# weiaicunzai/pytorch-camvid

Hardware: AMD Instinct MI355X
Metric: images/sec fwd+bwd UNet 3x360x480 bs=8 (higher is better)
Workload: dtype f32; 1 GPU; UNET(3,12) train fwd+bwd+CE, per-GPU batch 8 x 3x360x480 fp32 (BASELINE.json configs[1]); global_batch=8, parallelism=dp1

## Files before the change

include/cvk.h:

```cpp
#ifndef CVK_H
#define CVK_H

#include <stddef.h>
#include <stdint.h>

#ifdef __cplusplus
extern "C" {
#endif

#define CVK_VERSION 100
#define CVK_OK 0
#define CVK_EINVAL (-1)
#define CVK_EWORKSPACE (-2)
#define CVK_STAT_ROWS 64

typedef struct cvk_view {
    float*  ptr;
    int64_t sN, sY, sX;
} cvk_view;

typedef struct cvk_viewh {
    void*   ptr;
    int64_t sN, sY, sX;
} cvk_viewh;

int         cvk_version(void);
uint64_t    cvk_abi_hash(void);
const char* cvk_last_error_string(void);

int cvk_import_nchw(const float* src, int64_t sN, int64_t sC, int64_t sH, int64_t sW,
                    float* dst, int ld, int N, int C, int H, int W, void* stream);
int cvk_export_nchw(const float* src, int ld, float* dst, int64_t dN, int64_t dC, int64_t dH, int64_t dW,
                    int N, int C, int H, int W, void* stream);
int cvk_zero_frame(cvk_view buf, int N, int H, int W, int C, int y0, int x0, int h, int w, void* stream);

int cvk_conv3x3_fwd(const float* x, const float* w, const float* bias, float* y, float* stats,
                    int N, int H, int W, int Cin, int Cout, int ldy, void* stream);
int cvk_pack_weight_fwd(const float* w_src, float* dst, int Cout, int Cin, int Cin_pad, void* stream);
int cvk_pack_weight_dgrad(const float* w_src, float* dst, int Cout, int Cin, int Cin_pad, int Cout_pad, void* stream);
size_t cvk_conv3x3_wgrad_workspace_bytes(int N, int H, int W, int Cin_pad, int Cout);
int cvk_conv3x3_wgrad(const float* x, const float* dy, float* dw, int N, int H, int W, int Cin, int Cin_pad,
                      int Cout, int ld_dy, void* workspace, size_t workspace_bytes, void* stream);

int cvk_wino_weight_transform(const float* w, float* U, int Cout, int Cin, void* stream);
size_t cvk_conv3x3_wino_workspace_bytes(int N, int H, int W, int Cout_ld);
int cvk_conv3x3_wino_gemm(const float* x, const float* U, float* Mo, int N, int H, int W, int Cin, int Cout, int ldm,
                          void* stream);
int cvk_wino_output(const float* Mo, const float* bias, float* y, float* stats, int N, int H, int W, int Cout, int ldy,
                    void* stream);

int cvk_wino4_weight_transform(const float* w, float* U, int Cout, int Cin, void* stream);
int cvk_wino4_weight_transform_dgrad(const float* w, float* U, int Cout, int Cin, void* stream);
int cvk_conv3x3_wino4_ksplit(int N, int H, int W, int Cin, int Cout_ld);
size_t cvk_conv3x3_wino4_workspace_bytes(int N, int H, int W, int Cin, int Cout_ld);
int cvk_conv3x3_wino4_gemm(const float* x, const float* U, float* Mo, int N, int H, int W, int Cin, int Cout, int ldm,
                           void* stream);
int cvk_wino4_output(const float* Mo, const float* bias, float* y, float* stats, int N, int H, int W, int Cout, int ldy,
                     int ksplit, void* stream);

int cvk_w2d_tiles(int N, int H, int W);
int cvk_w2d_tpad(int T);
int cvk_w2d_stat_partials(int N, int H, int W);
size_t cvk_conv3x3_w2d_workspace_bytes(int N, int H, int W, int Cin, int Cout);
int cvk_w2d_weight_transform(const float* w, float* U, int Cout, int Cin, void* stream);
int cvk_w2d_weight_transform_dgrad(const float* w, float* U, int Cout, int Cin, void* stream);
int cvk_conv3x3_w2d(const float* x, const float* U, const float* bias, float* y, float* stats, float* counts, int N, int H,
                    int W, int Cin, int Cout, int ldy, void* workspace, size_t workspace_bytes, void* stream);
int cvk_w2d_ksplit(int T, int Cin, int Cout);
int cvk_w2d_input_transform(const float* x, float* V, int N, int H, int W, int Cin, void* stream);
int cvk_w2d_gemm(const float* V, const float* U, float* Mo, int T, int Cin, int Cout, void* stream);
int cvk_w2d_output(const float* Mo, const float* bias, float* y, float* stats, float* counts, int N, int H, int W, int Cin,
                   int Cout, int ldy, void* stream);
size_t cvk_conv3x3_wgrad_w2d_workspace_bytes(int N, int H, int W, int Cin_pad, int Cout);
int cvk_conv3x3_wgrad_w2d(const float* x, const float* dy, float* dw, int N, int H, int W, int Cin, int Cin_pad, int Cout,
                          int ld_dy, void* workspace, size_t workspace_bytes, void* stream);
int cvk_w2d_wgrad_ksplit(int T, int Cin_pad, int Cout);
int cvk_w2d_dy_transform(const float* dy, int ld_dy, float* E, int N, int H, int W, int Cout, void* stream);
int cvk_w2d_dy_transform_both(const float* dy, int ld_dy, float* Vp, float* E, int N, int H, int W, int Cout, void* stream);
int cvk_w2d_gemm_tn(const float* E, const float* V, float* P, int T, int Cin_pad, int Cout, void* stream);
int cvk_w2d_wgrad_output(const float* P, float* dw, int T, int Cin, int Cin_pad, int Cout, void* stream);

int cvk_w6_tiles(int N, int H, int W);
int cvk_w6_stat_partials(int N, int H, int W);
size_t cvk_conv3x3_w6_workspace_bytes(int N, int H, int W, int Cin, int Cout);
int cvk_w6_weight_transform(const float* w, float* U, int Cout, int Cin, void* stream);
int cvk_w6_weight_transform_dgrad(const float* w, float* U, int Cout, int Cin, void* stream);
int cvk_w6_ksplit(int T, int Cin, int Cout);
int cvk_w6_input_transform(const float* x, float* V, int N, int H, int W, int Cin, void* stream);
int cvk_w6_gemm(const float* V, const float* U, float* Mo, int T, int Cin, int Cout, void* stream);
int cvk_w6_output(const float* Mo, const float* bias, float* y, float* stats, float* counts, int N, int H, int W, int Cin,
                  int Cout, int ldy, void* stream);
int cvk_w6_wgrad_ksplit(int T, int Cin_pad, int Cout);
int cvk_w6_dy_transform(const float* dy, int ld_dy, float* E, int N, int H, int W, int Cout, void* stream);
int cvk_w6_dy_transform_both(const float* dy, int ld_dy, float* Vp, float* E, int N, int H, int W, int Cout, void* stream);
int cvk_w6_gemm_tn(const float* E, const float* V, float* P, int T, int Cin_pad, int Cout, void* stream);
int cvk_split3_rows_pad(int R, int mult);
int cvk_split3_planes(const float* P, void* S, int NX, int R, int Rpad, int C, void* stream);
int cvk_w2d_gemm_split3(const void* V3, const void* U3, float* Mo, int NX, int T, int Tpad, int Cin, int Cout, int Cpad, void* stream);
int cvk_amax_block_words(void);
unsigned cvk_amax_block_value(const unsigned* host_words, int n);
int cvk_absmax_f32(const float* x, long rows, int C, int ld, void* amax_block, void* stream);
int cvk_split_scale_exponent(int tile, int kind, int xi, unsigned amax_block);
int cvk_split_planes(int fmt, int tile, int kind, const float* P, void* S, const void* amax, int NX, int R, int Rpad, int C, void* stream);
int cvk_w2d_gemm_split(int fmt, int tile, const void* V, const void* U, float* Mo, const void* amax_v, const void* amax_u, int NX, int T, int Tpad,
                       int Cin, int Cout, int Cpad, void* stream);
int cvk_w2d_input_transform_split3(int tile, const float* x, void* V3, int N, int H, int W, int Cin, void* stream);
int cvk_w2d_dy_transform_both_split3(int tile, const float* dy, int ld_dy, void* Vp3, void* E, int e_split, int N, int H, int W, int C,
                                     void* stream);
int cvk_w2d_weight_transform_split3(int tile, const float* w, void* U3, float* tmp, int Cout, int Cin, int dgrad, void* stream);
int cvk_w2d_input_transform_split(int fmt, int tile, const float* x, void* V, const void* amax_x, int N, int H, int W, int Cin, void* stream);
int cvk_w2d_dy_transform_both_split(int fmt, int tile, const float* dy, int ld_dy, void* Vp, void* E, int e_split, const void* amax_dy, int N, int H,
                                    int W, int C, void* stream);
int cvk_w2d_weight_transform_split(int fmt, int tile, const float* w, void* U, const void* amax_w, int Cout, int Cin, int dgrad, void* stream);
int cvk_w2d_output_plain(int tile, const float* Mo, const float* bias, float* y, float* stats, float* counts, int N, int H, int W,
                         int Cout, int ldy, void* stream);
int cvk_w2d_gemm_tn_split3_ksplit(int NX, int Tpad, int Cin, int Cout);
int cvk_w2d_gemm_tn_split3(const void* E3, const void* V3, float* P, int NX, int Tpad, int Cin, int Cout, void* stream);
int cvk_w2d_gemm_tn_split(int fmt, int tile, const void* E, const void* V, float* P, const void* amax_e, const void* amax_v, int NX, int Tpad, int Cin,
                          int Cout, void* stream);
int cvk_w2d_wgrad_output_f(int tile, const float* P, float* dw, int Cin, int Cin_pad, int Cout, int f, void* stream);
int cvk_w6_wgrad_output(const float* P, float* dw, int T, int Cin, int Cin_pad, int Cout, void* stream);
int cvk_wino4h_weight_transform(const float* w, void* Uh, const void* amax_w, int Cn, int Ck, int dgrad, void* stream);
int cvk_conv3x3_wino4h(const float* x, const void* Uh, const float* bias, float* y, float* stats, float* counts, const void* amax_x,
                       const void* amax_w, int N, int H, int W, int Cin, int Cout, int ldy, int max_workgroups, void* stream);
int cvk_conv3x3_wino4h_bnred(const float* x, const void* Uh, float* y, const void* amax_x, const void* amax_w, int N, int H, int W, int Cin,
                             int Cout, int ldy, const float* yP, const float* scale, const float* shift, const float* mean,
                             const float* rstd, float* part, int max_workgroups, void* stream);
size_t cvk_wino4f_weight_floats(int Cn, int Ck);
int cvk_wino4f_weight_transform(const float* w, float* Uf, int Cn, int Ck, int dgrad, void* stream);
#define CVK_WT_BATCH_MAX 48
typedef struct cvk_wt_job { const float* w; float* out; int rows, cols, tile, dgrad; } cvk_wt_job;
int cvk_wino4f_weight_transform_batch(const cvk_wt_job* jobs, int n, void* stream);
int cvk_w2d_weight_transform_batch(const cvk_wt_job* jobs, int n, void* stream);
int cvk_wino4f_stat_partials(int N, int H, int W);
int cvk_conv3x3_wino4f_vplanes(const float* x, const float* Uf, const float* bias, float* y, float* stats, float* counts, float* Vsm,
                               int N, int H, int W, int Cin, int Cout, int ldy, int max_workgroups, void* stream);
int cvk_conv3x3_wino4f(const float* x, const float* Uf, const float* bias, float* y, float* stats, float* counts, int N, int H,
                       int W, int Cin, int Cout, int ldy, int max_workgroups, void* stream);
int cvk_conv3x3_wino4f_bnred(const float* x, const float* Uf, float* y, int N, int H, int W, int Cin, int Cout, int ldy,
                             const float* yP, const float* scale, const float* shift, const float* mean, const float* rstd,
                             float* part, int max_workgroups, void* stream);

int cvk_thin_fwd_supported(int Cin_ld, int Cout, int ldy);
int cvk_thin_stat_partials(int N, int H, int W, int Cin_ld);
int cvk_conv3x3_thin_fwd(const float* x, const float* w, const float* bias, float* y, float* stats, float* counts, int N, int H,
                         int W, int Cin_ld, int Cout, int ldy, void* stream);
int cvk_thin_wgrad_supported(int Cin, int Cin_ld, int Cout, int ld_dy);
size_t cvk_conv3x3_thin_wgrad_workspace_bytes(int N, int H, int W, int Cin_ld, int Cout);
int cvk_conv3x3_thin_wgrad(const float* x, const float* dy, float* dw, int N, int H, int W, int Cin, int Cin_ld, int Cout,
                           int ld_dy, void* workspace, size_t workspace_bytes, void* stream);

size_t cvk_conv3x3_wgradp_workspace_bytes(int N, int H, int W, int Cin_pad, int Cout);
int cvk_conv3x3_wgradp(const float* x, const float* dy, const float* E6_pre, float* dw, int N, int H, int W, int Cin, int Cin_pad,
                       int Cout, int ld_dy, void* workspace, size_t workspace_bytes, void* stream);
long cvk_wgradp_plane_rows(int N, int H, int W);
int cvk_wgradp_planes(const float* t, int ld, float* planes, int N, int H, int W, int C, int is_dy, void* stream);
size_t cvk_wgradp_gemm_workspace_bytes(int N, int H, int W, int Cin_pad, int Cout);
int cvk_wgradp_gemm(const float* E6, const float* V6, float* dw, int N, int H, int W, int Cin, int Cin_pad, int Cout, void* workspace,
                    size_t workspace_bytes, void* stream);
int cvk_wgradp_zero_pads(float* planes, int N, int H, int W, int C, void* stream);
int cvk_wgradp_zero_pads_sm(float* planes, int N, int H, int W, int C, void* stream);
int cvk_wgradp_planes_sm(const float* x, int ld, float* planes, int N, int H, int W, int C, void* stream);
int cvk_wgradp_gemm_sm(const float* E6, const float* V6sm, float* dw, int N, int H, int W, int Cin, int Cin_pad, int Cout, void* workspace,
                       size_t workspace_bytes, void* stream);
int cvk_wgradp_zero_pads4(float* planes, int N, int H, int W, int C, void* stream);
int cvk_bn_bwd_dx_e4p(cvk_view dout, const float* y, int ldy, const float* scale, const float* shift, const float* mean,
                      const float* rstd, const float* dgamma, const float* dbeta, float* dy, int ld_dy, float* E4p, float* part,
                      int N, int H, int W, int C, int use_batch_stats, void* stream);
int cvk_wgradp_dy_slack(int W);
int cvk_wgradp_gemm_sm_dy(const float* E4p, const float* dy, const float* V6sm, float* dw, int N, int H, int W, int Cin, int Cin_pad, int Cout,
                          void* workspace, size_t workspace_bytes, void* stream);
int cvk_bn_bwd_dx_e6(cvk_view dout, const float* y, int ldy, const float* scale, const float* shift, const float* mean,
                     const float* rstd, const float* dgamma, const float* dbeta, float* dy, int ld_dy, float* E6, float* part,
                     int N, int H, int W, int C, int use_batch_stats, void* stream);

size_t cvk_conv3x3_wgrad_wino4_workspace_bytes(int N, int H, int W, int Cin_pad, int Cout, int ld_dy);
int cvk_conv3x3_wgrad_wino4(const float* x, const float* dy, const float* E_pre, float* dw, int N, int H, int W, int Cin,
                            int Cin_pad, int Cout, int ld_dy, void* workspace, size_t workspace_bytes, void* stream);
int cvk_bn_bwd_e_blocks(int N, int H, int W);
int cvk_bn_bwd_dx_e(cvk_view dout, const float* y, int ldy, const float* scale, const float* shift, const float* mean,
                    const float* rstd, const float* dgamma, const float* dbeta, float* dy, int ld_dy, float* E, float* part,
                    int N, int H, int W, int C, int use_batch_stats, void* stream);

size_t cvk_conv3x3_wgrad_wino_workspace_bytes(int N, int H, int W, int Cin_pad, int Cout);
int cvk_conv3x3_wgrad_wino(const float* x, const float* dy, float* dw, int N, int H, int W, int Cin, int Cin_pad,
                           int Cout, int ld_dy, void* workspace, size_t workspace_bytes, void* stream);

size_t cvk_bn_finalize_workspace_bytes(int P, int C);
int cvk_bn_finalize(const float* stats, int P, int M, int C, const float* gamma, const float* beta,
                    float* mean, float* rstd, float* scale, float* shift,
                    float* running_mean, float* running_var, int64_t* num_batches_tracked,
                    float momentum, float eps, void* workspace, size_t workspace_bytes, void* stream);
int cvk_bn_eval_params(const float* gamma, const float* beta, const float* running_mean, const float* running_var,
                       float* mean, float* rstd, float* scale, float* shift, int C, float eps, void* stream);
int cvk_bn_relu_apply(const float* y, int ldy, const float* scale, const float* shift, cvk_view out,
                      int N, int H, int W, int C, void* stream);
int cvk_bn_relu_apply_pool(const float* y, int ldy, const float* scale, const float* shift, cvk_view out, float* pool,
                           unsigned char* code, int N, int H, int W, int C, void* stream);
int cvk_bn_bwd_blocks(int M);
int cvk_bn_bwd_reduce(cvk_view dout, const float* y, int ldy, const float* scale, const float* shift,
                      const float* mean, const float* rstd, float* part, int N, int H, int W, int C, void* stream);
int cvk_colsum_finalize(const float* part, int PB, int C, float* out0, float* out1, void* stream);
#define CVK_COLSUM_BATCH_MAX 64
typedef struct cvk_colsum_job { const float* part; float* out; int PB, C; } cvk_colsum_job;
int cvk_colsum_finalize_batch(const cvk_colsum_job* jobs, int n, void* stream);
int cvk_bn_relu_apply_amax(const float* y, int ldy, const float* scale, const float* shift, cvk_view out, int N, int H, int W, int C,
                           void* amax_block, void* stream);
int cvk_bn_relu_apply_pool_amax(const float* y, int ldy, const float* scale, const float* shift, cvk_view out, float* pool,
                                unsigned char* code, int N, int H, int W, int C, void* amax_out, void* amax_pool, void* stream);
int cvk_bn_bwd_dx_e_amax(int six, cvk_view dout, const float* y, int ldy, const float* scale, const float* shift, const float* mean,
                         const float* rstd, const float* dgamma, const float* dbeta, float* dy, int ld_dy, float* E, float* part, int N, int H,
                         int W, int C, int use_batch_stats, void* amax_block, void* stream);
int cvk_bn_bwd_dx_amax(cvk_view dout, const float* y, int ldy, const float* scale, const float* shift, const float* mean,
                       const float* rstd, const float* dgamma, const float* dbeta, float* dy, int ld_dy, float* dbias_part, int N,
                       int H, int W, int C, int use_batch_stats, void* amax_block, void* stream);
int cvk_bn_bwd_dx(cvk_view dout, const float* y, int ldy, const float* scale, const float* shift,
                  const float* mean, const float* rstd, const float* dgamma, const float* dbeta,
                  float* dy, int ld_dy, float* dbias_part, int N, int H, int W, int C, int use_batch_stats, void* stream);

int cvk_maxpool2x2_fwd(cvk_view x, float* out, uint8_t* code, int N, int H, int W, int C, void* stream);
int cvk_maxpool2x2_bwd(const float* dout, cvk_view x, const uint8_t* code, cvk_view dx, int accumulate,
                       int N, int H, int W, int C, void* stream);
int cvk_maxpool2x2_bwd_bnred_blocks(int N, int H, int W, int C);
int cvk_maxpool2x2_bwd_bnred(const float* dout, cvk_view x, const uint8_t* code, cvk_view dx, int accumulate, int N, int H, int W, int C,
                             const float* yP, int ldp, const float* scale, const float* shift, const float* mean, const float* rstd,
                             float* part, void* stream);
int cvk_maxunpool2x2_fwd(const float* v, const uint8_t* code, float* out, int N, int H, int W, int C, void* stream);
int cvk_maxunpool2x2_bwd(const float* dout, const uint8_t* code, float* dv, int N, int H, int W, int C, void* stream);
int cvk_pool_code_to_index(const uint8_t* code, int64_t* idx, int N, int H, int W, int C, void* stream);

int cvk_bilinear_up2_fwd(const float* x, float* out, int N, int H, int W, int C, void* stream);
int cvk_bilinear_up2_bwd(const float* dout, float* dx, int N, int H, int W, int C, void* stream);

int cvk_ce_blocks(int M);
int cvk_softmax_ce_fwd(const float* logits, int ld, const int64_t* target, float* part, float* loss,
                       int M, int C, int ignore_index, void* stream);
int cvk_softmax_ce_bwd(const float* logits, int ld, const int64_t* target, const float* loss3, const float* grad_out,
                       float scale, float* dlogits, int ld_d, int M, int C, int ignore_index, void* stream);

#define CVK_REDUCTION_NONE 0
#define CVK_REDUCTION_MEAN 1
#define CVK_REDUCTION_SUM 2
int cvk_ce_ex_part_floats(int M);
int cvk_softmax_ce_fwd_ex(const float* logits, int ld, const int64_t* target, const float* weight, float label_smoothing,
                          int reduction, float* part, float* loss, float* loss_px, int M, int C, int ignore_index, void* stream);
int cvk_softmax_ce_bwd_ex(const float* logits, int ld, const int64_t* target, const float* weight, float label_smoothing,
                          int reduction, const float* loss4, const float* grad_out, float scale, float* dlogits, int ld_d,
                          int M, int C, int ignore_index, void* stream);

#define CVK_DICE_PRESENT 0
#define CVK_DICE_ALL 1
int cvk_seg_loss_part_floats(int M, int C);
int cvk_seg_loss_record_floats(int C);
int cvk_seg_loss_fwd(const float* logits, int ld, const int64_t* target, const float* weight, float ce, float dice, float focal_gamma,
                     float dice_smooth, int dice_average, float* part, float* record, int M, int C, int ignore_index, void* stream);
int cvk_seg_loss_bwd(const float* logits, int ld, const int64_t* target, const float* weight, float ce, float dice, float focal_gamma,
                     const float* record, const float* grad_out, float scale, float* dlogits, int ld_d, int M, int C, int ignore_index,
                     void* stream);

int cvk_ohem_scratch_bytes(int M);
int cvk_ohem_record_floats(void);
int cvk_ohem_ce_fwd(const float* logits, int ld, const int64_t* target, const float* weight, float loss_thresh, int min_kept,
                    void* scratch, float* record, float* loss_px, int M, int C, int ignore_index, void* stream);
int cvk_ohem_ce_bwd(const float* logits, int ld, const int64_t* target, const float* weight, const float* record,
                    const float* loss_px, const float* grad_out, float scale, float* dlogits, int ld_d, int M, int C, int ignore_index,
                    void* stream);

int cvk_class_histogram(const void* masks, int mask_bytes, int N, int64_t HW, int num_classes, int ignore_index, int64_t* hist,
                        void* stream);

int cvk_argmax_channels(const float* logits, int ld, int64_t* out, int M, int C, void* stream);
int cvk_confusion_accumulate(const int64_t* pred, const int64_t* label, int64_t* hist, int M, int num_classes,
                             int ignore_index, void* stream);

int cvk_tta_accumulate(const float* logits, int ld, int h, int w, float* acc, int64_t* pred, int N, int H, int W, int C, int flip,
                       int first, int last, float inv_k, void* stream);
int cvk_tta_resize_input(const float* src, int64_t sN, int64_t sC, int64_t sH, int64_t sW, float* dst, int N, int H, int W, int h, int w,
                         int flip, void* stream);

int cvk_window_merge(const float* logits, int ld, float* out, int64_t* pred, int N, int H, int W, int C, int hc, int wc, int sy, int sx,
                     int iy, int ix, void* stream);

int cvk_preprocess_u8(const uint8_t* src, float* dst, int N, int H, int W, const float* mean3, const float* std3, void* stream);

typedef struct cvk_augment_record {
    int32_t flip;
    int32_t ksize;
    int32_t use_lut;
    int32_t reserved;
    float   taps[12];
    uint8_t lut[256];
} cvk_augment_record;
int cvk_augment_record_bytes(void);
int cvk_augment_u8(const uint8_t* frames, const void* masks, int mask_bytes, int N, int Hs, int Ws, int H, int W,
// ... 105 lines not shown
```

pytorch-camvid_amd/_lib.py:

```python
import ctypes
import os
import subprocess
import threading

_HERE = os.path.dirname(os.path.abspath(__file__))
LIB_PATH = os.environ.get("CVK_LIB_PATH") or os.path.join(_HERE, "lib", "libcvk.so")
CSRC = os.path.join(_HERE, "csrc")
HEADER = os.path.join(os.path.dirname(_HERE), "include", "cvk.h")

CVK_STAT_ROWS = 64

c_f32p = ctypes.c_void_p
c_i64 = ctypes.c_int64
c_int = ctypes.c_int
c_size = ctypes.c_size_t
c_float = ctypes.c_float
c_vp = ctypes.c_void_p


class View(ctypes.Structure):
    _fields_ = [("ptr", ctypes.c_void_p), ("sN", ctypes.c_int64), ("sY", ctypes.c_int64), ("sX", ctypes.c_int64)]


class ViewH(ctypes.Structure):
    _fields_ = [("ptr", ctypes.c_void_p), ("sN", ctypes.c_int64), ("sY", ctypes.c_int64), ("sX", ctypes.c_int64)]


SIGNATURES = {
    "cvk_version": (c_int, []),
    "cvk_abi_hash": (ctypes.c_uint64, []),
    "cvk_last_error_string": (ctypes.c_char_p, []),
    "cvk_import_nchw": (c_int, [c_vp, c_i64, c_i64, c_i64, c_i64, c_vp, c_int, c_int, c_int, c_int, c_int, c_vp]),
    "cvk_export_nchw": (c_int, [c_vp, c_int, c_vp, c_i64, c_i64, c_i64, c_i64, c_int, c_int, c_int, c_int, c_vp]),
    "cvk_zero_frame": (c_int, [View, c_int, c_int, c_int, c_int, c_int, c_int, c_int, c_int, c_vp]),
    "cvk_conv3x3_fwd": (c_int, [c_vp, c_vp, c_vp, c_vp, c_vp, c_int, c_int, c_int, c_int, c_int, c_int, c_vp]),
    "cvk_pack_weight_fwd": (c_int, [c_vp, c_vp, c_int, c_int, c_int, c_vp]),
    "cvk_pack_weight_dgrad": (c_int, [c_vp, c_vp, c_int, c_int, c_int, c_int, c_vp]),
    "cvk_conv3x3_wgrad_workspace_bytes": (c_size, [c_int, c_int, c_int, c_int, c_int]),
    "cvk_conv3x3_wgrad": (c_int, [c_vp, c_vp, c_vp, c_int, c_int, c_int, c_int, c_int, c_int, c_int, c_vp, c_size, c_vp]),
    "cvk_wino_weight_transform": (c_int, [c_vp, c_vp, c_int, c_int, c_vp]),
    "cvk_conv3x3_wino_workspace_bytes": (c_size, [c_int, c_int, c_int, c_int]),
    "cvk_conv3x3_wino_gemm": (c_int, [c_vp, c_vp, c_vp, c_int, c_int, c_int, c_int, c_int, c_int, c_vp]),
    "cvk_wino_output": (c_int, [c_vp, c_vp, c_vp, c_vp, c_int, c_int, c_int, c_int, c_int, c_vp]),
    "cvk_wino4_weight_transform": (c_int, [c_vp, c_vp, c_int, c_int, c_vp]),
    "cvk_wino4_weight_transform_dgrad": (c_int, [c_vp, c_vp, c_int, c_int, c_vp]),
    "cvk_conv3x3_wino4_ksplit": (c_int, [c_int, c_int, c_int, c_int, c_int]),
    "cvk_conv3x3_wino4_workspace_bytes": (c_size, [c_int, c_int, c_int, c_int, c_int]),
    "cvk_conv3x3_wino4_gemm": (c_int, [c_vp, c_vp, c_vp, c_int, c_int, c_int, c_int, c_int, c_int, c_vp]),
    "cvk_wino4_output": (c_int, [c_vp, c_vp, c_vp, c_vp, c_int, c_int, c_int, c_int, c_int, c_int, c_vp]),
    "cvk_wino4f_weight_floats": (c_size, [c_int, c_int]),
    "cvk_wino4f_weight_transform": (c_int, [c_vp, c_vp, c_int, c_int, c_int, c_vp]),
    "cvk_wino4f_weight_transform_batch": (c_int, [c_vp, c_int, c_vp]),
    "cvk_w2d_weight_transform_batch": (c_int, [c_vp, c_int, c_vp]),
    "cvk_wino4f_stat_partials": (c_int, [c_int, c_int, c_int]),
    "cvk_conv3x3_wino4f": (c_int, [c_vp, c_vp, c_vp, c_vp, c_vp, c_vp, c_int, c_int, c_int, c_int, c_int, c_int, c_int, c_vp]),
    "cvk_conv3x3_wino4f_bnred": (c_int, [c_vp, c_vp, c_vp, c_int, c_int, c_int, c_int, c_int, c_int, c_vp, c_vp, c_vp, c_vp, c_vp, c_vp, c_int, c_vp]),
    "cvk_wino4h_weight_transform": (c_int, [c_vp, c_vp, c_vp, c_int, c_int, c_int, c_vp]),
    "cvk_conv3x3_wino4h": (c_int, [c_vp, c_vp, c_vp, c_vp, c_vp, c_vp, c_vp, c_vp, c_int, c_int, c_int, c_int, c_int, c_int, c_int, c_vp]),
    "cvk_conv3x3_wino4h_bnred": (c_int, [c_vp, c_vp, c_vp, c_vp, c_vp, c_int, c_int, c_int, c_int, c_int, c_int, c_vp, c_vp, c_vp, c_vp, c_vp, c_vp,
                                         c_int, c_vp]),
    "cvk_thin_fwd_supported": (c_int, [c_int, c_int, c_int]),
    "cvk_thin_stat_partials": (c_int, [c_int, c_int, c_int, c_int]),
    "cvk_conv3x3_thin_fwd": (c_int, [c_vp, c_vp, c_vp, c_vp, c_vp, c_vp, c_int, c_int, c_int, c_int, c_int, c_int, c_vp]),
    "cvk_thin_wgrad_supported": (c_int, [c_int, c_int, c_int, c_int]),
    "cvk_conv3x3_thin_wgrad_workspace_bytes": (c_size, [c_int, c_int, c_int, c_int, c_int]),
    "cvk_conv3x3_thin_wgrad": (c_int, [c_vp, c_vp, c_vp, c_int, c_int, c_int, c_int, c_int, c_int, c_int, c_vp, c_size, c_vp]),
    "cvk_conv3x3_wgradp_workspace_bytes": (c_size, [c_int, c_int, c_int, c_int, c_int]),
    "cvk_conv3x3_wgradp": (c_int, [c_vp, c_vp, c_vp, c_vp, c_int, c_int, c_int, c_int, c_int, c_int, c_int, c_vp, c_size, c_vp]),
    "cvk_wgradp_plane_rows": (ctypes.c_long, [c_int, c_int, c_int]),
    "cvk_wgradp_planes": (c_int, [c_vp, c_int, c_vp, c_int, c_int, c_int, c_int, c_int, c_vp]),
    "cvk_wgradp_gemm_workspace_bytes": (c_size, [c_int, c_int, c_int, c_int, c_int]),
    "cvk_wgradp_gemm": (c_int, [c_vp, c_vp, c_vp, c_int, c_int, c_int, c_int, c_int, c_int, c_vp, c_size, c_vp]),
    "cvk_wgradp_zero_pads": (c_int, [c_vp, c_int, c_int, c_int, c_int, c_vp]),
    "cvk_wgradp_zero_pads_sm": (c_int, [c_vp, c_int, c_int, c_int, c_int, c_vp]),
    "cvk_wgradp_planes_sm": (c_int, [c_vp, c_int, c_vp, c_int, c_int, c_int, c_int, c_vp]),
    "cvk_wgradp_gemm_sm": (c_int, [c_vp, c_vp, c_vp, c_int, c_int, c_int, c_int, c_int, c_int, c_vp, c_size, c_vp]),
    "cvk_wgradp_zero_pads4": (c_int, [c_vp, c_int, c_int, c_int, c_int, c_vp]),
    "cvk_bn_bwd_dx_e4p": (c_int, [View, c_vp, c_int, c_vp, c_vp, c_vp, c_vp, c_vp, c_vp, c_vp, c_int, c_vp, c_vp,
                                  c_int, c_int, c_int, c_int, c_int, c_vp]),
    "cvk_wgradp_dy_slack": (c_int, [c_int]),
    "cvk_wgradp_gemm_sm_dy": (c_int, [c_vp, c_vp, c_vp, c_vp, c_int, c_int, c_int, c_int, c_int, c_int, c_vp, c_size, c_vp]),
    "cvk_conv3x3_wino4f_vplanes": (c_int, [c_vp, c_vp, c_vp, c_vp, c_vp, c_vp, c_vp, c_int, c_int, c_int, c_int, c_int, c_int, c_int, c_vp]),
    "cvk_bn_bwd_dx_e6": (c_int, [View, c_vp, c_int, c_vp, c_vp, c_vp, c_vp, c_vp, c_vp, c_vp, c_int, c_vp, c_vp,
                                 c_int, c_int, c_int, c_int, c_int, c_vp]),
    "cvk_w2d_tiles": (c_int, [c_int, c_int, c_int]),
    "cvk_w6_tiles": (c_int, [c_int, c_int, c_int]),
    "cvk_w6_stat_partials": (c_int, [c_int, c_int, c_int]),
    "cvk_conv3x3_w6_workspace_bytes": (c_size, [c_int, c_int, c_int, c_int, c_int]),
    "cvk_w6_weight_transform": (c_int, [c_vp, c_vp, c_int, c_int, c_vp]),
    "cvk_w6_weight_transform_dgrad": (c_int, [c_vp, c_vp, c_int, c_int, c_vp]),
    "cvk_w6_input_transform": (c_int, [c_vp, c_vp, c_int, c_int, c_int, c_int, c_vp]),
    "cvk_w6_gemm": (c_int, [c_vp, c_vp, c_vp, c_int, c_int, c_int, c_vp]),
    "cvk_w6_wgrad_ksplit": (c_int, [c_int, c_int, c_int]),
    "cvk_w6_dy_transform": (c_int, [c_vp, c_int, c_vp, c_int, c_int, c_int, c_int, c_vp]),
    "cvk_w6_gemm_tn": (c_int, [c_vp, c_vp, c_vp, c_int, c_int, c_int, c_vp]),
    "cvk_w6_wgrad_output": (c_int, [c_vp, c_vp, c_int, c_int, c_int, c_int, c_vp]),
    "cvk_w6_ksplit": (c_int, [c_int, c_int, c_int]),
    "cvk_w6_output": (c_int, [c_vp, c_vp, c_vp, c_vp, c_vp, c_int, c_int, c_int, c_int, c_int, c_int, c_vp]),
    "cvk_w2d_stat_partials": (c_int, [c_int, c_int, c_int]),
    "cvk_conv3x3_w2d_workspace_bytes": (c_size, [c_int, c_int, c_int, c_int, c_int]),
    "cvk_w2d_weight_transform": (c_int, [c_vp, c_vp, c_int, c_int, c_vp]),
    "cvk_w2d_weight_transform_dgrad": (c_int, [c_vp, c_vp, c_int, c_int, c_vp]),
    "cvk_w2d_input_transform": (c_int, [c_vp, c_vp, c_int, c_int, c_int, c_int, c_vp]),
    "cvk_w2d_gemm": (c_int, [c_vp, c_vp, c_vp, c_int, c_int, c_int, c_vp]),
    "cvk_conv3x3_wgrad_w2d_workspace_bytes": (c_size, [c_int, c_int, c_int, c_int, c_int]),
    "cvk_conv3x3_wgrad_w2d": (c_int, [c_vp, c_vp, c_vp, c_int, c_int, c_int, c_int, c_int, c_int, c_int, c_vp, c_size, c_vp]),
    "cvk_w2d_tpad": (c_int, [c_int]),
    "cvk_split3_rows_pad": (c_int, [c_int, c_int]),
    "cvk_split3_planes": (c_int, [c_vp, c_vp, c_int, c_int, c_int, c_int, c_vp]),
    "cvk_w2d_gemm_split3": (c_int, [c_vp, c_vp, c_vp, c_int, c_int, c_int, c_int, c_int, c_int, c_vp]),
    "cvk_w2d_input_transform_split3": (c_int, [c_int, c_vp, c_vp, c_int, c_int, c_int, c_int, c_vp]),
    "cvk_w2d_dy_transform_both_split3": (c_int, [c_int, c_vp, c_int, c_vp, c_vp, c_int, c_int, c_int, c_int, c_int, c_vp]),
    "cvk_w2d_weight_transform_split3": (c_int, [c_int, c_vp, c_vp, c_vp, c_int, c_int, c_int, c_vp]),
    "cvk_w2d_output_plain": (c_int, [c_int, c_vp, c_vp, c_vp, c_vp, c_vp, c_int, c_int, c_int, c_int, c_int, c_vp]),
    "cvk_w2d_gemm_tn_split3_ksplit": (c_int, [c_int, c_int, c_int, c_int]),
    "cvk_w2d_gemm_tn_split3": (c_int, [c_vp, c_vp, c_vp, c_int, c_int, c_int, c_int, c_vp]),
    "cvk_amax_block_words": (c_int, []),
    "cvk_amax_block_value": (ctypes.c_uint, [c_vp, c_int]),
    "cvk_absmax_f32": (c_int, [c_vp, ctypes.c_long, c_int, c_int, c_vp, c_vp]),
    "cvk_split_scale_exponent": (c_int, [c_int, c_int, c_int, ctypes.c_uint]),
    "cvk_split_planes": (c_int, [c_int, c_int, c_int, c_vp, c_vp, c_vp, c_int, c_int, c_int, c_int, c_vp]),
    "cvk_w2d_gemm_split": (c_int, [c_int, c_int, c_vp, c_vp, c_vp, c_vp, c_vp, c_int, c_int, c_int, c_int, c_int, c_int, c_vp]),
    "cvk_w2d_input_transform_split": (c_int, [c_int, c_int, c_vp, c_vp, c_vp, c_int, c_int, c_int, c_int, c_vp]),
    "cvk_w2d_dy_transform_both_split": (c_int, [c_int, c_int, c_vp, c_int, c_vp, c_vp, c_int, c_vp, c_int, c_int, c_int, c_int, c_vp]),
    "cvk_w2d_weight_transform_split": (c_int, [c_int, c_int, c_vp, c_vp, c_vp, c_int, c_int, c_int, c_vp]),
    "cvk_w2d_gemm_tn_split": (c_int, [c_int, c_int, c_vp, c_vp, c_vp, c_vp, c_vp, c_int, c_int, c_int, c_int, c_vp]),
    "cvk_w2d_wgrad_output_f": (c_int, [c_int, c_vp, c_vp, c_int, c_int, c_int, c_int, c_vp]),
    "cvk_w2d_wgrad_ksplit": (c_int, [c_int, c_int, c_int]),
    "cvk_w2d_dy_transform": (c_int, [c_vp, c_int, c_vp, c_int, c_int, c_int, c_int, c_vp]),
    "cvk_w2d_dy_transform_both": (c_int, [c_vp, c_int, c_vp, c_vp, c_int, c_int, c_int, c_int, c_vp]),
    "cvk_w6_dy_transform_both": (c_int, [c_vp, c_int, c_vp, c_vp, c_int, c_int, c_int, c_int, c_vp]),
    "cvk_w2d_gemm_tn": (c_int, [c_vp, c_vp, c_vp, c_int, c_int, c_int, c_vp]),
    "cvk_w2d_wgrad_output": (c_int, [c_vp, c_vp, c_int, c_int, c_int, c_int, c_vp]),
    "cvk_w2d_ksplit": (c_int, [c_int, c_int, c_int]),
    "cvk_w2d_output": (c_int, [c_vp, c_vp, c_vp, c_vp, c_vp, c_int, c_int, c_int, c_int, c_int, c_int, c_vp]),
    "cvk_conv3x3_w2d": (c_int, [c_vp, c_vp, c_vp, c_vp, c_vp, c_vp, c_int, c_int, c_int, c_int, c_int, c_int, c_vp, c_size, c_vp]),
    "cvk_conv3x3_wgrad_wino4_workspace_bytes": (c_size, [c_int, c_int, c_int, c_int, c_int, c_int]),
    "cvk_conv3x3_wgrad_wino4": (c_int, [c_vp, c_vp, c_vp, c_vp, c_int, c_int, c_int, c_int, c_int, c_int, c_int, c_vp, c_size, c_vp]),
    "cvk_bn_bwd_e_blocks": (c_int, [c_int, c_int, c_int]),
    "cvk_bn_bwd_dx_e": (c_int, [View, c_vp, c_int, c_vp, c_vp, c_vp, c_vp, c_vp, c_vp, c_vp, c_int, c_vp, c_vp,
                                c_int, c_int, c_int, c_int, c_int, c_vp]),
    "cvk_conv3x3_wgrad_wino_workspace_bytes": (c_size, [c_int, c_int, c_int, c_int, c_int]),
    "cvk_conv3x3_wgrad_wino": (c_int, [c_vp, c_vp, c_vp, c_int, c_int, c_int, c_int, c_int, c_int, c_int, c_vp, c_size, c_vp]),
    "cvk_bn_finalize_workspace_bytes": (c_size, [c_int, c_int]),
    "cvk_bn_finalize": (c_int, [c_vp, c_int, c_int, c_int, c_vp, c_vp, c_vp, c_vp, c_vp, c_vp, c_vp, c_vp, c_vp,
                                c_float, c_float, c_vp, c_size, c_vp]),
    "cvk_bn_eval_params": (c_int, [c_vp, c_vp, c_vp, c_vp, c_vp, c_vp, c_vp, c_vp, c_int, c_float, c_vp]),
    "cvk_bn_relu_apply": (c_int, [c_vp, c_int, c_vp, c_vp, View, c_int, c_int, c_int, c_int, c_vp]),
    "cvk_bn_relu_apply_pool": (c_int, [c_vp, c_int, c_vp, c_vp, View, c_vp, c_vp, c_int, c_int, c_int, c_int, c_vp]),
    "cvk_bn_bwd_blocks": (c_int, [c_int]),
    "cvk_bn_bwd_reduce": (c_int, [View, c_vp, c_int, c_vp, c_vp, c_vp, c_vp, c_vp, c_int, c_int, c_int, c_int, c_vp]),
    "cvk_colsum_finalize": (c_int, [c_vp, c_int, c_int, c_vp, c_vp, c_vp]),
    "cvk_colsum_finalize_batch": (c_int, [c_vp, c_int, c_vp]),
    "cvk_bn_bwd_dx": (c_int, [View, c_vp, c_int, c_vp, c_vp, c_vp, c_vp, c_vp, c_vp, c_vp, c_int, c_vp,
                              c_int, c_int, c_int, c_int, c_int, c_vp]),
    "cvk_bn_relu_apply_amax": (c_int, [c_vp, c_int, c_vp, c_vp, View, c_int, c_int, c_int, c_int, c_vp, c_vp]),
    "cvk_bn_relu_apply_pool_amax": (c_int, [c_vp, c_int, c_vp, c_vp, View, c_vp, c_vp, c_int, c_int, c_int, c_int, c_vp, c_vp, c_vp]),
    "cvk_bn_bwd_dx_e_amax": (c_int, [c_int, View, c_vp, c_int, c_vp, c_vp, c_vp, c_vp, c_vp, c_vp, c_vp, c_int, c_vp, c_vp,
                                     c_int, c_int, c_int, c_int, c_int, c_vp, c_vp]),
    "cvk_bn_bwd_dx_amax": (c_int, [View, c_vp, c_int, c_vp, c_vp, c_vp, c_vp, c_vp, c_vp, c_vp, c_int, c_vp,
                                   c_int, c_int, c_int, c_int, c_int, c_vp, c_vp]),
    "cvk_maxpool2x2_fwd": (c_int, [View, c_vp, c_vp, c_int, c_int, c_int, c_int, c_vp]),
    "cvk_maxpool2x2_bwd": (c_int, [c_vp, View, c_vp, View, c_int, c_int, c_int, c_int, c_int, c_vp]),
    "cvk_maxpool2x2_bwd_bnred_blocks": (c_int, [c_int, c_int, c_int, c_int]),
    "cvk_maxpool2x2_bwd_bnred": (c_int, [c_vp, View, c_vp, View, c_int, c_int, c_int, c_int, c_int, c_vp, c_int, c_vp, c_vp, c_vp, c_vp, c_vp, c_vp]),
    "cvk_maxunpool2x2_fwd": (c_int, [c_vp, c_vp, c_vp, c_int, c_int, c_int, c_int, c_vp]),
    "cvk_maxunpool2x2_bwd": (c_int, [c_vp, c_vp, c_vp, c_int, c_int, c_int, c_int, c_vp]),
    "cvk_pool_code_to_index": (c_int, [c_vp, c_vp, c_int, c_int, c_int, c_int, c_vp]),
    "cvk_bilinear_up2_fwd": (c_int, [c_vp, c_vp, c_int, c_int, c_int, c_int, c_vp]),
    "cvk_bilinear_up2_bwd": (c_int, [c_vp, c_vp, c_int, c_int, c_int, c_int, c_vp]),
    "cvk_ce_blocks": (c_int, [c_int]),
    "cvk_softmax_ce_fwd": (c_int, [c_vp, c_int, c_vp, c_vp, c_vp, c_int, c_int, c_int, c_vp]),
    "cvk_softmax_ce_bwd": (c_int, [c_vp, c_int, c_vp, c_vp, c_vp, c_float, c_vp, c_int, c_int, c_int, c_int, c_vp]),
    "cvk_ce_ex_part_floats": (c_int, [c_int]),
    "cvk_softmax_ce_fwd_ex": (c_int, [c_vp, c_int, c_vp, c_vp, c_float, c_int, c_vp, c_vp, c_vp, c_int, c_int, c_int, c_vp]),
    "cvk_softmax_ce_bwd_ex": (c_int, [c_vp, c_int, c_vp, c_vp, c_float, c_int, c_vp, c_vp, c_float, c_vp, c_int, c_int, c_int, c_int,
                                      c_vp]),
    "cvk_seg_loss_part_floats": (c_int, [c_int, c_int]),
    "cvk_seg_loss_record_floats": (c_int, [c_int]),
    "cvk_seg_loss_fwd": (c_int, [c_vp, c_int, c_vp, c_vp, c_float, c_float, c_float, c_float, c_int, c_vp, c_vp, c_int, c_int, c_int, c_vp]),
    "cvk_seg_loss_bwd": (c_int, [c_vp, c_int, c_vp, c_vp, c_float, c_float, c_float, c_vp, c_vp, c_float, c_vp, c_int, c_int, c_int, c_int,
                                 c_vp]),
    "cvk_ohem_scratch_bytes": (c_int, [c_int]),
    "cvk_ohem_record_floats": (c_int, []),
    "cvk_ohem_ce_fwd": (c_int, [c_vp, c_int, c_vp, c_vp, c_float, c_int, c_vp, c_vp, c_vp, c_int, c_int, c_int, c_vp]),
    "cvk_ohem_ce_bwd": (c_int, [c_vp, c_int, c_vp, c_vp, c_vp, c_vp, c_vp, c_float, c_vp, c_int, c_int, c_int, c_int, c_vp]),
    "cvk_class_histogram": (c_int, [c_vp, c_int, c_int, c_i64, c_int, c_int, c_vp, c_vp]),
    "cvk_argmax_channels": (c_int, [c_vp, c_int, c_vp, c_int, c_int, c_vp]),
    "cvk_confusion_accumulate": (c_int, [c_vp, c_vp, c_vp, c_int, c_int, c_int, c_vp]),
    "cvk_tta_accumulate": (c_int, [c_vp, c_int, c_int, c_int, c_vp, c_vp, c_int, c_int, c_int, c_int, c_int, c_int, c_int, c_float, c_vp]),
    "cvk_tta_resize_input": (c_int, [c_vp, c_i64, c_i64, c_i64, c_i64, c_vp, c_int, c_int, c_int, c_int, c_int, c_int, c_vp]),
    "cvk_window_merge": (c_int, [c_vp, c_int, c_vp, c_vp, c_int, c_int, c_int, c_int, c_int, c_int, c_int, c_int, c_int, c_int, c_vp]),
    "cvk_preprocess_u8": (c_int, [c_vp, c_vp, c_int, c_int, c_int, ctypes.POINTER(ctypes.c_float), ctypes.POINTER(ctypes.c_float), c_vp]),
    "cvk_augment_record_bytes": (c_int, []),
    "cvk_augment_u8": (c_int, [c_vp, c_vp, c_int, c_int, c_int, c_int, c_int, c_int, c_vp, ctypes.POINTER(ctypes.c_float),
                               ctypes.POINTER(ctypes.c_float), c_vp, c_vp, c_vp, c_vp]),
    "cvk_bf16s_rows_pad": (c_int, [c_int]),
    "cvk_bf16s_stat_partials": (c_int, [c_int, c_int, c_int]),
    "cvk_bf16s_stat_partials_c": (c_int, [c_int, c_int, c_int, c_int, c_int]),
    "cvk_pack_weight_fwd_bf16": (c_int, [c_vp, c_vp, c_int, c_int, c_int, c_vp]),
    "cvk_pack_weight_dgrad_bf16": (c_int, [c_vp, c_vp, c_int, c_int, c_int, c_vp]),
    "cvk_pack_weights_bf16_batch": (c_int, [c_vp, c_int, c_vp]),
    "cvk_conv3x3_bf16s": (c_int, [c_vp, c_vp, c_vp, c_vp, c_vp, c_vp, c_int, c_int, c_int, c_int, c_int, c_int, c_vp]),
    "cvk_conv3x3_bf16s_wg": (c_int, [c_vp, c_vp, c_vp, c_vp, c_vp, c_vp, c_int, c_int, c_int, c_int, c_int, c_int, c_int, c_vp]),
    "cvk_conv3x3_bf16s_kernel": (c_int, [c_int, c_int, c_int, c_int, c_int, c_int]),
    "cvk_thin_bf16_mode": (c_int, [c_int, c_int, c_int, c_int, c_int]),
    "cvk_thin_bf16_stat_partials": (c_int, [c_int, c_int, c_int]),
    "cvk_thin_bf16_pack_elems": (c_size, [c_int]),
    "cvk_pack_weight_thin_bf16": (c_int, [c_vp, c_vp, c_int, c_int, c_int, c_vp]),
    "cvk_conv3x3_thin_bf16": (c_int, [c_vp, c_vp, c_vp, c_vp, c_vp, c_vp, c_int, c_int, c_int, c_int, c_int, c_int, c_int, c_vp]),
# ... 145 lines not shown
```

pytorch-camvid_amd/conv_fp32.py:

```python
import torch

from . import _lib
from ._lib import check
from .engine import _BF16, _F32, Op, Saved, _empty, _timed, amax_blocks, channels_last
from .route import pad4


def w2fn(lib, tile, name):
    return getattr(lib, ("cvk_w6_" if tile == 6 else "cvk_w2d_") + name)


_PLANE_DT = {0: _F32, 2: torch.float16, 3: _BF16}


def planes2d(lib, tile, N, H, W, fmt=0):
    T = w2fn(lib, tile, "tiles")(N, H, W)
    return 64 if tile == 6 else 36, T, lib.cvk_split3_rows_pad(T, 256) if fmt else lib.cvk_w2d_tpad(T)


def plane_elems(NX, Tp, C, fmt=0):
    return NX * (C // 32) * fmt * Tp * 32 if fmt else NX * Tp * C + 128


def absmax(R, t, rows, cols, ld, s, what):
    a = amax_blocks(R.lib, 1, t.device)[0]
    _timed(R, "k_absmax", 4.0 * rows * cols, lambda: check(R.lib.cvk_absmax_f32(t.data_ptr(), rows, cols, ld, a.data_ptr(), s), "cvk_absmax_f32(%s)" % what), "byte")
    return a


def amax_call(lib, name, args, blocks, s):
    if blocks.count(None) == len(blocks):
        return getattr(lib, name)(*args, s)
    return getattr(lib, name + "_amax")(*args, *(b.data_ptr() if b is not None else None for b in blocks), s)


class WinoConv:

    def __init__(self, R, s, x, w, bias, y, sp, N, H, W, k_ch, cout, ldy, flops, wsrc, ck, what="", dgrad_of=None):
        self.R, self.lib, self.s, self.x, self.w, self.bias, self.y, self.sp = R, R.lib, s, x, w, bias, y, sp
        self.N, self.H, self.W, self.M, self.k_ch, self.cout, self.ldy = N, H, W, N * H * W, k_ch, cout, ldy
        self.flops, self.wsrc, self.ck, self.what, self.dgrad_of = flops, wsrc, ck, what, dgrad_of
        self.wt = dgrad_of[0] if dgrad_of is not None else w
        self.v = self.v_amax = self.bnred_sums = None

    def run(self, fam, tile=0, fmt=0, keep=False, v_pre=None, x_amax=None, bnred=None):
        if fam == "w2d":
            return self.w2d(tile, keep, v_pre)
        if fam == "w2d_split":
            return self.w2d_split(tile, fmt, keep, v_pre, x_amax)
        if fam in ("w4f", "w4f_vplanes", "w4h"):
            return self.w4f(fam == "w4f_vplanes", bnred, fam == "w4h", x_amax)
        return self.w4() if fam == "w4" else self.w2()

    def _filter(self, kind, build, job=None):
        d = self.dgrad_of
        straight = self.wt.data_ptr() == self.wsrc.data_ptr() and (d is None or (d[1] == self.k_ch and d[2] == self.cout))
        return self.R.derived((self.ck, kind), self.wsrc, build, job if straight else None)

    def _amax_w(self):
        wt = self.wt
        return self.R.derived(((self.ck[0], "a"), "amaxw"), self.wsrc, lambda: absmax(self.R, wt, wt.numel() // 4, 4, 4, self.s, "w"))

    def _counts(self, P):
        return self.sp + 4 * 2 * P * self.cout if self.sp is not None else None

    def w2d(self, tile, keep, v_pre):
        R, lib, s, x, d = self.R, self.lib, self.s, self.x, self.dgrad_of
        N, H, W, M, k_ch, cout, ldy = self.N, self.H, self.W, self.M, self.k_ch, self.cout, self.ldy
        NX, T, Tp = planes2d(lib, tile, N, H, W)

        dg = d is not None and d[1] == k_ch and d[2] == cout
        rows, cols = (d[1], d[2]) if dg else (cout, k_ch)

        def build():
            u, wt = _empty(NX * cout * k_ch, x.device), d[0] if dg else (self.w() if callable(self.w) else self.w)
            kind = "weight_transform_dgrad" if dg else "weight_transform"
            _timed(R, "k_w2d_weight_dgrad" if dg else "k_w2d_weight", 4.0 * (9 + NX) * cout * k_ch, lambda: check(
                w2fn(lib, tile, kind)(wt.data_ptr(), u.data_ptr(), rows, cols, s), "cvk_w2d_" + kind), "byte")
            return u
        U = self._filter("w2d%d" % tile, build, ("w2d", NX * cout * k_ch, rows, cols, tile, int(d is not None)))
        vfl = plane_elems(NX, Tp, k_ch)
        if keep:
            self.v = _empty(vfl, x.device)
        Vt = v_pre if v_pre is not None else self.v
        wsb = (lib.cvk_conv3x3_w6_workspace_bytes if tile == 6 else lib.cvk_conv3x3_w2d_workspace_bytes)(N, H, W, k_ch, cout)
        ws = R.workspace(wsb - (4 * vfl if Vt is not None else 0), x.device)
        V, Mo = (Vt.data_ptr(), ws.data_ptr()) if Vt is not None else (ws.data_ptr(), ws.data_ptr() + 4 * vfl)
        P2 = w2fn(lib, tile, "stat_partials")(N, H, W)
        cnt = self._counts(P2)
        if v_pre is None:
            _timed(R, "k_w2d_input", 4.0 * (M + NX * T) * k_ch, lambda: check(
                w2fn(lib, tile, "input_transform")(x.data_ptr(), V, N, H, W, k_ch, s), "cvk_w2d_input_transform" + self.what), "byte")
        _timed(R, "k_w2d_gemm<128, 32, 2, 2>", self.flops, lambda: check(w2fn(lib, tile, "gemm")(V, U.data_ptr(), Mo, T, k_ch, cout, s), "cvk_w2d_gemm" + self.what),
            executed=2.0 * NX * T * k_ch * cout)
        _timed(R, "k_w2d_output", 4.0 * (NX * T + M) * cout, lambda: check(
            w2fn(lib, tile, "output")(Mo, self.bias, self.y.data_ptr(), self.sp, cnt, N, H, W, k_ch, cout, ldy, s), "cvk_w2d_output" + self.what), "byte")
        return (P2, cnt) if self.sp is not None else None

    def w2d_split(self, tile, fmt, keep, v_pre, x_amax):
        R, lib, s, x, d = self.R, self.lib, self.s, self.x, self.dgrad_of
        N, H, W, M, k_ch, cout, ldy = self.N, self.H, self.W, self.M, self.k_ch, self.cout, self.ldy
        (NX, T, Tp), pdt = planes2d(lib, tile, N, H, W, fmt), _PLANE_DT[fmt]
        tag = "split3" if fmt == 3 else "split2h"
        Cp = lib.cvk_split3_rows_pad(cout, 128)
        wt = self.wt
        am_w = self._amax_w() if fmt == 2 else None

        def build():
            u3 = torch.empty(NX * (k_ch // 32) * fmt * Cp * 32, device=x.device, dtype=pdt)
            amp = am_w.data_ptr() if am_w is not None else None
            rows, cols = (d[1], d[2]) if d is not None else (cout, k_ch)
            _timed(R, ("k_w2d_weight_dgrad+" if d is not None else "k_w2d_weight+") + tag, 4.0 * 9 * cout * k_ch + 2.0 * fmt * NX * cout * k_ch,
                   lambda: check(lib.cvk_w2d_weight_transform_split(fmt, tile, wt.data_ptr(), u3.data_ptr(), amp, rows, cols, int(d is not None), s),
                                 "cvk_w2d_weight_transform_split" + ("(dgrad)" if d is not None else "")), "byte")
            return u3
        U3 = self._filter("w2ds%d_%d" % (fmt, tile), build)
        am_x = x_amax
        if v_pre is not None:
            V3 = v_pre
        else:
            V3 = torch.empty(plane_elems(NX, Tp, k_ch, fmt), device=x.device, dtype=pdt)
            if fmt == 2 and am_x is None:
                am_x = absmax(R, x, M, k_ch, k_ch, s, "x")
            if keep:
                self.v, self.v_amax = V3, am_x
            _timed(R, "k_w2d_input<%s>" % tag, (4.0 * M + 2.0 * fmt * NX * T) * k_ch, lambda: check(
                lib.cvk_w2d_input_transform_split(fmt, tile, x.data_ptr(), V3.data_ptr(), am_x.data_ptr() if am_x is not None else None,
                                                  N, H, W, k_ch, s), "cvk_w2d_input_transform_split" + self.what), "byte")
        ws = R.workspace(4 * NX * T * cout + 1024, x.device)
        _timed(R, "k_gemm_" + tag, self.flops, lambda: check(
            lib.cvk_w2d_gemm_split(fmt, tile, V3.data_ptr(), U3.data_ptr(), ws.data_ptr(), am_x.data_ptr() if am_x is not None else None,
                                   am_w.data_ptr() if am_w is not None else None, NX, T, Tp, k_ch, cout, Cp, s), "cvk_w2d_gemm_split" + self.what),
            executed=2.0 * (6 if fmt == 3 else 3) * NX * Tp * k_ch * Cp)
        P2 = w2fn(lib, tile, "stat_partials")(N, H, W)
        cnt = self._counts(P2)
        _timed(R, "k_w2d_output", 4.0 * (NX * T + M) * cout, lambda: check(
            lib.cvk_w2d_output_plain(tile, ws.data_ptr(), self.bias, self.y.data_ptr(), self.sp, cnt, N, H, W, cout, ldy, s),
            "cvk_w2d_output_plain" + self.what), "byte")
        return (P2, cnt) if self.sp is not None else None

    def w4f(self, vplanes=False, bnred=None, h2=False, x_amax=None):
        R, lib, s, x, d, wt = self.R, self.lib, self.s, self.x, self.dgrad_of, self.wt
        N, H, W, M, k_ch, cout, ldy, flops = self.N, self.H, self.W, self.M, self.k_ch, self.cout, self.ldy, self.flops
        floats, dg, f = lib.cvk_wino4f_weight_floats(cout, k_ch), int(d is not None), "h" if h2 else "f"
        am_w = self._amax_w() if h2 else None

        def build():
            u, name = _empty(floats, x.device), "cvk_wino4%s_weight_transform" % f
            _timed(R, "k_wino4%s_weight" % f, 4.0 * (9 + 18) * cout * k_ch, lambda: check(getattr(lib, name)(
                wt.data_ptr(), u.data_ptr(), *((am_w.data_ptr(),) if h2 else ()), cout, k_ch, dg, s), name + ("(dgrad)" if dg and not h2 else "")), "byte")
            return u
        U = self._filter("w4" + f, build, None if h2 else ("w4f", floats, cout, k_ch, 0, dg))
        am = ()
        if h2:
            am_x = x_amax if x_amax is not None else absmax(R, x, M, k_ch, k_ch, s, "x")
            am = (am_x.data_ptr(), am_w.data_ptr())
        executed = (1.5 if h2 else 0.5) * flops
        Pf = lib.cvk_wino4f_stat_partials(N, H, W)
        cnt = self._counts(Pf)
        if bnred is not None:
            bpart = _empty(2 * Pf * cout, x.device)
            name = "cvk_conv3x3_wino4%s_bnred" % f
            _timed(R, "k_conv3x3_wino4%s<bnred>" % f, flops, lambda: check(getattr(lib, name)(
                x.data_ptr(), U.data_ptr(), self.y.data_ptr(), *am, N, H, W, k_ch, cout, ldy, *bnred, bpart.data_ptr(), R.launch_wgs(), s), name), executed=executed)
            self.bnred_sums = (bpart, Pf)
            return None
        if vplanes:
            self.v = _empty(6 * lib.cvk_wgradp_plane_rows(N, H, W) * k_ch, x.device)
            check(lib.cvk_wgradp_zero_pads_sm(self.v.data_ptr(), N, H, W, k_ch, s), "cvk_wgradp_zero_pads_sm")
            _timed(R, "k_conv3x3_wino4f<vplanes>", flops, lambda: check(
                lib.cvk_conv3x3_wino4f_vplanes(x.data_ptr(), U.data_ptr(), self.bias, self.y.data_ptr(), self.sp, cnt, self.v.data_ptr(), N, H, W,
                                               k_ch, cout, ldy, R.launch_wgs(), s), "cvk_conv3x3_wino4f_vplanes" + self.what), executed=executed)
        else:
            name = "cvk_conv3x3_wino4" + f
            _timed(R, "k_conv3x3_wino4" + f, flops, lambda: check(getattr(lib, name)(
                x.data_ptr(), U.data_ptr(), self.bias, self.y.data_ptr(), self.sp, cnt, *am, N, H, W, k_ch, cout, ldy, R.launch_wgs(), s),
                name + self.what), executed=executed)
        return (Pf, cnt) if self.sp is not None else None

    def w4(self):
        R, lib, s, x, d = self.R, self.lib, self.s, self.x, self.dgrad_of
        N, H, W, M, k_ch, cout, ldy = self.N, self.H, self.W, self.M, self.k_ch, self.cout, self.ldy

        dg = d is not None and d[1] == k_ch and d[2] == cout

        def build():
            u, wt = _empty(6 * cout * 3 * k_ch, x.device), d[0] if dg else (self.w() if callable(self.w) else self.w)
            kind = "weight_transform_dgrad" if dg else "weight_transform"
            _timed(R, "k_wino4_weight_dgrad" if dg else "k_wino4_weight", 4.0 * (9 + 18) * cout * k_ch, lambda: check(getattr(lib, "cvk_wino4_" + kind)(
                wt.data_ptr(), u.data_ptr(), *((d[1], d[2]) if dg else (cout, k_ch)), s), "cvk_wino4_" + kind), "byte")
            return u
        U = self._filter("w4", build)
        ws = R.workspace(lib.cvk_conv3x3_wino4_workspace_bytes(N, H, W, k_ch, ldy), x.device)
        ksplit = lib.cvk_conv3x3_wino4_ksplit(N, H, W, k_ch, ldy)
        _timed(R, conv_kernel_name("wino4", ldy), self.flops, lambda: check(
            lib.cvk_conv3x3_wino4_gemm(x.data_ptr(), U.data_ptr(), ws.data_ptr(), N, H, W, k_ch, cout, ldy, s), "cvk_conv3x3_wino4_gemm" + self.what))
        _timed(R, "k_wino4_output", (4.0 + 6.0 * ksplit) * M * ldy, lambda: check(
            lib.cvk_wino4_output(ws.data_ptr(), self.bias, self.y.data_ptr(), self.sp, N, H, W, cout, ldy, ksplit, s), "cvk_wino4_output"), "byte")

    def w2(self):
        R, lib, s, x = self.R, self.lib, self.s, self.x
        N, H, W, M, k_ch, cout, ldy = self.N, self.H, self.W, self.M, self.k_ch, self.cout, self.ldy

        def build():
            wt = self.w() if callable(self.w) else self.w
            u = _empty(4 * cout * 3 * k_ch, x.device)
            _timed(R, "k_wino_weight", 4.0 * (9 + 12) * cout * k_ch, lambda: check(
                lib.cvk_wino_weight_transform(wt.data_ptr(), u.data_ptr(), cout, k_ch, s), "cvk_wino_weight_transform"), "byte")
            return u
        U = self._filter("w", build)
        ws = R.workspace(lib.cvk_conv3x3_wino_workspace_bytes(N, H, W, ldy), x.device)
        _timed(R, conv_kernel_name("wino", ldy), self.flops, lambda: check(
            lib.cvk_conv3x3_wino_gemm(x.data_ptr(), U.data_ptr(), ws.data_ptr(), N, H, W, k_ch, cout, ldy, s), "cvk_conv3x3_wino_gemm" + self.what))
        _timed(R, "k_wino_output", 12.0 * M * ldy, lambda: check(
            lib.cvk_wino_output(ws.data_ptr(), self.bias, self.y.data_ptr(), self.sp, N, H, W, cout, ldy, s), "cvk_wino_output"), "byte")


class WeightGrad:

    def __init__(self, R, s, x, dy, gw, N, H, W, cin, k_ch, cout, ldy, flops):
        self.R, self.lib, self.s, self.x, self.dy, self.gw = R, R.lib, s, x, dy, gw
        self.N, self.H, self.W, self.M, self.cin, self.k_ch, self.cout, self.ldy, self.flops = N, H, W, N * H * W, cin, k_ch, cout, ldy, flops

    def run(self, fam, tile=0, fmt=0, V=None, am_v=None, E=None, dy_e=False, Eb=None, am_dy=None):
        if fam == "w2d":
            return self.w2d(tile, V, Eb)
        if fam == "w2d_split":
            return self.w2d_split(tile, fmt, V, am_v, Eb, am_dy)
        if fam in ("wgradp", "wgradp_sm"):
            return self.wgradp(fam == "wgradp", V, E, dy_e and E is not None)
        return self.w4(E) if fam == "w4" else self.direct(fam)

    def w2d(self, tile, V, Eb):
        R, lib, s, x, dy = self.R, self.lib, self.s, self.x, self.dy
        N, H, W, M, k_ch, C, ldy = self.N, self.H, self.W, self.M, self.k_ch, self.cout, self.ldy
        NX, T, Tp = planes2d(lib, tile, N, H, W)
        efl = plane_elems(NX, Tp, C)
        f = w2fn(lib, tile, "wgrad_ksplit")(T, k_ch, C)
        if V is None:
            V = _empty(plane_elems(NX, Tp, k_ch), x.device)
            _timed(R, "k_w2d_input", 4.0 * (M + NX * T) * k_ch, lambda: check(
                w2fn(lib, tile, "input_transform")(x.data_ptr(), V.data_ptr(), N, H, W, k_ch, s), "cvk_w2d_input_transform(wgrad)"), "byte")
        ws = R.workspace(4 * ((0 if Eb is not None else efl) + f * NX * C * k_ch), x.device)
        Ep, Pp = (Eb.data_ptr(), ws.data_ptr()) if Eb is not None else (ws.data_ptr(), ws.data_ptr() + 4 * efl)
        if Eb is None:
            _timed(R, "k_w2d_dy", 4.0 * (M + NX * T) * C, lambda: check(
                w2fn(lib, tile, "dy_transform")(dy.data_ptr(), ldy, Ep, N, H, W, C, s), "cvk_w2d_dy_transform"), "byte")
        _timed(R, "k_w2d_gemm_tn", self.flops, lambda: check(
            w2fn(lib, tile, "gemm_tn")(Ep, V.data_ptr(), Pp, T, k_ch, C, s), "cvk_w2d_gemm_tn"), executed=2.0 * NX * Tp * k_ch * C)
        _timed(R, "k_w2d_wgrad_out", 4.0 * (NX * f + 9) * C * self.cin, lambda: check(
            w2fn(lib, tile, "wgrad_output")(Pp, self.gw, T, self.cin, k_ch, C, s), "cvk_w2d_wgrad_output"), "byte")

    def w2d_split(self, tile, fmt, V, am_v, Eb, am_dy):
        R, lib, s, k_ch, C = self.R, self.lib, self.s, self.k_ch, self.cout
        NX, _, Tp = planes2d(lib, tile, self.N, self.H, self.W, fmt)
        f = lib.cvk_w2d_gemm_tn_split3_ksplit(NX, Tp, k_ch, C)
        ws = R.workspace(4 * f * NX * C * k_ch, self.x.device)
        _timed(R, "k_gemm_tn_" + ("split3" if fmt == 3 else "split2h"), self.flops, lambda: check(
            lib.cvk_w2d_gemm_tn_split(fmt, tile, Eb.data_ptr(), V.data_ptr(), ws.data_ptr(), am_dy.data_ptr() if am_dy is not None else None,
                                      am_v.data_ptr() if am_v is not None else None, NX, Tp, k_ch, C, s), "cvk_w2d_gemm_tn_split"),
            executed=2.0 * (6 if fmt == 3 else 3) * NX * Tp * k_ch * C)
        _timed(R, "k_w2d_wgrad_out", 4.0 * (NX * f + 9) * C * self.cin, lambda: check(
            lib.cvk_w2d_wgrad_output_f(tile, ws.data_ptr(), self.gw, self.cin, k_ch, C, f, s), "cvk_w2d_wgrad_output_f"), "byte")

    def wgradp(self, own_v, V, E, sm_dy):
        R, lib, s, x, dy = self.R, self.lib, self.s, self.x, self.dy
        N, H, W, M, k_ch, C, ldy = self.N, self.H, self.W, self.M, self.k_ch, self.cout, self.ldy
        rows6 = lib.cvk_wgradp_plane_rows(N, H, W)
        wsb = lib.cvk_wgradp_gemm_workspace_bytes(N, H, W, k_ch, C)
        nE = 0 if E is not None else 6 * rows6 * C
        nV = 6 * rows6 * k_ch if own_v else 0
        ws = R.workspace(4 * (nV + nE) + wsb, x.device)
        V6p = ws.data_ptr() if own_v else V.data_ptr()
        E6p = E.data_ptr() if E is not None else ws.data_ptr() + 4 * nV
        slabp = ws.data_ptr() + 4 * (nV + nE)
        if own_v:
            _timed(R, "k_wgradp_planes", 4.0 * (M + 6.0 * rows6) * k_ch, lambda: check(
                lib.cvk_wgradp_planes(x.data_ptr(), k_ch, V6p, N, H, W, k_ch, 0, s), "cvk_wgradp_planes(x)"), "byte")
        if E is None:
            _timed(R, "k_wgradp_planes", 4.0 * (M + 6.0 * rows6) * C, lambda: check(
                lib.cvk_wgradp_planes(dy.data_ptr(), ldy, E6p, N, H, W, C, 1, s), "cvk_wgradp_planes(dy)"), "byte")
        fn = "cvk_wgradp_gemm_sm_dy" if sm_dy else ("cvk_wgradp_gemm" if own_v else "cvk_wgradp_gemm_sm")
        ev = (E6p, dy.data_ptr(), V6p) if sm_dy else (E6p, V6p)
        _timed(R, "k_wgradp_gemm", self.flops, lambda: check(getattr(lib, fn)(*ev, self.gw, N, H, W, self.cin, k_ch, C, slabp, wsb, s), fn),
               executed=9.0 * M * C * self.cin)

    def w4(self, E):
        R, lib, N, H, W, k_ch, C, ldy = self.R, self.lib, self.N, self.H, self.W, self.k_ch, self.cout, self.ldy
        wsb = lib.cvk_conv3x3_wgrad_wino4_workspace_bytes(N, H, W, k_ch, C, ldy)
        ws = R.workspace(wsb, self.x.device)
        _timed(R, f"k_wgrad_wino4<{'128' if C > 64 else '64'}, 128, 2, 2>", self.flops, lambda: check(
            lib.cvk_conv3x3_wgrad_wino4(self.x.data_ptr(), self.dy.data_ptr(), E.data_ptr() if E is not None else None, self.gw, N, H, W,
                                        self.cin, k_ch, C, ldy, ws.data_ptr(), wsb, self.s), "cvk_conv3x3_wgrad_wino4"))

    def direct(self, fam):
        R, lib, N, H, W, M, k_ch, C, ldy = self.R, self.lib, self.N, self.H, self.W, self.M, self.k_ch, self.cout, self.ldy
        fn = {"thin": "cvk_conv3x3_thin_wgrad", "w2": "cvk_conv3x3_wgrad_wino", "direct": "cvk_conv3x3_wgrad"}[fam]
        wsb = getattr(lib, fn + "_workspace_bytes")(N, H, W, k_ch, C)
        ws = R.workspace(wsb, self.x.device)
        head = k_ch == 64
        name, kw = {"thin": ("k_thin_co_wgrad" if head else "k_thin_ci_wgrad",
                             dict(executed=18.0 * M * (16 * self.cin if head else C * 16 / 3.0), nbytes=4.0 * M * (k_ch + ldy))),
                    "w2": (f"k_wgrad_wino<{'128' if C > 64 else '64'}, 128, 2, 2>", {}), "direct": (conv_kernel_name("wgrad", C, k_ch), {})}[fam]
        _timed(R, name, self.flops, lambda: check(getattr(lib, fn)(
            self.x.data_ptr(), self.dy.data_ptr(), self.gw, N, H, W, self.cin, k_ch, C, ldy, ws.data_ptr(), wsb, self.s), fn), **kw)


def conv_kernel_name(kind, n_cols, k_ch=32):
    if kind in ("wino4", "wino"):
        return "k_conv3x3_%s<%s>" % (kind, "128, 128, 2, 2" if n_cols > 64 else ("128, 64, 2, 2" if n_cols > 32 else "128, 32, 4, 1"))
    if kind == "wgrad":
        if n_cols <= 16 and k_ch == 64:
            return "k_wgrad_smallco"
        t = "128, 128, 2, 2" if n_cols > 64 else ("64, 128, 2, 2" if n_cols > 32 else "32, 256, 1, 4")
        if 32 < n_cols <= 64 and k_ch * 9 <= 64:
            t = "64, 64, 2, 2"
        return f"k_conv3x3_wgrad<{t}>"
    t = "128, 128, 2, 2" if n_cols > 64 else ("128, 64, 2, 2" if n_cols > 32 else "256, 32, 4, 1")
    return f"k_conv3x3_igemm<{t}, {'true' if kind == 'fwd' else 'false'}, {'true' if k_ch % 32 == 0 else 'false'}>"


class ConvBnRelu(Op):
    _pitch, _ydt = staticmethod(pad4), _F32
    _BN = ("cvk_bn_bwd_blocks", "cvk_bn_bwd_reduce", "k_bn_bwd<reduce>")

    def __init__(self, src, dst, pslot, holder, cin, cout, src_needs_grad, bn_train=True, req=(True, True, True, True)):
        self.src, self.dst, self.pslot, self.holder = src, dst, pslot, holder
        self.cin, self.cout, self.src_needs_grad = cin, cout, src_needs_grad
        self.bn_train = bool(bn_train)
# ... 253 lines not shown
```

pytorch-camvid_amd/csrc/wino4f.hip:

```cpp
#include "conv_tile.h"
#include "lds_dma.h"
#include "split_fmt.h"
#include <utility>

namespace {

template <int... Ks, class F>
__device__ __forceinline__ void f_static_for(std::integer_sequence<int, Ks...>, F&& f) {
    (f(std::integral_constant<int, Ks>{}), ...);
}

constexpr int F_BM = 128, F_BN = 64, F_BK = 16;
constexpr int F_ABYTES = 6 * F_BM * 64;
constexpr int F_BBYTES = 6 * F_BN * 64;
constexpr int F_STAGE = F_ABYTES + F_BBYTES;
constexpr int F_CMAX = 512;
constexpr int F_CST = 5 * F_CMAX * 4;

template <bool H2 = false>
__device__ __forceinline__ void wino4f_weight_body(const float* __restrict__ w, float* __restrict__ Uf, int Cn, int Ck, int tilesN, int dgrad,
                                                   unsigned vblock, unsigned nblocks, const unsigned* __restrict__ amaxW = nullptr,
                                                   const CvkSplitTab& tabG = CvkSplitTab{}) {
    float sc[6] = {1.f, 1.f, 1.f, 1.f, 1.f, 1.f};
    if (H2) {
        const unsigned am = cvk_amax_read(amaxW);
#pragma unroll
        for (int x = 0; x < 6; ++x) sc[x] = cvk_pow2f(cvk_split_exp(am, cvk_split_tab_c(tabG, x), 0));
    }
    const int Nn = tilesN * F_BN;
    const size_t total = (size_t)Nn * 3 * Ck;
    for (size_t i = (size_t)vblock * blockDim.x + threadIdx.x; i < total; i += (size_t)nblocks * blockDim.x) {
        int n, r, k;
        if (dgrad) {
            n = (int)(i % Nn);
            const size_t q = i / Nn;
            k = (int)(q % Ck);
            r = (int)(q / Ck);
        } else {
            k = (int)(i % Ck);
            const size_t q = i / Ck;
            r = (int)(q % 3);
            n = (int)(q / 3);
        }
        double g0 = 0.0, g1 = 0.0, g2 = 0.0;
        if (n < Cn) {
            if (dgrad) {
                const float* g = w + ((size_t)(k * 3 + (2 - r)) * 3) * Cn + n;
                g0 = g[2 * (size_t)Cn]; g1 = g[Cn]; g2 = g[0];
            } else {
                const float* g = w + ((size_t)(n * 3 + r) * 3) * Ck + k;
                g0 = g[0]; g1 = g[Ck]; g2 = g[2 * (size_t)Ck];
            }
        }
        const int kk = r * Ck + k, slice = kk >> 4, kf = kk & 15;
        const int tn = n >> 6, nl = n & 63;
        if (H2) {
            const float u[6] = {(float)(0.25 * g0), (float)(-(g0 + g1 + g2) / 6.0), (float)(-(g0 - g1 + g2) / 6.0),
                                (float)(g0 / 24.0 + g1 / 12.0 + g2 / 6.0), (float)(g0 / 24.0 - g1 / 12.0 + g2 / 6.0), (float)g2};
            _Float16* const Uh = reinterpret_cast<_Float16*>(Uf);
            const int swz = (nl >> 2) & 3;
            const size_t row = (((size_t)(slice * tilesN + tn) * 6) * 64 + nl) * 32;
            const int p1 = (((kf >> 3) ^ swz) << 3) + (kf & 7), p2 = (((2 + (kf >> 3)) ^ swz) << 3) + (kf & 7);
#pragma unroll
            for (int x = 0; x < 6; ++x) {
                const float v = u[x] * sc[x];
                const _Float16 h1 = (_Float16)v;
                const _Float16 h2 = (_Float16)(v - (float)h1);
                Uh[row + (size_t)x * (64 * 32) + p1] = h1;
                Uh[row + (size_t)x * (64 * 32) + p2] = h2;
            }
            continue;
        }
        const size_t o = (((size_t)(slice * tilesN + tn) * 6) * 64 + nl) * 16 + (((kf >> 2) ^ ((nl >> 2) & 3)) << 2) + (kf & 3);
        const size_t ps = 64 * 16;
        Uf[o] = (float)(0.25 * g0);
        Uf[o + ps] = (float)(-(g0 + g1 + g2) / 6.0);
        Uf[o + 2 * ps] = (float)(-(g0 - g1 + g2) / 6.0);
        Uf[o + 3 * ps] = (float)(g0 / 24.0 + g1 / 12.0 + g2 / 6.0);
        Uf[o + 4 * ps] = (float)(g0 / 24.0 - g1 / 12.0 + g2 / 6.0);
        Uf[o + 5 * ps] = (float)g2;
    }
}

__global__ __launch_bounds__(256) void k_wino4f_weight(const float* __restrict__ w, float* __restrict__ Uf, int Cn, int Ck,
                                                      int tilesN, int dgrad) {
    wino4f_weight_body(w, Uf, Cn, Ck, tilesN, dgrad, blockIdx.x, gridDim.x);
}
__global__ __launch_bounds__(256) void k_wino4h_weight(const float* __restrict__ w, float* __restrict__ Uh, int Cn, int Ck, int tilesN, int dgrad,
                                                      const unsigned* __restrict__ amaxW, CvkSplitTab tabG) {
    wino4f_weight_body<true>(w, Uh, Cn, Ck, tilesN, dgrad, blockIdx.x, gridDim.x, amaxW, tabG);
}

struct F4WJobsDev { const float* w[CVK_WT_BATCH_MAX]; float* out[CVK_WT_BATCH_MAX]; int Cn[CVK_WT_BATCH_MAX], Ck[CVK_WT_BATCH_MAX], dgrad[CVK_WT_BATCH_MAX];
                    unsigned first[CVK_WT_BATCH_MAX + 1]; int n; };
__global__ __launch_bounds__(256) void k_wino4f_weight_batch(const F4WJobsDev jobs) {
    int j = 0;
    while (j + 1 < jobs.n && blockIdx.x >= jobs.first[j + 1]) ++j;
    wino4f_weight_body(jobs.w[j], jobs.out[j], jobs.Cn[j], jobs.Ck[j], (jobs.Cn[j] + F_BN - 1) / F_BN, jobs.dgrad[j],
                       blockIdx.x - jobs.first[j], jobs.first[j + 1] - jobs.first[j]);
}

__device__ __forceinline__ void f_dma16(const void* sbase, unsigned voff, unsigned lds_byte_addr) {
    asm volatile("s_mov_b32 m0, %2\n\ts_nop 0\n\tglobal_load_lds_dwordx4 %0, %1" : : "v"(voff), "s"(sbase), "s"(lds_byte_addr) : "memory");
}

struct FBnRed {
    const float* y;
    const float* scale;
    const float* shift;
    const float* mean;
    const float* rstd;
};

struct FSplit {
    const unsigned* amaxX;
    const unsigned* amaxW;
    CvkSplitTab tabB, tabG;
};
struct FVpl {
    float* p;
    long rows;
    int Wtp;
};
typedef unsigned u32x4f __attribute__((ext_vector_type(4)));
typedef _Float16 f16x8 __attribute__((ext_vector_type(8)));
typedef _Float16 f16x4 __attribute__((ext_vector_type(4)));
typedef float f32x2v __attribute__((ext_vector_type(2)));

template <bool STATS, int ABL = 0, bool BNR = false, bool H2 = false, bool VPL = false, bool CL = false>
__global__ __launch_bounds__(512, 2) void k_conv3x3_wino4f(
    const float* __restrict__ X, const float* __restrict__ Uf, const float* __restrict__ bias, float* __restrict__ Y,
    float* __restrict__ stats, float* __restrict__ counts, int Mt, int H, int W, int Wt, int Cin, int Cout, int ldy,
    int tilesN, int ntiles, int Mpix, int P, FBnRed bn, FSplit sp, FVpl vp) {
    static_assert(!(STATS && BNR), "forward statistics and the BatchNorm-backward sums are different launches");
    static_assert(!(VPL && (BNR || H2)), "the weight-grad's V planes are written by exact-fp32 forward launches only");
    static_assert(!(CL && H2) && !(VPL && !CL), "LDS constants: exact-fp32 variants; the plane-writing launch always has them");
    __shared__ __attribute__((aligned(1024))) char smem[2 * F_STAGE + 2048 + (CL ? F_CST : 0)];
    const unsigned smem_addr = cvk_lds_addr(smem);
    float* const red = reinterpret_cast<float*>(smem + 2 * F_STAGE);
    float* const cst = red + 512;
    if constexpr (CL) {
        const int c = threadIdx.x;
        const bool ok = c < Cout;
        cst[c] = (bias != nullptr && ok) ? bias[c] : 0.f;
        if (BNR) {
            cst[F_CMAX + c] = ok ? bn.scale[c] : 0.f;
            cst[2 * F_CMAX + c] = ok ? bn.shift[c] : 0.f;
            cst[3 * F_CMAX + c] = ok ? bn.mean[c] : 0.f;
            cst[4 * F_CMAX + c] = ok ? bn.rstd[c] : 0.f;
        }
    }

    const int tid = threadIdx.x, lane = tid & 63;
    const int wave = __builtin_amdgcn_readfirstlane(tid >> 6);
    const int li = lane & 31, lh = lane >> 5;
    const int wm = wave >> 1, wn = wave & 1;

    const int G = gridDim.x;
    const int nx = G < 8 ? G : 8;
    const int xcd = blockIdx.x % nx, wi = blockIdx.x / nx;
    const int ng = G / nx + (xcd < G % nx ? 1 : 0);
    const int xbeg = (int)((long)xcd * ntiles / nx), xend = (int)((long)(xcd + 1) * ntiles / nx);
    const int tbeg = xbeg + wi, tend = xend, tstride = ng;
    if (tbeg >= tend) return;
    const int ntw = (tend - tbeg + tstride - 1) / tstride;
    const int nS = 3 * Cin / F_BK;
    const int total = ntw * nS;
    float sA[6];
    CvkUnscale un[6];
#pragma unroll
    for (int x = 0; x < 6; ++x) { sA[x] = 1.f; un[x] = CvkUnscale{1.f, 1.f}; }
    if (H2) {
        const unsigned ax = cvk_amax_read(sp.amaxX), aw = cvk_amax_read(sp.amaxW);
#pragma unroll
        for (int x = 0; x < 6; ++x) {
            const int ea = cvk_split_exp(ax, cvk_split_tab_c(sp.tabB, x), 0), eu = cvk_split_exp(aw, cvk_split_tab_c(sp.tabG, x), 0);
            sA[x] = cvk_pow2f(ea);
            un[x] = cvk_unscale(-(ea + eu));
        }
    }

    const FastDiv divWt((unsigned)Wt), divH((unsigned)H);
    __amdgpu_buffer_rsrc_t xr;
    const __amdgpu_buffer_rsrc_t null_rsrc = __builtin_amdgcn_make_buffer_rsrc((void*)X, 0, 0, 0x00020000);

    const int srow = tid >> 2, schunk = tid & 3;
    unsigned ibase = 0, iflag = 0;
    unsigned aoff[6];
    constexpr unsigned VPO_NONE = 0xFFFFFFF0u;
    unsigned vpo = VPO_NONE;
    auto set_tile = [&](int tile) {
        const int m0 = (tile / tilesN) * F_BM;
        const int q0 = (int)divWt.div((unsigned)m0);
        const int first = q0 * W + 4 * (m0 - q0 * Wt);
        const long xfirst = ((long)first - (W + 1)) * Cin;
        const size_t xbytes = (size_t)((long)Mpix * Cin - xfirst) * 4;
        xr = __builtin_amdgcn_make_buffer_rsrc((void*)(X + xfirst), 0, (int)(xbytes < 0x7FFFFFFFu ? xbytes : 0x7FFFFFFFu), 0x00020000);
        const int t = m0 + srow;
        unsigned fl = 0, base = 0;
        if (t < Mt) {
            const int q = (int)divWt.div((unsigned)t), xt = t - q * Wt;
            const int nimg = (int)divH.div((unsigned)q);
            const int y = q - nimg * H;
            if (VPL) vpo = ((unsigned)(vp.Wtp + (q + 2 * nimg + 1) * vp.Wtp + xt) << 6) + (unsigned)schunk * 16u;
            fl = 2u | (y > 0 ? 1u : 0u) | (y + 1 < H ? 4u : 0u);
            fl |= (xt > 0 ? 8u : 0u) | 16u;
#pragma unroll
            for (int j = 2; j < 6; ++j) fl |= (4 * xt + j - 1 < W) ? (8u << j) : 0u;
            base = (unsigned)(q * W + 4 * xt - first) * (unsigned)Cin * 4u + (unsigned)schunk * 16u;
        }
        else if (VPL) vpo = VPO_NONE;
        ibase = base;
        iflag = fl;
    };
    auto regroup = [&](int r) {
        const unsigned cs = (unsigned)Cin * 4u;
#pragma unroll
        for (int j = 0; j < 6; ++j) {
            const unsigned need = (1u << r) | (8u << j);
            aoff[j] = oob_unless((iflag & need) == need, ibase + j * cs);
        }
    };

    int ltile = tbeg, lr = 0, lcib = 0, lleft = total;
    f32x4 d[2][6];
    auto load_A = [&](int set, int j) {
        const __amdgpu_buffer_rsrc_t xs = (lleft > 0 && !(ABL & 1)) ? xr : null_rsrc;
        const unsigned so = (unsigned)((lr * W * Cin + lcib) * 4);
        d[set][j] = __builtin_bit_cast(f32x4, __builtin_amdgcn_raw_buffer_load_b128(xs, aoff[j], so, 0));
    };
    auto advance_A = [&]() {
        --lleft;
        lcib += F_BK;
        const int w1 = lcib >= Cin;
        lcib = w1 ? 0 : lcib;
        lr += w1;
        const int w2 = lr == 3;
        lr = w2 ? 0 : lr;
        ltile += w2 ? tstride : 0;
    };
    auto issue_A = [&](int set) {
        if (lcib == 0) {
            if (lr == 0 && ltile < tend) set_tile(ltile);
            regroup(lr);
        }
#pragma unroll
        for (int j = 0; j < 6; ++j) load_A(set, j);
        advance_A();
    };
    f32x4 tv[6];
    auto xform2 = [&](int set, int p) {
        if (ABL & 2) return;
        auto pr = [&](int j) { return f32x2v{d[set][j][2 * p], d[set][j][2 * p + 1]}; };
        const f32x2v d0 = pr(0), d1 = pr(1), d2 = pr(2), d3 = pr(3), d4 = pr(4), d5 = pr(5);
        auto pkfma = [](unsigned long long cc, f32x2v u, f32x2v v) {
            f32x2v r;
            asm("v_pk_fma_f32 %0, %1, %2, %3" : "=v"(r) : "s"(cc), "v"(u), "v"(v));
            return r;
        };
        auto pkadd = [](f32x2v u, f32x2v v) {
            f32x2v r;
            asm("v_pk_add_f32 %0, %1, %2" : "=v"(r) : "v"(u), "v"(v));
            return r;
        };
        constexpr unsigned long long C_M4 = 0xC0800000C0800000ull, C_M1 = 0xBF800000BF800000ull, C_P4 = 0x4080000040800000ull,
                                     C_P2 = 0x4000000040000000ull, C_M2 = 0xC0000000C0000000ull, C_M5 = 0xC0A00000C0A00000ull;
        const f32x2v a = pkfma(C_M4, d2, d4), b = pkfma(C_M4, d1, d3), e = pkfma(C_M1, d2, d4), f = pkfma(C_M1, d1, d3);
        const f32x2v t0 = pkfma(C_P4, d0, pkfma(C_M5, d2, d4)), t1 = pkadd(a, b), t2 = pkfma(C_M1, b, a), t3 = pkfma(C_P2, f, e),
                     t4 = pkfma(C_M2, f, e), t5 = pkfma(C_P4, d1, pkfma(C_M5, d3, d5));
        tv[0][2 * p] = t0[0]; tv[0][2 * p + 1] = t0[1]; tv[1][2 * p] = t1[0]; tv[1][2 * p + 1] = t1[1];
        tv[2][2 * p] = t2[0]; tv[2][2 * p + 1] = t2[1]; tv[3][2 * p] = t3[0]; tv[3][2 * p + 1] = t3[1];
        tv[4][2 * p] = t4[0]; tv[4][2 * p + 1] = t4[1]; tv[5][2 * p] = t5[0]; tv[5][2 * p + 1] = t5[1];
    };
    const int wr_off = srow * 64 + ((schunk ^ ((srow >> 2) & 3)) << 4);
    auto write_A = [&](char* stage, int x) {
        if (ABL & 2) return;
        *reinterpret_cast<f32x4*>(stage + x * (F_BM * 64) + wr_off) = tv[x];
    };
    int st_r = 0, st_cib = F_BK, st_tn = tbeg % tilesN;
    const unsigned vsub = VPL ? (unsigned)(vp.rows * 64) : 0u;
    const unsigned vxs = vsub * (unsigned)(Cin >> 4);
    const unsigned long long vpa = (unsigned long long)vp.p;
    const u32x4f vr = {(unsigned)vpa, (unsigned)(vpa >> 32) & 0xFFFFu, 6u * vxs, 0x00020000u};
    unsigned vso = 0;
    auto advance_staged = [&]() {
        st_cib += F_BK;
        const int w1 = st_cib >= Cin;
        st_cib = w1 ? 0 : st_cib;
        st_r += w1;
        const int w2 = st_r == 3;
        st_r = w2 ? 0 : st_r;
        st_tn = w2 ? (st_tn + tstride) % tilesN : st_tn;
    };
    auto store_V = [&](int x) {
        if (!VPL) return;
asm volatile("buffer_store_dwordx4 %0, %1, %2, %3 offen nt" : : "v"(tv[x]), "v"(vpo), "s"(vr), "s"(vso + (unsigned)x * vxs) : "memory");
    };
    const int swr = (((srow >> 2) & 1) << 1) | ((srow >> 3) & 1);
    const int wr_h1 = srow * 64 + (((schunk >> 1) ^ swr) << 4) + (schunk & 1) * 8;
    const int wr_h2 = srow * 64 + (((2 + (schunk >> 1)) ^ swr) << 4) + (schunk & 1) * 8;
    auto split_A = [&](char* stage, int x) {
        if (ABL & 2) return;
        const unsigned sb = __builtin_bit_cast(unsigned, sA[x]);
        const unsigned long long sc2 = ((unsigned long long)sb << 32) | sb;
        f32x2v vlo = {tv[x][0], tv[x][1]}, vhi = {tv[x][2], tv[x][3]};
        asm("v_pk_mul_f32 %0, %1, %2" : "=v"(vlo) : "v"(vlo), "s"(sc2));
        asm("v_pk_mul_f32 %0, %1, %2" : "=v"(vhi) : "v"(vhi), "s"(sc2));
        const f32x4 v = {vlo[0], vlo[1], vhi[0], vhi[1]};
        if (ABL & 32) {
            typedef unsigned u32x2q __attribute__((ext_vector_type(2)));
            const u32x2q a = {(__builtin_bit_cast(unsigned, v[0]) >> 16) | (__builtin_bit_cast(unsigned, v[1]) & 0xFFFF0000u),
                              (__builtin_bit_cast(unsigned, v[2]) >> 16) | (__builtin_bit_cast(unsigned, v[3]) & 0xFFFF0000u)};
            *reinterpret_cast<u32x2q*>(stage + x * (F_BM * 64) + wr_h1) = a;
            *reinterpret_cast<u32x2q*>(stage + x * (F_BM * 64) + wr_h2) = a;
            return;
        }
        const f16x4 h1 = __builtin_convertvector(v, f16x4);
        typedef unsigned u32x2h __attribute__((ext_vector_type(2)));
        const u32x2h hp = __builtin_bit_cast(u32x2h, h1);
        f32x4 r;
        asm("v_fma_mix_f32 %0, %1, -1.0, %2 op_sel_hi:[1,0,0]" : "=v"(r[0]) : "v"(hp[0]), "v"(v[0]));
        asm("v_fma_mix_f32 %0, %1, -1.0, %2 op_sel:[1,0,0] op_sel_hi:[1,0,0]" : "=v"(r[1]) : "v"(hp[0]), "v"(v[1]));
        asm("v_fma_mix_f32 %0, %1, -1.0, %2 op_sel_hi:[1,0,0]" : "=v"(r[2]) : "v"(hp[1]), "v"(v[2]));
        asm("v_fma_mix_f32 %0, %1, -1.0, %2 op_sel:[1,0,0] op_sel_hi:[1,0,0]" : "=v"(r[3]) : "v"(hp[1]), "v"(v[3]));
        const f16x4 h2 = __builtin_convertvector(r, f16x4);
        if (ABL & 64) {
            asm volatile("" :: "v"(h1), "v"(h2));
            return;
        }
        *reinterpret_cast<f16x4*>(stage + x * (F_BM * 64) + wr_h1) = h1;
        *reinterpret_cast<f16x4*>(stage + x * (F_BM * 64) + wr_h2) = h2;
    };
    auto store_A = [&](char* stage, int set) {
        xform2(set, 0);
        xform2(set, 1);
#pragma unroll
        for (int x = 0; x < 6; ++x) { if (H2) split_A(stage, x); else write_A(stage, x); }
    };
    int btn = tbeg % tilesN, bslice = 0, bleft = total;
    const unsigned bvoff = (unsigned)(wave * 3 * 1024 + lane * 16);
    const char* bsrc = nullptr;
    auto dma_B_begin = [&]() {
        bsrc = reinterpret_cast<const char*>(Uf) + (size_t)(bslice * tilesN + btn) * F_BBYTES;
        if (--bleft > 0) {
            const int w = ++bslice == nS;
            bslice = w ? 0 : bslice;
            btn = w ? (btn + tstride) % tilesN : btn;
        }
    };
    auto dma_B_piece = [&](unsigned stage_addr, int q) {
        if (!(ABL & 4)) f_dma16(bsrc + q * 1024, bvoff, stage_addr + F_ABYTES + (wave * 3 + q) * 1024);
    };

    f32x16 acc[6];
#pragma unroll
    for (int x = 0; x < 6; ++x)
#pragma unroll
        for (int e = 0; e < 16; ++e) acc[x][e] = 0.f;

    const int sw = (li >> 2) & 3;
    const int a_off = (wm * 32 + li) * 64 + ((lh ^ sw) << 4);
    const int b_off = F_ABYTES + (wn * 32 + li) * 64 + ((lh ^ sw) << 4);
    f32x4 fa[2], fb[2];
    auto load_frag = [&](const char* st, int sidx, int slot) {
        const int x = sidx >> 1, kk = sidx & 1;
        fa[slot] = *reinterpret_cast<const f32x4*>(st + ((x * (F_BM * 64) + a_off) ^ (kk << 5)));
        fb[slot] = *reinterpret_cast<const f32x4*>(st + ((x * (F_BN * 64) + b_off) ^ (kk << 5)));
    };
    auto mfma1 = [&](int k) {
        if (ABL & 16) return;
        const int sidx = k >> 2, x = sidx >> 1, slot = sidx & 1, j = k & 3;
        acc[x] = __builtin_amdgcn_mfma_f32_32x32x2f32(fa[slot][j], fb[slot][j], acc[x], 0, 0, 0);
    };

    f16x8 ha1[2], hb1[2], ha2, hb2;
    const int swl = (li >> 2) & 3;
    const int swa = (((li >> 2) & 1) << 1) | ((li >> 3) & 1);
    const int ha_row = (wm * 32 + li) * 64, hb_row = F_ABYTES + (wn * 32 + li) * 64;
    auto load_h1 = [&](const char* st, int x, int slot) {
        ha1[slot] = *reinterpret_cast<const f16x8*>(st + x * (F_BM * 64) + ha_row + ((lh ^ swa) << 4));
        hb1[slot] = *reinterpret_cast<const f16x8*>(st + x * (F_BN * 64) + hb_row + ((lh ^ swl) << 4));
    };
    auto load_ha2 = [&](const char* st, int x) { ha2 = *reinterpret_cast<const f16x8*>(st + x * (F_BM * 64) + ha_row + (((2 + lh) ^ swa) << 4)); };
    auto load_hb2 = [&](const char* st, int x) { hb2 = *reinterpret_cast<const f16x8*>(st + x * (F_BN * 64) + hb_row + (((2 + lh) ^ swl) << 4)); };
    auto mfma_h = [&](int k) {
        if (ABL & 16) return;
        const int x = k / 3, p = k - 3 * x, slot = x & 1;
        if (p == 0) acc[x] = __builtin_amdgcn_mfma_f32_32x32x16_f16(ha1[slot], hb1[slot], acc[x], 0, 0, 0);
        else if (p == 1) acc[x] = __builtin_amdgcn_mfma_f32_32x32x16_f16(ha2, hb1[slot], acc[x], 0, 0, 0);
        else acc[x] = __builtin_amdgcn_mfma_f32_32x32x16_f16(ha1[slot], hb2, acc[x], 0, 0, 0);
    };

    auto epilogue = [&](int tile) {
        if (ABL & 8) {
            if (tile == -1) {
                float z = 0.f;
#pragma unroll
                for (int x = 0; x < 6; ++x)
#pragma unroll
                    for (int e = 0; e < 16; ++e) z += acc[x][e];
                Y[tid] = z;
            }
            return;
        }
        const int mt = tile / tilesN, tn = tile - mt * tilesN;
        const int m0 = mt * F_BM;
        const int col = tn * F_BN + wn * 32 + li;
        const bool cok = col < Cout;
        const float bs = CL ? cst[col & (F_CMAX - 1)] : ((bias != nullptr && cok) ? bias[col] : 0.f);
        const int qb = (int)divWt.div((unsigned)m0);
        const int pixb = qb * W + 4 * (m0 - qb * Wt);
        const size_t ybytes = ((size_t)Mpix - pixb) * ldy * 4;
        const __amdgpu_buffer_rsrc_t yr = __builtin_amdgcn_make_buffer_rsrc((void*)(Y + (size_t)pixb * ldy), 0,
                                                                            (int)(ybytes < 0x7FFFFFFFu ? ybytes : 0x7FFFFFFFu), 0x00020000);
        const unsigned ls = (unsigned)ldy * 4u;
        float s1 = 0.f, s2 = 0.f;
        __amdgpu_buffer_rsrc_t pr = null_rsrc;
        float bsc = 0.f, bsh = 0.f, bmu = 0.f;
        if (BNR) {
            pr = __builtin_amdgcn_make_buffer_rsrc((void*)(bn.y + (size_t)pixb * ldy), 0,
                                                   (int)(ybytes < 0x7FFFFFFFu ? ybytes : 0x7FFFFFFFu), 0x00020000);
            if (CL) { bsc = cst[F_CMAX + (col & (F_CMAX - 1))]; bsh = cst[2 * F_CMAX + (col & (F_CMAX - 1))]; bmu = cst[3 * F_CMAX + (col & (F_CMAX - 1))]; }
            else if (cok) { bsc = bn.scale[col]; bsh = bn.shift[col]; bmu = bn.mean[col]; }
        }
        auto bnacc = [&](float q, float v) {
            const float g = fmaf(q, bsc, bsh) > 0.f ? v : 0.f;
            s1 += g;
            s2 = fmaf(g, q - bmu, s2);
        };
        if ((W & 3) == 0 && m0 + F_BM <= Mt && (tn + 1) * F_BN <= Cout) {
            const unsigned ob = (unsigned)((4 * (wm * 32 + 4 * lh)) * ldy + col) * 4u;
#pragma unroll
            for (int e = 0; e < 16; ++e) {
                const float m0_ = H2 ? acc[0][e] * un[0].a * un[0].b : acc[0][e], m1 = H2 ? acc[1][e] * un[1].a * un[1].b : acc[1][e],
                            m2 = H2 ? acc[2][e] * un[2].a * un[2].b : acc[2][e], m3 = H2 ? acc[3][e] * un[3].a * un[3].b : acc[3][e],
                            m4 = H2 ? acc[4][e] * un[4].a * un[4].b : acc[4][e], m5 = H2 ? acc[5][e] * un[5].a * un[5].b : acc[5][e];
                const float s12 = m1 + m2, d12 = m1 - m2, s34 = m3 + m4, d34 = m3 - m4;
                const float y0 = m0_ + s12 + s34, y1 = fmaf(2.f, d34, d12), y2 = fmaf(4.f, s34, s12), y3 = fmaf(8.f, d34, d12) + m5;
#pragma unroll
                for (int x = 0; x < 6; ++x) acc[x][e] = 0.f;
                const unsigned so = (unsigned)(4 * ((e & 3) + 8 * (e >> 2))) * ls;
                __builtin_amdgcn_raw_buffer_store_b32(__builtin_bit_cast(unsigned, y0 + bs), yr, ob, so, 0);
                __builtin_amdgcn_raw_buffer_store_b32(__builtin_bit_cast(unsigned, y1 + bs), yr, ob, so + ls, 0);
                __builtin_amdgcn_raw_buffer_store_b32(__builtin_bit_cast(unsigned, y2 + bs), yr, ob, so + 2 * ls, 0);
                __builtin_amdgcn_raw_buffer_store_b32(__builtin_bit_cast(unsigned, y3 + bs), yr, ob, so + 3 * ls, 0);
                if (STATS) {
                    s1 += (y0 + y1) + (y2 + y3);
                    s2 += fmaf(y0, y0, y1 * y1) + fmaf(y2, y2, y3 * y3);
                }
                if (BNR) {
                    const float q0 = __builtin_bit_cast(float, __builtin_amdgcn_raw_buffer_load_b32(pr, ob, so, 0));
                    const float q1 = __builtin_bit_cast(float, __builtin_amdgcn_raw_buffer_load_b32(pr, ob, so + ls, 0));
                    const float q2 = __builtin_bit_cast(float, __builtin_amdgcn_raw_buffer_load_b32(pr, ob, so + 2 * ls, 0));
                    const float q3 = __builtin_bit_cast(float, __builtin_amdgcn_raw_buffer_load_b32(pr, ob, so + 3 * ls, 0));
                    bnacc(q0, y0 + bs); bnacc(q1, y1 + bs); bnacc(q2, y2 + bs); bnacc(q3, y3 + bs);
                }
            }
        } else {
#pragma unroll
            for (int e = 0; e < 16; ++e) {
                const int t = m0 + wm * 32 + (e & 3) + 8 * (e >> 2) + 4 * lh;
                const float m0_ = H2 ? acc[0][e] * un[0].a * un[0].b : acc[0][e], m1 = H2 ? acc[1][e] * un[1].a * un[1].b : acc[1][e],
                            m2 = H2 ? acc[2][e] * un[2].a * un[2].b : acc[2][e], m3 = H2 ? acc[3][e] * un[3].a * un[3].b : acc[3][e],
                            m4 = H2 ? acc[4][e] * un[4].a * un[4].b : acc[4][e], m5 = H2 ? acc[5][e] * un[5].a * un[5].b : acc[5][e];
                const float s12 = m1 + m2, d12 = m1 - m2, s34 = m3 + m4, d34 = m3 - m4;
                const float y0 = m0_ + s12 + s34, y1 = fmaf(2.f, d34, d12), y2 = fmaf(4.f, s34, s12), y3 = fmaf(8.f, d34, d12) + m5;
#pragma unroll
                for (int x = 0; x < 6; ++x) acc[x][e] = 0.f;
                const int q = (int)divWt.div((unsigned)t), xt = t - q * Wt;
                const int nv = (t < Mt && cok) ? W - 4 * xt : 0;
                const unsigned o = (unsigned)((q * W + 4 * xt - pixb) * ldy + col) * 4u;
                __builtin_amdgcn_raw_buffer_store_b32(__builtin_bit_cast(unsigned, y0 + bs), yr, oob_unless(nv > 0, o), 0, 0);
                __builtin_amdgcn_raw_buffer_store_b32(__builtin_bit_cast(unsigned, y1 + bs), yr, oob_unless(nv > 1, o), ls, 0);
                __builtin_amdgcn_raw_buffer_store_b32(__builtin_bit_cast(unsigned, y2 + bs), yr, oob_unless(nv > 2, o), 2 * ls, 0);
                __builtin_amdgcn_raw_buffer_store_b32(__builtin_bit_cast(unsigned, y3 + bs), yr, oob_unless(nv > 3, o), 3 * ls, 0);
                if (STATS) {
                    const float z0 = nv > 0 ? y0 : 0.f, z1 = nv > 1 ? y1 : 0.f, z2 = nv > 2 ? y2 : 0.f, z3 = nv > 3 ? y3 : 0.f;
                    s1 += (z0 + z1) + (z2 + z3);
                    s2 += fmaf(z0, z0, z1 * z1) + fmaf(z2, z2, z3 * z3);
                }
                if (BNR) {
                    const float q0 = __builtin_bit_cast(float, __builtin_amdgcn_raw_buffer_load_b32(pr, oob_unless(nv > 0, o), 0, 0));
                    const float q1 = __builtin_bit_cast(float, __builtin_amdgcn_raw_buffer_load_b32(pr, oob_unless(nv > 1, o), ls, 0));
                    const float q2 = __builtin_bit_cast(float, __builtin_amdgcn_raw_buffer_load_b32(pr, oob_unless(nv > 2, o), 2 * ls, 0));
                    const float q3 = __builtin_bit_cast(float, __builtin_amdgcn_raw_buffer_load_b32(pr, oob_unless(nv > 3, o), 3 * ls, 0));
                    bnacc(q0, nv > 0 ? y0 + bs : 0.f); bnacc(q1, nv > 1 ? y1 + bs : 0.f);
                    bnacc(q2, nv > 2 ? y2 + bs : 0.f); bnacc(q3, nv > 3 ? y3 + bs : 0.f);
                }
            }
        }
        if (BNR) {
            s1 += __shfl_xor(s1, 32, 64);
            s2 += __shfl_xor(s2, 32, 64);
            if (lh == 0) {
                red[wm * 64 + wn * 32 + li] = s1;
                red[256 + wm * 64 + wn * 32 + li] = s2;
            }
            __syncthreads();
            if (tid < 64) {
                const int c = tn * F_BN + tid;
                if (c < Cout) {
                    const float a = (red[tid] + red[64 + tid]) + (red[128 + tid] + red[192 + tid]);
                    const float b = (red[256 + tid] + red[320 + tid]) + (red[384 + tid] + red[448 + tid]);
                    stats[(size_t)mt * Cout + c] = a;
                    stats[(size_t)(P + mt) * Cout + c] = b * (CL ? cst[4 * F_CMAX + c] : bn.rstd[c]);
                }
            }
        }
        if (STATS) {
            s1 += __shfl_xor(s1, 32, 64);
            s2 += __shfl_xor(s2, 32, 64);
            if (lh == 0) {
                red[wm * 64 + wn * 32 + li] = s1;
                red[256 + wm * 64 + wn * 32 + li] = s2;
            }
            __syncthreads();
            if (tid < 64) {
                const int c = tn * F_BN + tid;
                if (c < Cout) {
                    const int mend = min(Mt, m0 + F_BM);
                    const int nlast = (int)divWt.div((unsigned)mend) - qb;
                    const float cnt = (float)(4 * (mend - m0) - nlast * (4 * Wt - W));
                    const float a = (red[tid] + red[64 + tid]) + (red[128 + tid] + red[192 + tid]);
                    const float b = (red[256 + tid] + red[320 + tid]) + (red[384 + tid] + red[448 + tid]);
                    const float m2 = b - a * a / cnt;
                    const float bc = CL ? cst[c] : (bias != nullptr ? bias[c] : 0.f);
                    stats[(size_t)mt * Cout + c] = a + cnt * bc;
                    stats[(size_t)(P + mt) * Cout + c] = m2 > 0.f ? m2 : 0.f;
                    if (tid == 0 && tn == 0) counts[mt] = cnt;
                }
            }
        }
    };

    char* const buf0 = smem;
    char* const buf1 = smem + F_STAGE;
    issue_A(0);
    issue_A(1);
    dma_B_begin();
#pragma unroll
    for (int q = 0; q < 3; ++q) dma_B_piece(smem_addr, q);
    store_A(buf0, 0);
    issue_A(0);
    cvk_wait_vm<6>();
    cvk_lds_retire_barrier();

#define F_SB() __builtin_amdgcn_sched_barrier(0)
    auto step = [&](auto par_, const char* cur, char* nxt, unsigned nxt_addr) {
        constexpr int SET = 1 - decltype(par_)::value;
        const bool VST = VPL && st_r == 1 && st_tn == 0;
        if (VPL) vso = (unsigned)(st_cib >> 4) * vsub;
        if (lcib == 0) {
            if (lr == 0 && ltile < tend) set_tile(ltile);
            regroup(lr);
        }
        dma_B_begin();
        load_frag(cur, 0, 0);
        F_SB();
        f_static_for(std::make_integer_sequence<int, 48>{}, [&](auto kc_) {
            constexpr int k_ = decltype(kc_)::value;
            constexpr int q_ = k_;
            mfma1(k_);
            if constexpr ((k_ & 3) == 0) {
                if constexpr (k_ < 44) load_frag(cur, (k_ >> 2) + 1, ((k_ >> 2) + 1) & 1);
            } else if constexpr (q_ == 1) {
                xform2(SET, 0);
            } else if constexpr (q_ == 2) {
                xform2(SET, 1);
                dma_B_piece(nxt_addr, 0);
            } else if constexpr (q_ == 3) {
                dma_B_piece(nxt_addr, 1);
            } else if constexpr (q_ == 5) {
                dma_B_piece(nxt_addr, 2);
            } else if constexpr (q_ == 6 || q_ == 7) {
                write_A(nxt, q_ - 6);
                if (VST) store_V(q_ - 6);
                load_A(SET, q_ - 6);
            } else if constexpr (q_ >= 9 && q_ <= 11) {
                write_A(nxt, q_ - 7);
                if (VST) store_V(q_ - 7);
                load_A(SET, q_ - 7);
            } else if constexpr (q_ == 13) {
                write_A(nxt, 5);
                if (VST) store_V(5);
                load_A(SET, 5);
                advance_A();
            }
            F_SB();
        });
        if (VST) cvk_wait_vm<12>(); else cvk_wait_vm<6>();
        cvk_lds_retire_barrier();
        if (VPL) advance_staged();
    };
    auto step_h = [&](auto par_, const char* cur, char* nxt, unsigned nxt_addr) {
        constexpr int SET = 1 - decltype(par_)::value;
        if (lcib == 0) {
            if (lr == 0 && ltile < tend) set_tile(ltile);
            regroup(lr);
        }
        dma_B_begin();
        load_h1(cur, 0, 0);
        load_ha2(cur, 0);
        load_hb2(cur, 0);
        F_SB();
        f_static_for(std::make_integer_sequence<int, 18>{}, [&](auto kc_) {
            constexpr int k_ = decltype(kc_)::value;
            mfma_h(k_);
            if constexpr (k_ < 15) {
                if constexpr (k_ % 3 == 0) load_h1(cur, k_ / 3 + 1, (k_ / 3 + 1) & 1);
                else if constexpr (k_ % 3 == 1) load_ha2(cur, k_ / 3 + 1);
                else load_hb2(cur, k_ / 3 + 1);
            }
            if constexpr (k_ % 3 == 0) {
            } else if constexpr (k_ == 1) {
                xform2(SET, 0);
            } else if constexpr (k_ == 2) {
                xform2(SET, 1);
                dma_B_piece(nxt_addr, 0);
            } else if constexpr (k_ == 4) {
                dma_B_piece(nxt_addr, 1);
            } else if constexpr (k_ == 5) {
                dma_B_piece(nxt_addr, 2);
            } else if constexpr (k_ == 7 || k_ == 10 || k_ == 13) {
                split_A(nxt, 2 * ((k_ - 7) / 3));
                split_A(nxt, 2 * ((k_ - 7) / 3) + 1);
            } else if constexpr (k_ == 8 || k_ == 11) {
                load_A(SET, 2 * ((k_ - 8) / 3));
                load_A(SET, 2 * ((k_ - 8) / 3) + 1);
            } else if constexpr (k_ == 14) {
                load_A(SET, 4);
                load_A(SET, 5);
                advance_A();
            }
            F_SB();
        });
        cvk_wait_vm<6>();
        cvk_lds_retire_barrier();
    };
    for (int tile = tbeg; tile < tend; tile += tstride) {
        for (int ks = 0; ks < nS; ks += 2) {
            if (H2) {
                step_h(std::integral_constant<int, 0>{}, buf0, buf1, smem_addr + F_STAGE);
                step_h(std::integral_constant<int, 1>{}, buf1, buf0, smem_addr);
            } else {
                step(std::integral_constant<int, 0>{}, buf0, buf1, smem_addr + F_STAGE);
                step(std::integral_constant<int, 1>{}, buf1, buf0, smem_addr);
            }
        }
        epilogue(tile);
    }
#undef F_SB
    cvk_wait_vm<0>();
}

}

static inline int f_tiles_n(int Cn) { return cvk_cdiv(Cn, F_BN); }

extern "C" size_t cvk_wino4f_weight_floats(int Cn, int Ck) {
    if (Cn <= 0 || Ck <= 0 || Ck % F_BK) return 0;
    return (size_t)(3 * Ck / F_BK) * f_tiles_n(Cn) * 6 * F_BN * F_BK;
}

extern "C" int cvk_wino4f_weight_transform(const float* w, float* Uf, int Cn, int Ck, int dgrad, void* stream) {
    CVK_CHECK_ARG(w && Uf && Cn > 0 && Ck > 0, "cvk_wino4f_weight_transform: bad arguments");
    CVK_CHECK_ARG(Ck % F_BK == 0, "cvk_wino4f_weight_transform: the contraction channel count %d must be a multiple of 16", Ck);
    CVK_CHECK_ARG(cvk_aligned16(Uf), "cvk_wino4f_weight_transform: Uf must be 16-byte aligned");
    const size_t total = (size_t)f_tiles_n(Cn) * F_BN * 3 * Ck;
    const int blocks = (int)((total + 255) / 256 < 8192 ? (total + 255) / 256 : 8192);
    hipLaunchKernelGGL(k_wino4f_weight, dim3(blocks), dim3(256), 0, (hipStream_t)stream, w, Uf, Cn, Ck, f_tiles_n(Cn), dgrad ? 1 : 0);
    CVK_LAUNCH_RETURN("cvk_wino4f_weight_transform");
}

extern "C" int cvk_wino4f_weight_transform_batch(const cvk_wt_job* jobs, int n, void* stream) {
    CVK_CHECK_ARG(jobs && n > 0 && n <= CVK_WT_BATCH_MAX, "cvk_wino4f_weight_transform_batch: 1..%d jobs", CVK_WT_BATCH_MAX);
    F4WJobsDev d;
    unsigned nb = 0;
    for (int i = 0; i < n; ++i) {
        const cvk_wt_job& q = jobs[i];
        CVK_CHECK_ARG(q.w && q.out && q.rows > 0 && q.cols > 0 && q.cols % F_BK == 0 && cvk_aligned16(q.out), "cvk_wino4f_weight_transform_batch: bad job %d", i);
        d.w[i] = q.w; d.out[i] = q.out; d.Cn[i] = q.rows; d.Ck[i] = q.cols; d.dgrad[i] = q.dgrad ? 1 : 0;
        const size_t total = (size_t)f_tiles_n(q.rows) * F_BN * 3 * q.cols;
        d.first[i] = nb;
        nb += (unsigned)((total + 255) / 256 < 2048 ? (total + 255) / 256 : 2048);
    }
    d.first[n] = nb; d.n = n;
    hipLaunchKernelGGL(k_wino4f_weight_batch, dim3(nb), dim3(256), 0, (hipStream_t)stream, d);
    CVK_LAUNCH_RETURN("cvk_wino4f_weight_transform_batch");
}

extern "C" int cvk_wino4f_stat_partials(int N, int H, int W) {
    if (N <= 0 || H <= 0 || W <= 0) return 0;
    return cvk_cdiv((long)N * H * ((W + 3) / 4), F_BM);
}

static int wino4f_launch(const char* who, const float* x, const float* Uf, const float* bias, float* y, float* stats, float* counts,
                         const FBnRed* bn, int N, int H, int W, int Cin, int Cout, int ldy, int max_workgroups, void* stream,
                         const void* amax_x = nullptr, const void* amax_w = nullptr, float* vplanes = nullptr) {
    CVK_CHECK_ARG(x && Uf && y, "%s: null pointer", who);
    CVK_CHECK_ARG(N > 0 && H > 0 && W > 0 && Cout > 0 && ldy >= Cout, "%s: bad shape", who);
    CVK_CHECK_ARG(Cin >= 32 && Cin % 32 == 0, "%s: Cin=%d must be a multiple of 32", who, Cin);
    CVK_CHECK_ARG((stats == nullptr) == (counts == nullptr) || bn, "%s: stats and counts go together", who);
    CVK_CHECK_ARG(cvk_aligned16(x) && cvk_aligned16(Uf), "%s: x and Uf must be 16-byte aligned", who);
    CVK_CHECK_ARG((long)N * H * W < (1L << 31) - 512, "%s: tensor too large for 32-bit pixel indices", who);
    const int Wt = (W + 3) / 4, Mt = N * H * Wt, Mpix = N * H * W;
    CVK_CHECK_ARG((long)Mt * Wt < (1L << 32) && (long)N * H * H < (1L << 32), "%s: frame too large for the multiply-high coordinate split", who);
    const int tilesN = f_tiles_n(Cout), tilesM = cvk_cdiv(Mt, F_BM), ntiles = tilesM * tilesN;
    static int cus = 0;
    if (cus == 0) {
        int dev = 0, v = 0;
        if (hipGetDevice(&dev) == hipSuccess && hipDeviceGetAttribute(&v, hipDeviceAttributeMultiprocessorCount, dev) == hipSuccess && v > 0) cus = v;
        else cus = 256;
    }
    const int wgs = (max_workgroups > 0 && max_workgroups < cus) ? max_workgroups : cus;
    const int grid = ntiles < wgs ? ntiles : wgs;
    CVK_CHECK_ARG((F_BM * 4 + 3L * W + 8) * Cin * 4 < (1L << 31), "%s: a tile's input window exceeds the 2 GiB buffer-addressing limit", who);
    hipStream_t s = (hipStream_t)stream;
    const FBnRed none = {nullptr, nullptr, nullptr, nullptr, nullptr};
    const bool h2 = amax_x != nullptr;
    CVK_CHECK_ARG((amax_x == nullptr) == (amax_w == nullptr), "%s: the two amax blocks go together", who);
    FSplit sp = {(const unsigned*)amax_x, (const unsigned*)amax_w, CvkSplitTab{}, CvkSplitTab{}};
    if (h2) { sp.tabB = cvk_split_tab(4, CVK_SPLIT_KIND_B); sp.tabG = cvk_split_tab(4, CVK_SPLIT_KIND_G); }
    FVpl vp = {nullptr, 0, 0};
    if (vplanes) {
        CVK_CHECK_ARG(!bn && !h2 && cvk_aligned16(vplanes), "%s: V planes go with plain fp32 forward launches", who);
        vp.Wtp = (Wt + 7) / 8 * 8;
        vp.rows = (long)N * (H + 2) * vp.Wtp + 2L * vp.Wtp;
        vp.p = vplanes;
        CVK_CHECK_ARG(6L * Cin * vp.rows * 4 < (1L << 32) - 4096, "%s: V planes of %ld rows x %d channels exceed the 4 GiB addressing limit", who, vp.rows, Cin);
    }
    const bool cl = Cout <= F_CMAX;
    CVK_CHECK_ARG(!vplanes || cl, "%s: the plane-writing launch needs Cout <= %d", who, F_CMAX);
#define CVK_W4F_GO(ST_, BN_, H2_, CL_, BNV_) hipLaunchKernelGGL((k_conv3x3_wino4f<ST_, 0, BN_, H2_, false, CL_>), dim3(grid), dim3(512), 0, s, x, Uf, bias, y, \
                                                                stats, counts, Mt, H, W, Wt, Cin, Cout, ldy, tilesN, ntiles, Mpix, tilesM, BNV_, sp, vp)
#define CVK_W4F_GO2(ST_, BN_, BNV_) do { if (cl) CVK_W4F_GO(ST_, BN_, false, true, BNV_); else CVK_W4F_GO(ST_, BN_, false, false, BNV_); } while (0)
#define CVK_W4F_GOV(ST_) hipLaunchKernelGGL((k_conv3x3_wino4f<ST_, 0, false, false, true, true>), dim3(grid), dim3(512), 0, s, x, Uf, bias, y, stats, counts, \
                                            Mt, H, W, Wt, Cin, Cout, ldy, tilesN, ntiles, Mpix, tilesM, none, sp, vp)
    if (vplanes)    { if (stats) CVK_W4F_GOV(true); else CVK_W4F_GOV(false); }
    else if (bn)    { if (h2) CVK_W4F_GO(false, true, true, false, *bn); else CVK_W4F_GO2(false, true, *bn); }
    else if (stats) { if (h2) CVK_W4F_GO(true, false, true, false, none); else CVK_W4F_GO2(true, false, none); }
    else            { if (h2) CVK_W4F_GO(false, false, true, false, none); else CVK_W4F_GO2(false, false, none); }
#undef CVK_W4F_GO
#undef CVK_W4F_GO2
#undef CVK_W4F_GOV
    CVK_LAUNCH_RETURN(who);
}

extern "C" int cvk_conv3x3_wino4f(const float* x, const float* Uf, const float* bias, float* y, float* stats, float* counts, int N,
                                  int H, int W, int Cin, int Cout, int ldy, int max_workgroups, void* stream) {
    return wino4f_launch("cvk_conv3x3_wino4f", x, Uf, bias, y, stats, counts, nullptr, N, H, W, Cin, Cout, ldy, max_workgroups, stream);
}

extern "C" int cvk_conv3x3_wino4f_vplanes(const float* x, const float* Uf, const float* bias, float* y, float* stats, float* counts, float* Vsm,
                                          int N, int H, int W, int Cin, int Cout, int ldy, int max_workgroups, void* stream) {
    CVK_CHECK_ARG(Vsm, "cvk_conv3x3_wino4f_vplanes: null plane pointer");
    return wino4f_launch("cvk_conv3x3_wino4f_vplanes", x, Uf, bias, y, stats, counts, nullptr, N, H, W, Cin, Cout, ldy, max_workgroups, stream,
                         nullptr, nullptr, Vsm);
}

extern "C" int cvk_conv3x3_wino4f_bnred(const float* x, const float* Uf, float* y, int N, int H, int W, int Cin, int Cout, int ldy,
                                        const float* yP, const float* scale, const float* shift, const float* mean,
                                        const float* rstd, float* part, int max_workgroups, void* stream) {
    CVK_CHECK_ARG(yP && scale && shift && mean && rstd && part, "cvk_conv3x3_wino4f_bnred: null pointer");
    const FBnRed bn = {yP, scale, shift, mean, rstd};
    return wino4f_launch("cvk_conv3x3_wino4f_bnred", x, Uf, nullptr, y, part, nullptr, &bn, N, H, W, Cin, Cout, ldy, max_workgroups, stream);
}

extern "C" int cvk_wino4h_weight_transform(const float* w, void* Uh, const void* amax_w, int Cn, int Ck, int dgrad, void* stream) {
    CVK_CHECK_ARG(w && Uh && amax_w && Cn > 0 && Ck > 0, "cvk_wino4h_weight_transform: bad arguments");
    CVK_CHECK_ARG(Ck % F_BK == 0, "cvk_wino4h_weight_transform: the contraction channel count %d must be a multiple of 16", Ck);
    CVK_CHECK_ARG(cvk_aligned16(Uh), "cvk_wino4h_weight_transform: Uh must be 16-byte aligned");
    const size_t total = (size_t)f_tiles_n(Cn) * F_BN * 3 * Ck;
    const int blocks = (int)((total + 255) / 256 < 8192 ? (total + 255) / 256 : 8192);
    hipLaunchKernelGGL(k_wino4h_weight, dim3(blocks), dim3(256), 0, (hipStream_t)stream, w, (float*)Uh, Cn, Ck, f_tiles_n(Cn), dgrad ? 1 : 0,
                       (const unsigned*)amax_w, cvk_split_tab(4, CVK_SPLIT_KIND_G));
    CVK_LAUNCH_RETURN("cvk_wino4h_weight_transform");
}
extern "C" int cvk_conv3x3_wino4h(const float* x, const void* Uh, const float* bias, float* y, float* stats, float* counts, const void* amax_x,
                                  const void* amax_w, int N, int H, int W, int Cin, int Cout, int ldy, int max_workgroups, void* stream) {
    CVK_CHECK_ARG(amax_x && amax_w, "cvk_conv3x3_wino4h: null amax block");
    return wino4f_launch("cvk_conv3x3_wino4h", x, (const float*)Uh, bias, y, stats, counts, nullptr, N, H, W, Cin, Cout, ldy, max_workgroups, stream,
                         amax_x, amax_w);
}
extern "C" int cvk_conv3x3_wino4h_bnred(const float* x, const void* Uh, float* y, const void* amax_x, const void* amax_w, int N, int H, int W, int Cin,
                                        int Cout, int ldy, const float* yP, const float* scale, const float* shift, const float* mean,
                                        const float* rstd, float* part, int max_workgroups, void* stream) {
    CVK_CHECK_ARG(yP && scale && shift && mean && rstd && part && amax_x && amax_w, "cvk_conv3x3_wino4h_bnred: null pointer");
    const FBnRed bn = {yP, scale, shift, mean, rstd};
    return wino4f_launch("cvk_conv3x3_wino4h_bnred", x, (const float*)Uh, nullptr, y, part, nullptr, &bn, N, H, W, Cin, Cout, ldy, max_workgroups, stream,
                         amax_x, amax_w);
}

#ifdef CVK_WINO4F_ABLATE
extern "C" int cvk_conv3x3_wino4f_ablate(const float* x, const float* Uf, const float* bias, float* y, int N, int H, int W, int Cin,
                                         int Cout, int ldy, int abl, void* stream) {
    const int Wt = (W + 3) / 4, Mt = N * H * Wt, Mpix = N * H * W;
    const int tilesN = f_tiles_n(Cout), tilesM = cvk_cdiv(Mt, F_BM), ntiles = tilesM * tilesN;
    const int grid = ntiles < 256 ? ntiles : 256;
    hipStream_t s = (hipStream_t)stream;
#define CVK_ABL(A) case A: hipLaunchKernelGGL((k_conv3x3_wino4f<false, A>), dim3(grid), dim3(512), 0, s, x, Uf, bias, y, nullptr, nullptr, Mt, H, W, Wt, Cin, Cout, ldy, tilesN, ntiles, Mpix, tilesM, FBnRed{nullptr, nullptr, nullptr, nullptr, nullptr}, FSplit{nullptr, nullptr, CvkSplitTab{}, CvkSplitTab{}}, FVpl{nullptr, 0, 0}); break;
    switch (abl) {
        CVK_ABL(0) CVK_ABL(1) CVK_ABL(2) CVK_ABL(3) CVK_ABL(4) CVK_ABL(7) CVK_ABL(8) CVK_ABL(9) CVK_ABL(11) CVK_ABL(15) CVK_ABL(16) CVK_ABL(24) CVK_ABL(31)
        default: return -1;
    }
#undef CVK_ABL
    CVK_LAUNCH_RETURN("cvk_conv3x3_wino4f_ablate");
}
extern "C" int cvk_conv3x3_wino4h_ablate(const float* x, const void* Uh, const float* bias, float* y, const void* amax_x, const void* amax_w, int N,
                                         int H, int W, int Cin, int Cout, int ldy, int abl, void* stream) {
    const int Wt = (W + 3) / 4, Mt = N * H * Wt, Mpix = N * H * W;
    const int tilesN = f_tiles_n(Cout), tilesM = cvk_cdiv(Mt, F_BM), ntiles = tilesM * tilesN;
    const int grid = ntiles < 256 ? ntiles : 256;
    hipStream_t s = (hipStream_t)stream;
    const FSplit sp = {(const unsigned*)amax_x, (const unsigned*)amax_w, cvk_split_tab(4, CVK_SPLIT_KIND_B), cvk_split_tab(4, CVK_SPLIT_KIND_G)};
#define CVK_ABLH(A) case A: hipLaunchKernelGGL((k_conv3x3_wino4f<false, A, false, true>), dim3(grid), dim3(512), 0, s, x, (const float*)Uh, bias, y, nullptr, nullptr, Mt, H, W, Wt, Cin, Cout, ldy, tilesN, ntiles, Mpix, tilesM, FBnRed{nullptr, nullptr, nullptr, nullptr, nullptr}, sp, FVpl{nullptr, 0, 0}); break;
    switch (abl) {
        CVK_ABLH(0) CVK_ABLH(1) CVK_ABLH(2) CVK_ABLH(4) CVK_ABLH(8) CVK_ABLH(9) CVK_ABLH(11) CVK_ABLH(15) CVK_ABLH(16) CVK_ABLH(31) CVK_ABLH(32) CVK_ABLH(33) CVK_ABLH(64) CVK_ABLH(65)
        default: return -1;
    }
#undef CVK_ABLH
    CVK_LAUNCH_RETURN("cvk_conv3x3_wino4h_ablate");
}
#endif
```

pytorch-camvid_amd/engine.py:

```python
import ctypes
import os
from collections import namedtuple

import torch

from . import _lib
from ._lib import View, ViewH, check
from .route import conv_route, pad4, split_fmt
from .route import layer_tile, wgrad2d_pays, wino2d_ok, wino2d_pays, wino4_pays

_F32, _BF16 = torch.float32, torch.bfloat16


class ActBuf:
    __slots__ = ("id", "N", "H", "W", "C", "ld", "name", "dtype")

    def __init__(self, id_, N, H, W, C, name="", dtype=_F32):
        self.id, self.N, self.H, self.W, self.C, self.name, self.dtype = id_, N, H, W, C, name, dtype
        self.ld = pad4(C) if dtype == _F32 else max(32, (C + 7) // 8 * 8)

    @property
    def esize(self):
        return 4 if self.dtype == _F32 else 2

    @property
    def M(self):
        return self.N * self.H * self.W

    def full_view(self):
        return BufView(self, 0, self.C, 0, 0, self.H, self.W)

    def __repr__(self):
        return f"ActBuf({self.name}#{self.id} {self.N}x{self.H}x{self.W}x{self.C}/{self.ld})"


class BufView:
    __slots__ = ("buf", "c0", "C", "y0", "x0", "H", "W")

    def __init__(self, buf, c0, C, y0, x0, H, W):
        assert 0 <= c0 and c0 + C <= buf.ld and 0 <= y0 and y0 + H <= buf.H and 0 <= x0 and x0 + W <= buf.W
        self.buf, self.c0, self.C, self.y0, self.x0, self.H, self.W = buf, c0, C, y0, x0, H, W

    def cview(self, tensor):
        b = self.buf
        ptr = tensor.data_ptr() + 4 * ((self.y0 * b.W + self.x0) * b.ld + self.c0)
        return View(ptr, b.H * b.W * b.ld, b.W * b.ld, b.ld)

    def hview(self, tensor):
        b = self.buf
        ptr = tensor.data_ptr() + b.esize * ((self.y0 * b.W + self.x0) * b.ld + self.c0)
        return ViewH(ptr, b.H * b.W * b.ld, b.W * b.ld, b.ld)

    @property
    def is_full(self):
        b = self.buf
        return self.c0 == 0 and self.C == b.C and self.y0 == 0 and self.x0 == 0 and self.H == b.H and self.W == b.W


class RunState:

    def __init__(self, params, training, need_grad):
        self.params = params
        self.training = training
        self.need_grad = need_grad
        self.act = {}
        self.saved = {}
        self.routes = None
        self.grad = {}
        self.gflat = None
        self.stream = None
        self.sync = None
        self.pooled_by_block = {}
        self.colsums = []
        self.wreduces = []
        self.pass_token = 0
        self.bnred = {}
        self.amax = {}
        self.amax_spare = []
        self.scratch = []
        self.fold = None


def _empty(n, dev, dtype=_F32):
    return torch.empty(n, device=dev, dtype=dtype)


def channels_last(w):
    return w if w.is_contiguous(memory_format=torch.channels_last) else w.contiguous(memory_format=torch.channels_last)


class Saved(namedtuple("Saved", "y bnp rt kept", defaults=(None, None))):
    def pointers(self, ld):
        pb = self.bnp.data_ptr()
        return self.y.data_ptr(), pb + 8 * ld, pb + 12 * ld, pb, pb + 4 * ld


WINO_DEFAULT = os.environ.get("CVK_WINO", "1") != "0"
WINO4_DEFAULT = {"0": False, "1": True, "always": "always"}[os.environ.get("CVK_WINO4", "1")]
WINO2D_DEFAULT = {"0": False, "1": True, "always": "always"}[os.environ.get("CVK_WINO2D", "1")]
W2TILE_DEFAULT = {"auto": None, "4": 4, "6": 6}[os.environ.get("CVK_W2D_TILE", "auto")]
WINO4F_DEFAULT = os.environ.get("CVK_WINO4F", "1") != "0"
WGRADP_DEFAULT = {"0": False, "1": True, "always": "always"}[os.environ.get("CVK_WGRADP", "1")]
VPLANES_DEFAULT = os.environ.get("CVK_VPLANES", "1") != "0"


def amax_blocks(lib, n, dev):
    nw = lib.cvk_amax_block_words()
    t = torch.zeros(n * nw, device=dev, dtype=torch.int32)
    return [t[i * nw:(i + 1) * nw] for i in range(n)]


WEIGHT_EPOCH = [0]
WCACHE_DEFAULT = os.environ.get("CVK_WEIGHT_CACHE", "1") != "0"


def _bump_epoch(*_a, **_k):
    WEIGHT_EPOCH[0] += 1


try:
    from torch.optim.optimizer import register_optimizer_step_post_hook as _reg_opt_hook
    _reg_opt_hook(_bump_epoch)
except ImportError:
    WCACHE_DEFAULT = False


def mark_weights_dirty(module):
    from .modules import runner_of
    runner_of(module).wepoch += 1


PROF = None
PROF_OPS = None
_CUR_OP = [None]


def _timed(R, name, work, fn, unit="flop", executed=None, nbytes=None):
    if PROF is None:
        return fn()
    e0, e1 = torch.cuda.Event(enable_timing=True), torch.cuda.Event(enable_timing=True)
    e0.record()
    r = fn()
    e1.record()
    PROF.append((name, work, e0, e1, unit, executed, nbytes))
    if PROF_OPS is not None:
        PROF_OPS.append(_CUR_OP[0])
    return r


class Op:
    idx = -1

    def fwd(self, R, st):
        raise NotImplementedError

    def bwd(self, R, st):
        pass


class MaxPool(Op):

    def __init__(self, src_view, dst_buf, keep_code):
        self.src, self.dst, self.keep_code = src_view, dst_buf, keep_code
        self.fused = False
        self.producer_idx = -1
        self.wants = True
        if src_view.H < 2 or src_view.W < 2:
            raise RuntimeError(f"max_pool2d: input {src_view.H}x{src_view.W} is too small for a 2x2 window")

    def fwd(self, R, st):
        v, d = self.src, self.dst
        X = st.act[v.buf.id]
        if st.plan.bf16:
            if not self.fused:
                raise NotImplementedError("bf16 mode: a max pool must directly follow a conv block (it is fused into its BN pass)")
            return
        if self.fused and st.pooled_by_block.get(self.producer_idx, False):
            return
        out = R.alloc_act(st, d, X.device)
        code = None
        if self.keep_code:
            code = torch.empty(d.M * d.ld, device=X.device, dtype=torch.uint8)
            st.saved[self.idx] = code
        _timed(R, "k_maxpool_fwd", 5.0 * v.buf.N * v.H * v.W * v.C, lambda: check(
            R.lib.cvk_maxpool2x2_fwd(v.cview(X), out.data_ptr(), code.data_ptr() if code is not None else None,
                                     v.buf.N, v.H, v.W, v.C, st.stream), "cvk_maxpool2x2_fwd"), "byte")

    def bwd(self, R, st):
        v, d = self.src, self.dst
        if not self.wants or d.id not in st.grad:
            st.grad.pop(d.id, None)
            return
        X = st.act[v.buf.id]
        acc = v.buf.id in st.grad
        if not acc:
            if not v.is_full:
                st.grad[v.buf.id] = torch.zeros_like(X)
            else:
                st.grad[v.buf.id] = torch.empty_like(X)
        prod = st.plan.ops[self.producer_idx] if (self.fused and self.producer_idx >= 0) else None
        fuse_sums = (prod is not None and st.training and R.pool_bnred and isinstance(prod, ConvBnRelu) and prod.bn_train and prod.idx in st.saved
                     and prod.idx not in st.bnred and prod.dst.buf is v.buf
                     and (prod.dst.c0, prod.dst.C, prod.dst.y0, prod.dst.x0, prod.dst.H, prod.dst.W) == (v.c0, v.C, v.y0, v.x0, v.H, v.W)
                     and prod.cout == v.C and st.plan.last_gradient_writer(v, prod.idx) == self.idx)
        if st.plan.bf16:
            PBp = R.lib.cvk_maxpool2x2_bwd_bnred_blocks_bf16(v.buf.N, v.H, v.W, v.C) if fuse_sums else 0
            if PBp > 0:
                py, *pbn = st.saved[prod.idx].pointers(v.C)
                part = _empty(2 * PBp * v.C, X.device)
                rc = _timed(R, "k_pool_bwd_bf16(+bnred)", (2.0 * 0.25 + 2.0 + (4.0 if acc else 2.0) + 2.0) * v.buf.N * v.H * v.W * v.C,
                            lambda: R.lib.cvk_maxpool2x2_bwd_bnred_bf16(
                                st.grad[d.id].data_ptr(), v.hview(X), v.hview(st.grad[v.buf.id]), 1 if acc else 0, v.buf.N, v.H, v.W, v.C,
                                py, v.C, *pbn, part.data_ptr(), st.stream), "byte")
                if rc == 0:
                    st.bnred[prod.idx] = (part, PBp)
                    st.grad.pop(d.id)
                    return
            _timed(R, "k_pool_bwd_bf16", (2.0 * 0.25 + 2.0 + (4.0 if acc else 2.0)) * v.buf.N * v.H * v.W * v.C, lambda: check(
                R.lib.cvk_maxpool2x2_bwd_bf16(st.grad[d.id].data_ptr(), v.hview(X), v.hview(st.grad[v.buf.id]), 1 if acc else 0,
                                              v.buf.N, v.H, v.W, v.C, st.stream), "cvk_maxpool2x2_bwd_bf16"), "byte")
            st.grad.pop(d.id)
            return
        code = st.saved.get(self.idx)
        if fuse_sums and pad4(prod.cout) == prod.cout:
            PBp = R.lib.cvk_maxpool2x2_bwd_bnred_blocks(v.buf.N, v.H, v.W, v.C)
            if PBp > 0:
                ldp = pad4(prod.cout)
                py, *pbn = st.saved[prod.idx].pointers(ldp)
                part = _empty(2 * PBp * v.C, X.device)
                rc = _timed(R, "k_pool_scatter(bwd+bnred)", (1.0 + (0.25 if code is not None else 4.0) + (8.0 if acc else 4.0) + 4.0) * v.buf.N * v.H * v.W * v.C,
                            lambda: R.lib.cvk_maxpool2x2_bwd_bnred(
                                st.grad[d.id].data_ptr(), v.cview(X), code.data_ptr() if code is not None else None, v.cview(st.grad[v.buf.id]),
                                1 if acc else 0, v.buf.N, v.H, v.W, v.C, py, ldp, *pbn, part.data_ptr(), st.stream), "byte")
                if rc == 0:
                    st.bnred[prod.idx] = (part, PBp)
                    st.grad.pop(d.id)
                    return
        _timed(R, "k_pool_scatter(bwd)", (1.0 + (0.25 if code is not None else 4.0) + (8.0 if acc else 4.0)) * v.buf.N * v.H * v.W * v.C, lambda: check(
            R.lib.cvk_maxpool2x2_bwd(st.grad[d.id].data_ptr(), v.cview(X), code.data_ptr() if code is not None else None,
                                     v.cview(st.grad[v.buf.id]), 1 if acc else 0, v.buf.N, v.H, v.W, v.C, st.stream),
            "cvk_maxpool2x2_bwd"), "byte")
        st.grad.pop(d.id)


class Unpool(Op):

    def __init__(self, src_buf, pool_op, dst_buf):
        self.src, self.pool, self.dst = src_buf, pool_op, dst_buf
        self.wants = True

    def fwd(self, R, st):
        V = st.act[self.src.id]
        d = self.dst
        out = R.alloc_act(st, d, V.device)
        if st.plan.bf16:
            pv = self.pool.src
# ... 96 lines not shown
        self.routes = {}
        self.input = self.new_buf(cin, H, W, "input")
        self.output = None
        self.input_needs_grad = False

    def new_buf(self, C, H, W, name="", f32=False):
        b = ActBuf(len(self.bufs), self.N, H, W, C, name, _BF16 if (self.bf16 and not f32) else _F32)
        self.bufs.append(b)
        return b

    def add(self, op):
        op.idx = len(self.ops)
        self.ops.append(op)
        return op

    def _reads(self, buf):
        self._readers[buf.id] = self._readers.get(buf.id, 0) + 1

    def _writes(self, buf, c0, C, op):
        self._writers.setdefault(buf.id, []).append((c0, C, op))

    def _needs_grad(self, buf, c0=0, C=None):
        if buf is self.input:
            return bool(self.input_needs_grad)
        C = buf.C if C is None else C
        for w0, wC, op in self._writers.get(buf.id, ()):
            if w0 < c0 + C and c0 < w0 + wC and (op.active if isinstance(op, ConvBnRelu) else op.wants):
                return True
        return False

    def last_gradient_writer(self, view, producer_idx):
        for op in self.ops[producer_idx + 1:]:
            s = getattr(op, "src", None)
            if s is None:
                continue
            if isinstance(s, BufView):
                if s.buf is view.buf and s.c0 < view.c0 + view.C and view.c0 < s.c0 + s.C:
                    return op.idx
            elif s is view.buf:
                return op.idx
        return -1

    def sole_producer(self, buf):
        op = self._producer.get((buf.id, 0))
        if op is None or not op.dst.is_full or op.dst.buf is not buf or self._readers.get(buf.id, 0) != 1 or self.output is None \
                or self.output.buf is buf:
            return None
        return op

    def conv_bn_relu(self, src_buf, holder, dst_view=None):
        cin, cout = holder.in_channels, holder.out_channels
        if src_buf.C != cin:
            raise RuntimeError(f"Given groups=1, weight of size [{cout}, {cin}, 3, 3], expected input[{src_buf.N}, {src_buf.C}, "
                               f"{src_buf.H}, {src_buf.W}] to have {cin} channels, but got {src_buf.C} channels instead")
        if dst_view is None:
            dst_view = self.new_buf(cout, src_buf.H, src_buf.W, holder.tag).full_view()
        pslot = len(self.holders)
        self.holders.append(holder)
        conv, bn = holder.conv_bn()
        req = (conv.weight.requires_grad, conv.bias is not None and conv.bias.requires_grad, bn.weight is not None and bn.weight.requires_grad,
               bn.bias is not None and bn.bias.requires_grad)
        needs = self._needs_grad(src_buf)
        self._reads(src_buf)
        op = self.add((ConvBnReluBf16 if self.bf16 else ConvBnRelu)(src_buf, dst_view, pslot, holder, cin, cout, needs, bn.training, req))
        self.convs.append(op)
        self._producer[(dst_view.buf.id, dst_view.c0)] = op
        self._writes(dst_view.buf, dst_view.c0, dst_view.C, op)
        return dst_view

    def maxpool(self, src_view, keep_code=False):
        dst = self.new_buf(src_view.C, src_view.H // 2, src_view.W // 2, "pool")
        self._reads(src_view.buf)
        op = self.add(MaxPool(src_view, dst, keep_code))
        op.wants = self._needs_grad(src_view.buf, src_view.c0, src_view.C)
        self._writes(dst, 0, dst.C, op)
        prod = self._producer.get((src_view.buf.id, src_view.c0))
        if prod is not None and prod.dst.C == src_view.C and prod.pool_dst is None \
                and prod.dst.H == src_view.H and prod.dst.W == src_view.W and prod.dst.y0 == src_view.y0 and prod.dst.x0 == src_view.x0:
            prod.pool_dst = dst
            prod.pool_op = op
            op.fused = True
            op.producer_idx = prod.idx
        return op

    def unpool(self, src_buf, pool_op):
        v = pool_op.src
        dst = self.new_buf(v.C, v.H, v.W, "unpool")
        self._reads(src_buf)
        op = self.add(Unpool(src_buf, pool_op, dst))
        op.wants = self._needs_grad(src_buf)
        self._writes(dst, 0, dst.C, op)
        return dst

    def upsample(self, src_buf):
        dst = self.new_buf(src_buf.C, 2 * src_buf.H, 2 * src_buf.W, "up")
        self._reads(src_buf)
        op = self.add(Upsample(src_buf, dst))
        op.wants = self._needs_grad(src_buf)
        self._writes(dst, 0, dst.C, op)
        return dst

    def zero_frame(self, view):
        self.add(ZeroFrame(view))

    def seal(self, thin=True):
        if self.bf16:
            b = self.output.buf
            if not self.output.is_full:
                raise NotImplementedError("bf16 mode: the network output must be a whole buffer")
            b.dtype = _F32
            b.ld = pad4(b.C)
            readers = [op for op in self.ops if getattr(op, "src", None) is self.input]
            if (thin and not self.input_needs_grad and self.input.C <= 4 and readers and self.input is not self.output.buf
                    and all(isinstance(op, ConvBnRelu) and op.cout == 64 for op in readers)
                    and self.input.H * self.input.W * 64 * 2 < 2 ** 31):
                self.input.ld = 8


_SPLIT_ENV_LOGGED = False


def _split_mode_from_env():
    global _SPLIT_ENV_LOGGED
    raw = os.environ.get("CVK_W2D_SPLIT")
    if raw is None:
        return 0
    modes = {"0": 0, "1": 3, "3": 3, "2": 2}
    if raw.strip() not in modes:
        raise ValueError(f"CVK_W2D_SPLIT={raw!r}: allowed values are 0 (off, the default), 2 (two fp16 terms) and 3 or 1 (three bf16 terms); "
                         "or leave it unset and call pytorch_camvid_amd.set_split_operands(net, mode)")
    mode = modes[raw.strip()]
    if mode and not _SPLIT_ENV_LOGGED:
        _SPLIT_ENV_LOGGED = True
        import sys
        print(f"pytorch_camvid_amd: CVK_W2D_SPLIT={raw} — fp32 convolution products run as split {'fp16 x 2' if mode == 2 else 'bf16 x 3'} operands "
              "(opt-in, not the exact-fp32 default)", file=sys.stderr)
    return mode


class Runner:

    def __init__(self):
        self.lib = _lib.load()
        self._ws = None
        self._dp_wgs = None
        self._collectives_in_flight = False
        self.grad_sync = None
        self.accumulator = None
        self.wino = WINO_DEFAULT
        self.wino4 = WINO4_DEFAULT
        self.wino4f = WINO4F_DEFAULT
        self.wgradp = WGRADP_DEFAULT
        self.vplanes = VPLANES_DEFAULT
        self.thin = os.environ.get("CVK_THIN", "1") != "0"
        self.pool_bnred = os.environ.get("CVK_POOL_BNRED", "1") != "0"
        self.wino2d = WINO2D_DEFAULT
        self.w2d_split = _split_mode_from_env()
        self.w2tile_cfg = W2TILE_DEFAULT
        self.w2tile = 6
        self.w2tile_dgrad = 6
        self.bf16 = False
        self.wcache = WCACHE_DEFAULT
        self.wepoch = 0
        self._wc = {}
        self._wjobs, self._wjobs_cfg = {}, None
        self._pass_token = 0
        self._passes = 0
        self.wcache_builds = 0

    def persistent_wgs(self):
        gs = self.grad_sync
        if gs is None or (getattr(gs, "world", 1) <= 1 and not getattr(gs, "always_issue", False)):
            return 0
        if self._dp_wgs is None:
            cus = torch.cuda.get_device_properties(torch.cuda.current_device()).multi_processor_count
            self._dp_wgs = max(8, cus - int(os.environ.get("CVK_DP_RESERVE_CUS", "8")))
        return self._dp_wgs

    def launch_wgs(self):
        return self.persistent_wgs() if self._collectives_in_flight else 0

    def derived(self, key, src, build, job=None):
        if not self.wcache or key is None or torch.cuda.is_current_stream_capturing():
            self.wcache_builds += 1
            return build()
        if job is not None:
            self._wjobs[key] = (src, job)
        return self._cache(key, src, build)

    def _cache(self, key, src, build=None):
        sig = (WEIGHT_EPOCH[0], self.wepoch, src.data_ptr(), src._version, self._pass_token)
        ent = self._wc.get(key)
        if (ent is None or ent[0] != sig) and build is not None:
            ent = self._wc[key] = (sig, build())
            self.wcache_builds += 1
        return ent[1] if ent is not None and ent[0] == sig else None

    def prebuild_fp32(self, plan, st, need_grad):
        if not self.wcache or torch.cuda.is_current_stream_capturing():
            return
        cfg = (id(plan),) + self.kernel_config()
        if cfg != self._wjobs_cfg:
            self._wjobs, self._wjobs_cfg = {}, cfg
            return
        live = {p.data_ptr() for p in st.params}
        lib, fam_jobs = self.lib, {"w4f": [], "w2d": []}
        for key, (src, (fam, floats, rows, cols, tile, dgrad)) in self._wjobs.items():
            if src.data_ptr() not in live or (dgrad and not need_grad):
                continue
            if self._cache(key, src) is not None:
                continue
            t = self._cache(key, src, lambda: _empty(floats, src.device))
            fam_jobs[fam].append((_lib.WtJob(src.data_ptr(), t.data_ptr(), rows, cols, tile, dgrad), 4.0 * (src.numel() + floats)))
        for fam, fn in (("w4f", lib.cvk_wino4f_weight_transform_batch), ("w2d", lib.cvk_w2d_weight_transform_batch)):
            jobs = fam_jobs[fam]
            for i in range(0, len(jobs), _lib.WT_BATCH_MAX):
                chunk = jobs[i:i + _lib.WT_BATCH_MAX]
                arr = (_lib.WtJob * len(chunk))(*[j for j, _ in chunk])
                _timed(self, "k_weight_transform_batch", sum(b for _, b in chunk),
                       lambda: check(fn(ctypes.addressof(arr), len(chunk), st.stream), "cvk_%s_weight_transform_batch" % fam), "byte")

    def prepack_bf16(self, plan, st, need_grad):
        if not self.wcache or torch.cuda.is_current_stream_capturing():
            return
        lib, jobs, keep = self.lib, [], []
        for op in plan.ops:
            if not isinstance(op, ConvBnRelu):
                continue
            w = st.params[4 * op.pslot]
            for key, dgrad, rows, kpad in op.packs_wanted(self, need_grad):
                if self._cache(key, w) is not None:
                    continue
                wc = channels_last(w)
                t = self._cache(key, w, lambda: torch.empty(lib.cvk_bf16s_rows_pad(rows) * 9 * kpad, device=w.device, dtype=_BF16))
                jobs.append(_lib.PackJob(wc.data_ptr(), t.data_ptr(), op.cout, op.cin, kpad, dgrad))
                keep.append(wc)
        for i in range(0, len(jobs), _lib.PACK_BATCH_MAX):
            chunk = jobs[i:i + _lib.PACK_BATCH_MAX]
            arr = (_lib.PackJob * len(chunk))(*chunk)
            check(lib.cvk_pack_weights_bf16_batch(ctypes.addressof(arr), len(chunk), st.stream), "cvk_pack_weights_bf16_batch")

    def workspace(self, nbytes, dev):
        if self._ws is None or self._ws.numel() < nbytes or self._ws.device != dev:
            self._ws = torch.empty(max(nbytes, 1 << 20), device=dev, dtype=torch.uint8)
        return self._ws

    def alloc_act(self, st, buf, dev):
        t = st.act.get(buf.id)
        if t is None:
            shape = (buf.N, buf.H, buf.W, buf.ld)
            t = torch.zeros(shape, device=dev, dtype=buf.dtype) if buf.ld != buf.C else torch.empty(shape, device=dev, dtype=buf.dtype)
            st.act[buf.id] = t
        return t

    def grad_ptrs(self, st, slot):
        base = st.gflat.data_ptr()
        return tuple(base + 4 * st.goffs[4 * slot + j] for j in range(4))

    def defer_colsum(self, st, part, PB, C, out_ptr):
        st.colsums.append((part, PB, C, out_ptr))
        if len(st.colsums) >= _lib.COLSUM_BATCH_MAX:
            self.flush_colsums(st)

    def defer_wreduce(self, st, slab, splits, n, dw_ptr):
        st.wreduces.append((slab, splits, n, dw_ptr))
        if len(st.wreduces) >= _lib.WREDUCE_BATCH_MAX:
            self.flush_wreduces(st)

    def flush_wreduces(self, st):
        if not st.wreduces:
            return
        arr = (_lib.WReduceJob * len(st.wreduces))(*[_lib.WReduceJob(sl.data_ptr(), dw, n, sp, 0) for sl, sp, n, dw in st.wreduces])
        check(self.lib.cvk_wgrad_reduce_bf16s_batch(ctypes.addressof(arr), len(st.wreduces), st.stream), "cvk_wgrad_reduce_bf16s_batch")
        st.wreduces.clear()

    def flush_colsums(self, st):
        if not st.colsums:
            return
        arr = (_lib.ColsumJob * len(st.colsums))(*[_lib.ColsumJob(p.data_ptr(), o, pb, c) for p, pb, c, o in st.colsums])
        check(self.lib.cvk_colsum_finalize_batch(ctypes.addressof(arr), len(st.colsums), st.stream), "cvk_colsum_finalize_batch")
        st.colsums.clear()

    def grads_ready(self, st, slot):
        if st.sync is not None and st.plan.convs[slot].trainable:
            if st.sync.closes_bucket():
                self.flush_colsums(st)
                self.flush_wreduces(st)
            st.sync.layer_done(st, slot)
            self._collectives_in_flight = st.sync.in_flight()

    def begin_sync(self, st, plan, fold=None):
        gs = self.grad_sync
        if gs is None:
            return None
        if not gs.enabled or (fold is not None and not fold.closing):
            gs.launched = []
            return None
        return gs.begin(st, plan)

    def import_nchw(self, st, x, buf, dtype, zero_pad=False):
        xp = x.permute(0, 2, 3, 1)
        if dtype == _F32 and buf.ld == buf.C and xp.is_contiguous():
            return xp
        t = (torch.zeros if zero_pad and buf.ld != buf.C else torch.empty)((buf.N, buf.H, buf.W, buf.ld), device=x.device, dtype=dtype)
        fn = "cvk_import_nchw_bf16" if dtype == _BF16 else "cvk_import_nchw"
        check(getattr(self.lib, fn)(x.data_ptr(), *x.stride(), t.data_ptr(), buf.ld, buf.N, buf.C, buf.H, buf.W, st.stream), fn)
        return t

    def plan_amax(self, plan, st):
        if split_fmt(self) != 2 or plan.bf16 or not (st.training and st.need_grad):
            return
        routes = self.routes(plan, True, True)
        layers = [op for op in plan.ops if isinstance(op, ConvBnRelu) and (routes[op.idx].split or (op.src.ld % 32 == 0 and op.cout % 4 == 0))]
        if not layers:
            return

        def writers(buf):
            out = []
            for op in plan.ops:
                if isinstance(op, ConvBnRelu) and (op.dst.buf is buf or (op.pool_dst is buf and op.cout % 4 == 0)):
                    out.append(op)
                elif isinstance(op, (MaxPool, Unpool, Upsample)) and op.dst is buf and not (isinstance(op, MaxPool) and op.fused):
                    out.append(op)
                elif isinstance(op, ZeroFrame) and op.view.buf is buf:
                    out.append(op)
            return out

        want, ok = [], {}

        def fusable(buf):
            if buf.id in ok:
                return ok[buf.id]
            ok[buf.id] = False
            ws = writers(buf)
            good = bool(ws) and buf is not plan.input
            for op in ws:
                if isinstance(op, Upsample):
                    good = good and fusable(op.src)
                elif not isinstance(op, (ConvBnRelu, ZeroFrame)):
                    good = False
            ok[buf.id] = good
            if good:
                want.append(buf)
            return good
        for op in layers:
            fusable(op.src)
        blocks = amax_blocks(self.lib, len(want) + len(layers), st.device)
        for i, buf in enumerate(want):
            st.amax[buf.id] = blocks[i]
        st.amax_spare = blocks[len(want):]

    def kernel_config(self):
        return (self.wino, self.wino4, self.wino4f, self.wino2d, self.wgradp, self.vplanes, self.thin, self.pool_bnred, self.w2d_split,
                self.w2tile_cfg)

    def routes(self, plan, training, need_grad):
        key = (self.kernel_config(), training, need_grad)
        r = plan.routes.get(key)
        if r is None:
            if split_fmt(self):
                check_bn_modes(plan, training, "set_split_operands")
            self.w2tile, self.w2tile_dgrad = self.tile_for(plan)
            r = plan.routes[key] = {op.idx: conv_route(self, op, training, need_grad) for op in plan.ops if isinstance(op, ConvBnRelu)}
        return r

    def tile_for(self, plan):
        if self.w2tile_cfg in (4, 6):
            return self.w2tile_cfg, self.w2tile_cfg
        return (4, 6) if any(isinstance(op, Unpool) for op in plan.ops) else (6, 6)

    def forward(self, plan, x, params, training, need_grad):
        dev = x.device
        self._collectives_in_flight = False
        st = RunState(params, training, need_grad)
        st.device = dev
        st.plan = plan
        if training and need_grad:
            self._passes += 1
            st.pass_token = self._passes
        self._pass_token = st.pass_token
        st.stream = torch.cuda.current_stream(dev).cuda_stream
        st.act[plan.input.id] = self.import_nchw(st, x, plan.input, _BF16 if plan.bf16 else _F32)
        if plan.bf16:
            check_bn_modes(plan, training, "bf16 mode", need_grad, forward_only_ok=True)
            self.prepack_bf16(plan, st, need_grad)
        else:
            st.routes = self.routes(plan, training, need_grad)
            self.prebuild_fp32(plan, st, need_grad)
            self.plan_amax(plan, st)
        for op in plan.ops:
            _CUR_OP[0] = (op.idx, "fwd")
            op.fwd(self, st)
        _CUR_OP[0] = None
        ov = plan.output
        out = st.act[ov.buf.id][..., :ov.buf.C].permute(0, 3, 1, 2)
        if not need_grad:
            st.act.clear()
            st.saved.clear()
        return out, st

    def backward(self, plan, st, gout):
        dev = gout.device
        st.stream = torch.cuda.current_stream(dev).cuda_stream
        self._pass_token = st.pass_token
        params = st.params
        st.goffs, total = layout_grads(params)
        st.gflat = torch.empty(total, device=dev, dtype=_F32)
        fold = st.fold = self.accumulator.open_pass(st, plan, total) if self.accumulator is not None else None
        st.sync = self.begin_sync(st, plan, fold)
        self._collectives_in_flight = False
        st.grad[plan.output.buf.id] = self.import_nchw(st, gout, plan.output.buf, _F32, zero_pad=True)
        for op in reversed(plan.ops):
            _CUR_OP[0] = (op.idx, "bwd")
            op.bwd(self, st)
        _CUR_OP[0] = None
        self.flush_colsums(st)
        self.flush_wreduces(st)
        if fold is not None and st.sync is None:
            fold.whole(st)
        dx = None
        if plan.input_needs_grad:
            gi = st.grad[plan.input.id]
            dx = gi[..., :plan.input.C].permute(0, 3, 1, 2)
            if plan.bf16:
                dx = dx.float()
        grads = []
        hand_out = fold is None or fold.closing
        for i, p in enumerate(params):
            op = plan.convs[i // 4]
            if not hand_out or not (op.w_req, op.b_req, op.g_req, op.be_req)[i % 4]:
                grads.append(None)
                continue
            n = p.numel()
            seg = st.gflat[st.goffs[i]:st.goffs[i] + n]
            if p.dim() == 4:
                co, ci, kh, kw = p.shape
                seg = seg.view(co, kh, kw, ci).permute(0, 3, 1, 2)
            else:
                seg = seg.view(p.shape)
            grads.append(seg)
        if st.sync is not None:
            st.sync.finish(st)
        self._collectives_in_flight = False
        st.act.clear(); st.saved.clear(); st.grad.clear(); st.scratch.clear()
        if fold is not None:
            fold.done()
            st.fold = None
            if not hand_out:
                st.gflat = None
        return dx, grads


def check_bn_modes(plan, training, what, need_grad=True, forward_only_ok=False):
    for op in plan.convs:
        if forward_only_ok and not (need_grad and op.active):
            continue
        if op.bn_train != bool(training):
            raise NotImplementedError(f"{what}: BatchNorm of {op.label} is in {'training' if op.bn_train else 'eval'} mode inside a "
                                      f"{'training' if training else 'eval'} pass; per-block BatchNorm modes run in the fp32 mode only")


def layout_grads(params):
    offs = [0] * len(params)
    o = 0
    for slot in range(len(params) // 4 - 1, -1, -1):
        for j in range(4):
            i = 4 * slot + j
            offs[i] = o
            o += (params[i].numel() + 3) // 4 * 4
    return offs, o


class _PlanFunction(torch.autograd.Function):

    @staticmethod
    def forward(ctx, runner, plan, training, x, *params):
        out, st = runner.forward(plan, x, params, training, True)
        ctx.runner, ctx.plan, ctx.st = runner, plan, st
        return out

    @staticmethod
    def backward(ctx, gout):
        st = ctx.st
        if st is None:
            raise RuntimeError("Trying to backward through the plan a second time (activations were already freed)")
        ctx.st = None
        dx, grads = ctx.runner.backward(ctx.plan, st, gout)
        return (None, None, None, dx, *grads)


def run_plan(runner, plan, training, x, params):
    need = torch.is_grad_enabled() and (x.requires_grad or any(p.requires_grad for p in params))
    if not need:
        out, _ = runner.forward(plan, x, params, training, False)
        return out
    return _PlanFunction.apply(runner, plan, training, x, *params)


from .conv_fp32 import ConvBnRelu, conv_kernel_name
from .conv_bf16 import ConvBnReluBf16
```

Baseline: 247.7 images/s.

## Split leftover wino4f tiles across workgroups along K with slab reduction

Adds a tail-split mode to the persistent fused Winograd F(4,3) conv kernel. When the tile count per XCD does not divide evenly among its workgroups, the remainder tiles are split along the reduction dimension into 2-4 parts. Each part writes partial pre-transform products to workspace slabs, and a counter lets the last part finish the epilogue. This targets the idle-workgroup imbalance in the final wave, at the cost of a zeroing launch, a workspace, and extra slab traffic and synchronisation.

```diff
diff --git a/include/cvk.h b/include/cvk.h
--- a/include/cvk.h
+++ b/include/cvk.h
@@ -140,6 +140,16 @@
 int cvk_conv3x3_wino4f_bnred(const float* x, const float* Uf, float* y, int N, int H, int W, int Cin, int Cout, int ldy,
                              const float* yP, const float* scale, const float* shift, const float* mean, const float* rstd,
                              float* part, int max_workgroups, void* stream);
+size_t cvk_wino4f_tail_workspace_bytes(int N, int H, int W, int Cin, int Cout, int max_workgroups);
+int cvk_wino4f_tail_plan(int ntiles, int grid, int Cin, int* xcds, int* items, int max_items);
+int cvk_conv3x3_wino4f_ts(const float* x, const float* Uf, const float* bias, float* y, float* stats, float* counts, int N, int H, int W,
+                          int Cin, int Cout, int ldy, int max_workgroups, void* workspace, size_t workspace_bytes, int tail_split, void* stream);
+int cvk_conv3x3_wino4f_vplanes_ts(const float* x, const float* Uf, const float* bias, float* y, float* stats, float* counts, float* Vsm,
+                                  int N, int H, int W, int Cin, int Cout, int ldy, int max_workgroups, void* workspace,
+                                  size_t workspace_bytes, int tail_split, void* stream);
+int cvk_conv3x3_wino4f_bnred_ts(const float* x, const float* Uf, float* y, int N, int H, int W, int Cin, int Cout, int ldy,
+                                const float* yP, const float* scale, const float* shift, const float* mean, const float* rstd,
+                                float* part, int max_workgroups, void* workspace, size_t workspace_bytes, int tail_split, void* stream);
 
 int cvk_thin_fwd_supported(int Cin_ld, int Cout, int ldy);
 int cvk_thin_stat_partials(int N, int H, int W, int Cin_ld);
diff --git a/pytorch-camvid_amd/_lib.py b/pytorch-camvid_amd/_lib.py
--- a/pytorch-camvid_amd/_lib.py
+++ b/pytorch-camvid_amd/_lib.py
@@ -56,6 +56,13 @@
     "cvk_conv3x3_wino4f": (c_int, [c_vp, c_vp, c_vp, c_vp, c_vp, c_vp, c_int, c_int, c_int, c_int, c_int, c_int, c_int, c_vp]),
     "cvk_conv3x3_wino4f_bnred": (c_int, [c_vp, c_vp, c_vp, c_int, c_int, c_int, c_int, c_int, c_int, c_vp, c_vp, c_vp, c_vp, c_vp, c_vp, c_int, c_vp]),
     "cvk_wino4h_weight_transform": (c_int, [c_vp, c_vp, c_vp, c_int, c_int, c_int, c_vp]),
+    "cvk_wino4f_tail_workspace_bytes": (c_size, [c_int, c_int, c_int, c_int, c_int, c_int]),
+    "cvk_wino4f_tail_plan": (c_int, [c_int, c_int, c_int, c_vp, c_vp, c_int]),
+    "cvk_conv3x3_wino4f_ts": (c_int, [c_vp, c_vp, c_vp, c_vp, c_vp, c_vp, c_int, c_int, c_int, c_int, c_int, c_int, c_int, c_vp, c_size, c_int, c_vp]),
+    "cvk_conv3x3_wino4f_vplanes_ts": (c_int, [c_vp, c_vp, c_vp, c_vp, c_vp, c_vp, c_vp, c_int, c_int, c_int, c_int, c_int, c_int, c_int, c_vp, c_size,
+                                              c_int, c_vp]),
+    "cvk_conv3x3_wino4f_bnred_ts": (c_int, [c_vp, c_vp, c_vp, c_int, c_int, c_int, c_int, c_int, c_int, c_vp, c_vp, c_vp, c_vp, c_vp, c_vp, c_int, c_vp,
+                                            c_size, c_int, c_vp]),
     "cvk_conv3x3_wino4h": (c_int, [c_vp, c_vp, c_vp, c_vp, c_vp, c_vp, c_vp, c_vp, c_int, c_int, c_int, c_int, c_int, c_int, c_int, c_vp]),
     "cvk_conv3x3_wino4h_bnred": (c_int, [c_vp, c_vp, c_vp, c_vp, c_vp, c_int, c_int, c_int, c_int, c_int, c_int, c_vp, c_vp, c_vp, c_vp, c_vp, c_vp,
                                          c_int, c_vp]),
diff --git a/pytorch-camvid_amd/conv_fp32.py b/pytorch-camvid_amd/conv_fp32.py
--- a/pytorch-camvid_amd/conv_fp32.py
+++ b/pytorch-camvid_amd/conv_fp32.py
@@ -158,23 +158,28 @@
         executed = (1.5 if h2 else 0.5) * flops
         Pf = lib.cvk_wino4f_stat_partials(N, H, W)
         cnt = self._counts(Pf)
+        wgs, tail, sfx = R.launch_wgs(), (), ""
+        if not h2:
+            ts = 1 if R.w4f_tail and wgs == 0 else 0
+            wsb = lib.cvk_wino4f_tail_workspace_bytes(N, H, W, k_ch, cout, wgs) if ts else 0
+            tail, sfx = ((R.workspace(wsb, x.device).data_ptr() if wsb else None), wsb, ts), "_ts"
         if bnred is not None:
             bpart = _empty(2 * Pf * cout, x.device)
-            name = "cvk_conv3x3_wino4%s_bnred" % f
+            name = "cvk_conv3x3_wino4%s_bnred%s" % (f, sfx)
             _timed(R, "k_conv3x3_wino4%s<bnred>" % f, flops, lambda: check(getattr(lib, name)(
-                x.data_ptr(), U.data_ptr(), self.y.data_ptr(), *am, N, H, W, k_ch, cout, ldy, *bnred, bpart.data_ptr(), R.launch_wgs(), s), name), executed=executed)
+                x.data_ptr(), U.data_ptr(), self.y.data_ptr(), *am, N, H, W, k_ch, cout, ldy, *bnred, bpart.data_ptr(), wgs, *tail, s), name), executed=executed)
             self.bnred_sums = (bpart, Pf)
             return None
         if vplanes:
             self.v = _empty(6 * lib.cvk_wgradp_plane_rows(N, H, W) * k_ch, x.device)
             check(lib.cvk_wgradp_zero_pads_sm(self.v.data_ptr(), N, H, W, k_ch, s), "cvk_wgradp_zero_pads_sm")
             _timed(R, "k_conv3x3_wino4f<vplanes>", flops, lambda: check(
-                lib.cvk_conv3x3_wino4f_vplanes(x.data_ptr(), U.data_ptr(), self.bias, self.y.data_ptr(), self.sp, cnt, self.v.data_ptr(), N, H, W,
-                                               k_ch, cout, ldy, R.launch_wgs(), s), "cvk_conv3x3_wino4f_vplanes" + self.what), executed=executed)
+                lib.cvk_conv3x3_wino4f_vplanes_ts(x.data_ptr(), U.data_ptr(), self.bias, self.y.data_ptr(), self.sp, cnt, self.v.data_ptr(), N, H, W,
+                                                  k_ch, cout, ldy, wgs, *tail, s), "cvk_conv3x3_wino4f_vplanes_ts" + self.what), executed=executed)
         else:
-            name = "cvk_conv3x3_wino4" + f
+            name = "cvk_conv3x3_wino4" + f + sfx
             _timed(R, "k_conv3x3_wino4" + f, flops, lambda: check(getattr(lib, name)(
-                x.data_ptr(), U.data_ptr(), self.bias, self.y.data_ptr(), self.sp, cnt, *am, N, H, W, k_ch, cout, ldy, R.launch_wgs(), s),
+                x.data_ptr(), U.data_ptr(), self.bias, self.y.data_ptr(), self.sp, cnt, *am, N, H, W, k_ch, cout, ldy, wgs, *tail, s),
                 name + self.what), executed=executed)
         return (Pf, cnt) if self.sp is not None else None
 
diff --git a/pytorch-camvid_amd/csrc/wino4f.hip b/pytorch-camvid_amd/csrc/wino4f.hip
--- a/pytorch-camvid_amd/csrc/wino4f.hip
+++ b/pytorch-camvid_amd/csrc/wino4f.hip
@@ -100,6 +100,10 @@
                        blockIdx.x - jobs.first[j], jobs.first[j + 1] - jobs.first[j]);
 }
 
+__global__ __launch_bounds__(256) void k_wino4f_zero(unsigned* __restrict__ p, int n) {
+    for (int i = threadIdx.x; i < n; i += 256) p[i] = 0u;
+}
+
 __device__ __forceinline__ void f_dma16(const void* sbase, unsigned voff, unsigned lds_byte_addr) {
     asm volatile("s_mov_b32 m0, %2\n\ts_nop 0\n\tglobal_load_lds_dwordx4 %0, %1" : : "v"(voff), "s"(sbase), "s"(lds_byte_addr) : "memory");
 }
@@ -122,17 +126,38 @@
     long rows;
     int Wtp;
 };
+struct FTailX { int xbeg, nT, ng, full, r, S; };
+__host__ __device__ inline FTailX f_tail_xcd(int ntiles, int G, int xcd) {
+    const int nx = G < 8 ? G : 8;
+    FTailX t;
+    t.ng = G / nx + (xcd < G % nx ? 1 : 0);
+    t.xbeg = (int)((long)xcd * ntiles / nx);
+    t.nT = (int)((long)(xcd + 1) * ntiles / nx) - t.xbeg;
+    t.full = t.nT / t.ng;
+    t.r = t.nT % t.ng;
+    const int S = t.r > 0 ? t.ng / t.r : 0;
+    t.S = S >= 2 ? (S < 4 ? S : 4) : 0;
+    return t;
+}
+__host__ __device__ inline int f_tail_k(int part, int S, int nS) { return (int)((long)part * nS / S); }
+constexpr int F_TAIL_AUTO_CIN = 128;
+constexpr size_t F_SLAB_FLOATS = (size_t)F_BM * 4 * F_BN;
+struct FTail {
+    unsigned* ctr;
+    float* slabs;
+};
 typedef unsigned u32x4f __attribute__((ext_vector_type(4)));
 typedef _Float16 f16x8 __attribute__((ext_vector_type(8)));
 typedef _Float16 f16x4 __attribute__((ext_vector_type(4)));
 typedef float f32x2v __attribute__((ext_vector_type(2)));
 
-template <bool STATS, int ABL = 0, bool BNR = false, bool H2 = false, bool VPL = false, bool CL = false>
+template <bool STATS, int ABL = 0, bool BNR = false, bool H2 = false, bool VPL = false, bool CL = false, bool TS = false>
 __global__ __launch_bounds__(512, 2) void k_conv3x3_wino4f(
     const float* __restrict__ X, const float* __restrict__ Uf, const float* __restrict__ bias, float* __restrict__ Y,
     float* __restrict__ stats, float* __restrict__ counts, int Mt, int H, int W, int Wt, int Cin, int Cout, int ldy,
-    int tilesN, int ntiles, int Mpix, int P, FBnRed bn, FSplit sp, FVpl vp) {
+    int tilesN, int ntiles, int Mpix, int P, FBnRed bn, FSplit sp, FVpl vp, FTail tl) {
     static_assert(!(STATS && BNR), "forward statistics and the BatchNorm-backward sums are different launches");
+    static_assert(!(TS && (H2 || ABL)), "the tail split exists for the exact-fp32 product kernels only");
     static_assert(!(VPL && (BNR || H2)), "the weight-grad's V planes are written by exact-fp32 forward launches only");
     static_assert(!(CL && H2) && !(VPL && !CL), "LDS constants: exact-fp32 variants; the plane-writing launch always has them");
     __shared__ __attribute__((aligned(1024))) char smem[2 * F_STAGE + 2048 + (CL ? F_CST : 0)];
@@ -162,10 +187,35 @@
     const int ng = G / nx + (xcd < G % nx ? 1 : 0);
     const int xbeg = (int)((long)xcd * ntiles / nx), xend = (int)((long)(xcd + 1) * ntiles / nx);
     const int tbeg = xbeg + wi, tend = xend, tstride = ng;
-    if (tbeg >= tend) return;
-    const int ntw = (tend - tbeg + tstride - 1) / tstride;
     const int nS = 3 * Cin / F_BK;
-    const int total = ntw * nS;
+    int ntw, hs = 0, stile = 0, part = 0, nparts = 0, k0 = 0, k1 = 0, sr0 = 0, sc0 = 0, slab = 0, tctr = 0;
+    if constexpr (TS) {
+        const FTailX tx = f_tail_xcd(ntiles, G, xcd);
+        ntw = tx.full + ((tx.S == 0 && wi < tx.r) ? 1 : 0);
+        hs = tx.S >= 2 && wi < tx.r * tx.S;
+        if (ntw == 0 && !hs) return;
+        if (hs) {
+            nparts = tx.S;
+            part = wi % nparts;
+            stile = xbeg + tx.full * ng + wi / nparts;
+            k0 = f_tail_k(part, nparts, nS);
+            k1 = f_tail_k(part + 1, nparts, nS);
+            sr0 = k0 * F_BK / Cin;
+            sc0 = k0 * F_BK - sr0 * Cin;
+            slab = wi;
+            tctr = wi / nparts;
+            for (int j = 0; j < xcd; ++j) {
+                const FTailX o = f_tail_xcd(ntiles, G, j);
+                slab += o.S ? o.r * o.S : 0;
+                tctr += o.S ? o.r : 0;
+            }
+        }
+    } else {
+        if (tbeg >= tend) return;
+        ntw = (tend - tbeg + tstride - 1) / tstride;
+    }
+    const int total = ntw * nS + (TS ? k1 - k0 : 0);
+    const int stn0 = TS ? stile % tilesN : 0;
     float sA[6];
     CvkUnscale un[6];
 #pragma unroll
@@ -222,7 +272,9 @@
         }
     };
 
-    int ltile = tbeg, lr = 0, lcib = 0, lleft = total;
+    const bool sfirst = TS && ntw == 0;
+    int ltile = sfirst ? stile : tbeg, lr = sfirst ? sr0 : 0, lcib = sfirst ? sc0 : 0, lleft = total, lrem = ntw;
+    bool lfresh = sfirst;
     f32x4 d[2][6];
     auto load_A = [&](int set, int j) {
         const __amdgpu_buffer_rsrc_t xs = (lleft > 0 && !(ABL & 1)) ? xr : null_rsrc;
@@ -238,12 +290,31 @@
         const int w2 = lr == 3;
         lr = w2 ? 0 : lr;
         ltile += w2 ? tstride : 0;
+        if constexpr (TS) {
+            const bool j = w2 && lrem == 1 && hs;
+            lrem -= w2;
+            ltile = j ? stile : ltile;
+            lr = j ? sr0 : lr;
+            lcib = j ? sc0 : lcib;
+            lfresh = j ? true : lfresh;
+        }
+    };
+    auto open_A = [&]() {
+        if constexpr (TS) {
+            if (lcib == 0 || lfresh) {
+                if ((lr == 0 || lfresh) && ltile < tend) set_tile(ltile);
+                regroup(lr);
+                lfresh = false;
+            }
+        } else {
+            if (lcib == 0) {
+                if (lr == 0 && ltile < tend) set_tile(ltile);
+                regroup(lr);
+            }
+        }
     };
     auto issue_A = [&](int set) {
-        if (lcib == 0) {
-            if (lr == 0 && ltile < tend) set_tile(ltile);
-            regroup(lr);
-        }
+        open_A();
 #pragma unroll
         for (int j = 0; j < 6; ++j) load_A(set, j);
         advance_A();
@@ -277,7 +348,7 @@
         if (ABL & 2) return;
         *reinterpret_cast<f32x4*>(stage + x * (F_BM * 64) + wr_off) = tv[x];
     };
-    int st_r = 0, st_cib = F_BK, st_tn = tbeg % tilesN;
+    int st_r = sfirst ? sr0 : 0, st_cib = sfirst ? sc0 : (TS ? 0 : F_BK), st_tn = (sfirst ? stile : tbeg) % tilesN, st_rem = ntw, sleft = total;
     const unsigned vsub = VPL ? (unsigned)(vp.rows * 64) : 0u;
     const unsigned vxs = vsub * (unsigned)(Cin >> 4);
     const unsigned long long vpa = (unsigned long long)vp.p;
@@ -291,6 +362,14 @@
         const int w2 = st_r == 3;
         st_r = w2 ? 0 : st_r;
         st_tn = w2 ? (st_tn + tstride) % tilesN : st_tn;
+        if constexpr (TS) {
+            --sleft;
+            const bool j = w2 && st_rem == 1 && hs;
+            st_rem -= w2;
+            st_r = j ? sr0 : st_r;
+            st_cib = j ? sc0 : st_cib;
+            st_tn = j ? stn0 : st_tn;
+        }
     };
     auto store_V = [&](int x) {
         if (!VPL) return;
@@ -337,7 +416,7 @@
 #pragma unroll
         for (int x = 0; x < 6; ++x) { if (H2) split_A(stage, x); else write_A(stage, x); }
     };
-    int btn = tbeg % tilesN, bslice = 0, bleft = total;
+    int btn = (sfirst ? stile : tbeg) % tilesN, bslice = sfirst ? k0 : 0, bleft = total, brem = ntw;
     const unsigned bvoff = (unsigned)(wave * 3 * 1024 + lane * 16);
     const char* bsrc = nullptr;
     auto dma_B_begin = [&]() {
@@ -346,6 +425,12 @@
             const int w = ++bslice == nS;
             bslice = w ? 0 : bslice;
             btn = w ? (btn + tstride) % tilesN : btn;
+            if constexpr (TS) {
+                const bool j = w && brem == 1 && hs;
+                brem -= w;
+                bslice = j ? k0 : bslice;
+                btn = j ? stn0 : btn;
+            }
         }
     };
     auto dma_B_piece = [&](unsigned stage_addr, int q) {
@@ -391,7 +476,8 @@
         else acc[x] = __builtin_amdgcn_mfma_f32_32x32x16_f16(ha1[slot], hb2, acc[x], 0, 0, 0);
     };
 
-    auto epilogue = [&](int tile) {
+    auto epilogue = [&](int tile, auto pre_) {
+        constexpr bool PRE = decltype(pre_)::value;
         if (ABL & 8) {
             if (tile == -1) {
                 float z = 0.f;
@@ -436,7 +522,8 @@
                             m2 = H2 ? acc[2][e] * un[2].a * un[2].b : acc[2][e], m3 = H2 ? acc[3][e] * un[3].a * un[3].b : acc[3][e],
                             m4 = H2 ? acc[4][e] * un[4].a * un[4].b : acc[4][e], m5 = H2 ? acc[5][e] * un[5].a * un[5].b : acc[5][e];
                 const float s12 = m1 + m2, d12 = m1 - m2, s34 = m3 + m4, d34 = m3 - m4;
-                const float y0 = m0_ + s12 + s34, y1 = fmaf(2.f, d34, d12), y2 = fmaf(4.f, s34, s12), y3 = fmaf(8.f, d34, d12) + m5;
+                const float y0 = PRE ? m0_ : m0_ + s12 + s34, y1 = PRE ? m1 : fmaf(2.f, d34, d12), y2 = PRE ? m2 : fmaf(4.f, s34, s12),
+                            y3 = PRE ? m3 : fmaf(8.f, d34, d12) + m5;
 #pragma unroll
                 for (int x = 0; x < 6; ++x) acc[x][e] = 0.f;
                 const unsigned so = (unsigned)(4 * ((e & 3) + 8 * (e >> 2))) * ls;
@@ -464,7 +551,8 @@
                             m2 = H2 ? acc[2][e] * un[2].a * un[2].b : acc[2][e], m3 = H2 ? acc[3][e] * un[3].a * un[3].b : acc[3][e],
                             m4 = H2 ? acc[4][e] * un[4].a * un[4].b : acc[4][e], m5 = H2 ? acc[5][e] * un[5].a * un[5].b : acc[5][e];
                 const float s12 = m1 + m2, d12 = m1 - m2, s34 = m3 + m4, d34 = m3 - m4;
-                const float y0 = m0_ + s12 + s34, y1 = fmaf(2.f, d34, d12), y2 = fmaf(4.f, s34, s12), y3 = fmaf(8.f, d34, d12) + m5;
+                const float y0 = PRE ? m0_ : m0_ + s12 + s34, y1 = PRE ? m1 : fmaf(2.f, d34, d12), y2 = PRE ? m2 : fmaf(4.f, s34, s12),
+                            y3 = PRE ? m3 : fmaf(8.f, d34, d12) + m5;
 #pragma unroll
                 for (int x = 0; x < 6; ++x) acc[x][e] = 0.f;
                 const int q = (int)divWt.div((unsigned)t), xt = t - q * Wt;
@@ -541,6 +629,14 @@
 #pragma unroll
     for (int q = 0; q < 3; ++q) dma_B_piece(smem_addr, q);
     store_A(buf0, 0);
+    if constexpr (TS && VPL) {
+        if (st_r == 1 && st_tn == 0) {
+            vso = (unsigned)(st_cib >> 4) * vsub;
+#pragma unroll
+            for (int x = 0; x < 6; ++x) store_V(x);
+        }
+        advance_staged();
+    }
     issue_A(0);
     cvk_wait_vm<6>();
     cvk_lds_retire_barrier();
@@ -548,12 +644,9 @@
 #define F_SB() __builtin_amdgcn_sched_barrier(0)
     auto step = [&](auto par_, const char* cur, char* nxt, unsigned nxt_addr) {
         constexpr int SET = 1 - decltype(par_)::value;
-        const bool VST = VPL && st_r == 1 && st_tn == 0;
+        const bool VST = VPL && st_r == 1 && st_tn == 0 && (!TS || sleft > 0);
         if (VPL) vso = (unsigned)(st_cib >> 4) * vsub;
-        if (lcib == 0) {
-            if (lr == 0 && ltile < tend) set_tile(ltile);
-            regroup(lr);
-        }
+        open_A();
         dma_B_begin();
         load_frag(cur, 0, 0);
         F_SB();
@@ -637,6 +730,7 @@
         cvk_wait_vm<6>();
         cvk_lds_retire_barrier();
     };
+    if constexpr (!TS) {
     for (int tile = tbeg; tile < tend; tile += tstride) {
         for (int ks = 0; ks < nS; ks += 2) {
             if (H2) {
@@ -647,7 +741,59 @@
                 step(std::integral_constant<int, 1>{}, buf1, buf0, smem_addr);
             }
         }
-        epilogue(tile);
+        epilogue(tile, std::false_type{});
+    }
+    } else {
+    for (int it = 0, tile = tbeg; it < ntw + hs; ++it, tile += tstride) {
+        const int nk = it < ntw ? nS : k1 - k0;
+        for (int ks = 0; ks < nk; ks += 2) {
+            step(std::integral_constant<int, 0>{}, buf0, buf1, smem_addr + F_STAGE);
+            step(std::integral_constant<int, 1>{}, buf1, buf0, smem_addr);
+        }
+        if (it < ntw) epilogue(tile, std::false_type{});
+    }
+    if (hs) {
+        f32x4* const mine = reinterpret_cast<f32x4*>(tl.slabs + (size_t)slab * F_SLAB_FLOATS) + tid;
+#pragma unroll
+        for (int e = 0; e < 16; ++e) {
+            const float m0_ = acc[0][e], m1 = acc[1][e], m2 = acc[2][e], m3 = acc[3][e], m4 = acc[4][e], m5 = acc[5][e];
+            const float s12 = m1 + m2, d12 = m1 - m2, s34 = m3 + m4, d34 = m3 - m4;
+            const f32x4 yv = {m0_ + s12 + s34, fmaf(2.f, d34, d12), fmaf(4.f, s34, s12), fmaf(8.f, d34, d12) + m5};
+            mine[e * 512] = yv;
+        }
+        asm volatile("s_waitcnt vmcnt(0)" ::: "memory");
+        __syncthreads();
+        unsigned* const flag = reinterpret_cast<unsigned*>(red);
+        if (tid == 0) {
+            __builtin_amdgcn_fence(__ATOMIC_RELEASE, "agent");
+            asm volatile("s_waitcnt vmcnt(0)" ::: "memory");
+            *flag = __hip_atomic_fetch_add(tl.ctr + tctr, 1u, __ATOMIC_RELAXED, __HIP_MEMORY_SCOPE_AGENT);
+        }
+        __syncthreads();
+        const unsigned ticket = *flag;
+        if (ticket == (unsigned)(nparts - 1)) {
+        if (tid == 0) {
+            __builtin_amdgcn_fence(__ATOMIC_ACQUIRE, "agent");
+            asm volatile("s_waitcnt vmcnt(0)" ::: "memory");
+        }
+        __syncthreads();
+        const f32x4* const all = reinterpret_cast<const f32x4*>(tl.slabs + (size_t)(slab - part) * F_SLAB_FLOATS) + tid;
+#pragma unroll
+        for (int e = 0; e < 16; ++e) {
+            const f32x4 v = all[e * 512];
+            acc[0][e] = v[0]; acc[1][e] = v[1]; acc[2][e] = v[2]; acc[3][e] = v[3];
+        }
+        for (int p = 1; p < nparts; ++p) {
+            const f32x4* const sl = all + (size_t)p * (F_SLAB_FLOATS / 4);
+#pragma unroll
+            for (int e = 0; e < 16; ++e) {
+                const f32x4 v = sl[e * 512];
+                acc[0][e] += v[0]; acc[1][e] += v[1]; acc[2][e] += v[2]; acc[3][e] += v[3];
+            }
+        }
+        epilogue(stile, std::true_type{});
+        }
+    }
     }
 #undef F_SB
     cvk_wait_vm<0>();
@@ -694,9 +840,67 @@
     return cvk_cdiv((long)N * H * ((W + 3) / 4), F_BM);
 }
 
+struct FTailTotals { int items, tiles; };
+static FTailTotals f_tail_totals(int ntiles, int grid) {
+    FTailTotals t = {0, 0};
+    for (int xcd = 0; xcd < (grid < 8 ? grid : 8); ++xcd) {
+        const FTailX o = f_tail_xcd(ntiles, grid, xcd);
+        if (o.S) { t.items += o.r * o.S; t.tiles += o.r; }
+    }
+    return t;
+}
+static inline size_t f_tail_ctr_bytes(int tiles) { return ((size_t)tiles * 4 + 255) / 256 * 256; }
+static int f_cus() {
+    static int cus = 0;
+    if (cus == 0) {
+        int dev = 0, v = 0;
+        if (hipGetDevice(&dev) == hipSuccess && hipDeviceGetAttribute(&v, hipDeviceAttributeMultiprocessorCount, dev) == hipSuccess && v > 0) cus = v;
+        else cus = 256;
+    }
+    return cus;
+}
+static inline int f_grid(int ntiles, int max_workgroups) {
+    const int cus = f_cus();
+    const int wgs = (max_workgroups > 0 && max_workgroups < cus) ? max_workgroups : cus;
+    return ntiles < wgs ? ntiles : wgs;
+}
+
+extern "C" size_t cvk_wino4f_tail_workspace_bytes(int N, int H, int W, int Cin, int Cout, int max_workgroups) {
+    if (N <= 0 || H <= 0 || W <= 0 || Cin <= 0 || Cout <= 0) return 0;
+    const int ntiles = cvk_cdiv((long)N * H * ((W + 3) / 4), F_BM) * f_tiles_n(Cout);
+    if (Cout > F_CMAX) return 0;
+    const FTailTotals t = f_tail_totals(ntiles, f_grid(ntiles, max_workgroups));
+    return t.items ? f_tail_ctr_bytes(t.tiles) + (size_t)t.items * F_SLAB_FLOATS * 4 : 0;
+}
+
+extern "C" int cvk_wino4f_tail_plan(int ntiles, int grid, int Cin, int* xcds, int* items, int max_items) {
+    CVK_CHECK_ARG(ntiles > 0 && grid > 0 && grid <= ntiles && Cin >= 32 && Cin % 32 == 0 && xcds, "cvk_wino4f_tail_plan: bad arguments");
+    const int nx = grid < 8 ? grid : 8, nS = 3 * Cin / F_BK;
+    int n = 0, slab0 = 0, ctr0 = 0;
+    for (int xcd = 0; xcd < 8; ++xcd) {
+        int* const row = xcds + 6 * xcd;
+        for (int j = 0; j < 6; ++j) row[j] = 0;
+        if (xcd >= nx) continue;
+        const FTailX o = f_tail_xcd(ntiles, grid, xcd);
+        row[0] = o.xbeg; row[1] = o.nT; row[2] = o.ng; row[3] = o.full; row[4] = o.r; row[5] = o.S;
+        if (!o.S) continue;
+        for (int wi = 0; wi < o.r * o.S; ++wi, ++n) {
+            CVK_CHECK_ARG(items && n < max_items, "cvk_wino4f_tail_plan: more than %d work items", max_items);
+            int* const it = items + 6 * n;
+            it[0] = wi * nx + xcd; it[1] = o.xbeg + o.full * o.ng + wi / o.S;
+            it[2] = f_tail_k(wi % o.S, o.S, nS); it[3] = f_tail_k(wi % o.S + 1, o.S, nS);
+            it[4] = slab0 + wi; it[5] = ctr0 + wi / o.S;
+        }
+        slab0 += o.r * o.S;
+        ctr0 += o.r;
+    }
+    return n;
+}
+
 static int wino4f_launch(const char* who, const float* x, const float* Uf, const float* bias, float* y, float* stats, float* counts,
                          const FBnRed* bn, int N, int H, int W, int Cin, int Cout, int ldy, int max_workgroups, void* stream,
-                         const void* amax_x = nullptr, const void* amax_w = nullptr, float* vplanes = nullptr) {
+                         const void* amax_x = nullptr, const void* amax_w = nullptr, float* vplanes = nullptr,
+                         void* workspace = nullptr, size_t workspace_bytes = 0, int tail_split = 0) {
     CVK_CHECK_ARG(x && Uf && y, "%s: null pointer", who);
     CVK_CHECK_ARG(N > 0 && H > 0 && W > 0 && Cout > 0 && ldy >= Cout, "%s: bad shape", who);
     CVK_CHECK_ARG(Cin >= 32 && Cin % 32 == 0, "%s: Cin=%d must be a multiple of 32", who, Cin);
@@ -706,14 +910,7 @@
     const int Wt = (W + 3) / 4, Mt = N * H * Wt, Mpix = N * H * W;
     CVK_CHECK_ARG((long)Mt * Wt < (1L << 32) && (long)N * H * H < (1L << 32), "%s: frame too large for the multiply-high coordinate split", who);
     const int tilesN = f_tiles_n(Cout), tilesM = cvk_cdiv(Mt, F_BM), ntiles = tilesM * tilesN;
-    static int cus = 0;
-    if (cus == 0) {
-        int dev = 0, v = 0;
-        if (hipGetDevice(&dev) == hipSuccess && hipDeviceGetAttribute(&v, hipDeviceAttributeMultiprocessorCount, dev) == hipSuccess && v > 0) cus = v;
-        else cus = 256;
-    }
-    const int wgs = (max_workgroups > 0 && max_workgroups < cus) ? max_workgroups : cus;
-    const int grid = ntiles < wgs ? ntiles : wgs;
+    const int grid = f_grid(ntiles, max_workgroups);
     CVK_CHECK_ARG((F_BM * 4 + 3L * W + 8) * Cin * 4 < (1L << 31), "%s: a tile's input window exceeds the 2 GiB buffer-addressing limit", who);
     hipStream_t s = (hipStream_t)stream;
     const FBnRed none = {nullptr, nullptr, nullptr, nullptr, nullptr};
@@ -731,11 +928,34 @@
     }
     const bool cl = Cout <= F_CMAX;
     CVK_CHECK_ARG(!vplanes || cl, "%s: the plane-writing launch needs Cout <= %d", who, F_CMAX);
+    CVK_CHECK_ARG(tail_split >= 0 && tail_split <= 2, "%s: tail_split is 0 (off), 1 (auto) or 2 (every splittable geometry)", who);
+    FTail tl = {nullptr, nullptr};
+    if ((tail_split == 2 || (tail_split == 1 && Cin >= F_TAIL_AUTO_CIN)) && !h2 && cl) {
+        const FTailTotals t = f_tail_totals(ntiles, grid);
+        if (t.items) {
+            const size_t cb = f_tail_ctr_bytes(t.tiles);
+            CVK_CHECK_ARG(workspace && cvk_aligned16(workspace) && workspace_bytes >= cb + (size_t)t.items * F_SLAB_FLOATS * 4,
+                          "%s: the tail split needs a 16-byte aligned workspace of cvk_wino4f_tail_workspace_bytes() bytes", who);
+            tl.ctr = (unsigned*)workspace;
+            tl.slabs = (float*)((char*)workspace + cb);
+            hipLaunchKernelGGL(k_wino4f_zero, dim3(1), dim3(256), 0, s, tl.ctr, (int)(cb / 4));
+        }
+    }
+#define CVK_W4F_TS(ST_, BN_, VP_, BNV_) hipLaunchKernelGGL((k_conv3x3_wino4f<ST_, 0, BN_, false, VP_, true, true>), dim3(grid), dim3(512), 0, s, x, Uf, bias, y, \
+                                                           stats, counts, Mt, H, W, Wt, Cin, Cout, ldy, tilesN, ntiles, Mpix, tilesM, BNV_, sp, vp, tl)
+    if (tl.ctr) {
+        if (vplanes)    { if (stats) CVK_W4F_TS(true, false, true, none); else CVK_W4F_TS(false, false, true, none); }
+        else if (bn)    CVK_W4F_TS(false, true, false, *bn);
+        else if (stats) CVK_W4F_TS(true, false, false, none);
+        else            CVK_W4F_TS(false, false, false, none);
+        CVK_LAUNCH_RETURN(who);
+    }
+#undef CVK_W4F_TS
 #define CVK_W4F_GO(ST_, BN_, H2_, CL_, BNV_) hipLaunchKernelGGL((k_conv3x3_wino4f<ST_, 0, BN_, H2_, false, CL_>), dim3(grid), dim3(512), 0, s, x, Uf, bias, y, \
-                                                                stats, counts, Mt, H, W, Wt, Cin, Cout, ldy, tilesN, ntiles, Mpix, tilesM, BNV_, sp, vp)
+                                                                stats, counts, Mt, H, W, Wt, Cin, Cout, ldy, tilesN, ntiles, Mpix, tilesM, BNV_, sp, vp, tl)
 #define CVK_W4F_GO2(ST_, BN_, BNV_) do { if (cl) CVK_W4F_GO(ST_, BN_, false, true, BNV_); else CVK_W4F_GO(ST_, BN_, false, false, BNV_); } while (0)
 #define CVK_W4F_GOV(ST_) hipLaunchKernelGGL((k_conv3x3_wino4f<ST_, 0, false, false, true, true>), dim3(grid), dim3(512), 0, s, x, Uf, bias, y, stats, counts, \
-                                            Mt, H, W, Wt, Cin, Cout, ldy, tilesN, ntiles, Mpix, tilesM, none, sp, vp)
+                                            Mt, H, W, Wt, Cin, Cout, ldy, tilesN, ntiles, Mpix, tilesM, none, sp, vp, tl)
     if (vplanes)    { if (stats) CVK_W4F_GOV(true); else CVK_W4F_GOV(false); }
     else if (bn)    { if (h2) CVK_W4F_GO(false, true, true, false, *bn); else CVK_W4F_GO2(false, true, *bn); }
     else if (stats) { if (h2) CVK_W4F_GO(true, false, true, false, none); else CVK_W4F_GO2(true, false, none); }
@@ -764,6 +984,28 @@
     CVK_CHECK_ARG(yP && scale && shift && mean && rstd && part, "cvk_conv3x3_wino4f_bnred: null pointer");
     const FBnRed bn = {yP, scale, shift, mean, rstd};
     return wino4f_launch("cvk_conv3x3_wino4f_bnred", x, Uf, nullptr, y, part, nullptr, &bn, N, H, W, Cin, Cout, ldy, max_workgroups, stream);
+}
+
+extern "C" int cvk_conv3x3_wino4f_ts(const float* x, const float* Uf, const float* bias, float* y, float* stats, float* counts, int N, int H, int W,
+                                     int Cin, int Cout, int ldy, int max_workgroups, void* workspace, size_t workspace_bytes, int tail_split,
+                                     void* stream) {
+    return wino4f_launch("cvk_conv3x3_wino4f_ts", x, Uf, bias, y, stats, counts, nullptr, N, H, W, Cin, Cout, ldy, max_workgroups, stream,
+                         nullptr, nullptr, nullptr, workspace, workspace_bytes, tail_split);
+}
+extern "C" int cvk_conv3x3_wino4f_vplanes_ts(const float* x, const float* Uf, const float* bias, float* y, float* stats, float* counts, float* Vsm,
+                                             int N, int H, int W, int Cin, int Cout, int ldy, int max_workgroups, void* workspace,
+                                             size_t workspace_bytes, int tail_split, void* stream) {
+    CVK_CHECK_ARG(Vsm, "cvk_conv3x3_wino4f_vplanes_ts: null plane pointer");
+    return wino4f_launch("cvk_conv3x3_wino4f_vplanes_ts", x, Uf, bias, y, stats, counts, nullptr, N, H, W, Cin, Cout, ldy, max_workgroups, stream,
+                         nullptr, nullptr, Vsm, workspace, workspace_bytes, tail_split);
+}
+extern "C" int cvk_conv3x3_wino4f_bnred_ts(const float* x, const float* Uf, float* y, int N, int H, int W, int Cin, int Cout, int ldy,
+                                           const float* yP, const float* scale, const float* shift, const float* mean, const float* rstd,
+                                           float* part, int max_workgroups, void* workspace, size_t workspace_bytes, int tail_split, void* stream) {
+    CVK_CHECK_ARG(yP && scale && shift && mean && rstd && part, "cvk_conv3x3_wino4f_bnred_ts: null pointer");
+    const FBnRed bn = {yP, scale, shift, mean, rstd};
+    return wino4f_launch("cvk_conv3x3_wino4f_bnred_ts", x, Uf, nullptr, y, part, nullptr, &bn, N, H, W, Cin, Cout, ldy, max_workgroups, stream,
+                         nullptr, nullptr, nullptr, workspace, workspace_bytes, tail_split);
 }
 
 extern "C" int cvk_wino4h_weight_transform(const float* w, void* Uh, const void* amax_w, int Cn, int Ck, int dgrad, void* stream) {
@@ -798,7 +1040,7 @@
     const int tilesN = f_tiles_n(Cout), tilesM = cvk_cdiv(Mt, F_BM), ntiles = tilesM * tilesN;
     const int grid = ntiles < 256 ? ntiles : 256;
     hipStream_t s = (hipStream_t)stream;
-#define CVK_ABL(A) case A: hipLaunchKernelGGL((k_conv3x3_wino4f<false, A>), dim3(grid), dim3(512), 0, s, x, Uf, bias, y, nullptr, nullptr, Mt, H, W, Wt, Cin, Cout, ldy, tilesN, ntiles, Mpix, tilesM, FBnRed{nullptr, nullptr, nullptr, nullptr, nullptr}, FSplit{nullptr, nullptr, CvkSplitTab{}, CvkSplitTab{}}, FVpl{nullptr, 0, 0}); break;
+#define CVK_ABL(A) case A: hipLaunchKernelGGL((k_conv3x3_wino4f<false, A>), dim3(grid), dim3(512), 0, s, x, Uf, bias, y, nullptr, nullptr, Mt, H, W, Wt, Cin, Cout, ldy, tilesN, ntiles, Mpix, tilesM, FBnRed{nullptr, nullptr, nullptr, nullptr, nullptr}, FSplit{nullptr, nullptr, CvkSplitTab{}, CvkSplitTab{}}, FVpl{nullptr, 0, 0}, FTail{nullptr, nullptr}); break;
     switch (abl) {
         CVK_ABL(0) CVK_ABL(1) CVK_ABL(2) CVK_ABL(3) CVK_ABL(4) CVK_ABL(7) CVK_ABL(8) CVK_ABL(9) CVK_ABL(11) CVK_ABL(15) CVK_ABL(16) CVK_ABL(24) CVK_ABL(31)
         default: return -1;
@@ -813,7 +1055,7 @@
     const int grid = ntiles < 256 ? ntiles : 256;
     hipStream_t s = (hipStream_t)stream;
     const FSplit sp = {(const unsigned*)amax_x, (const unsigned*)amax_w, cvk_split_tab(4, CVK_SPLIT_KIND_B), cvk_split_tab(4, CVK_SPLIT_KIND_G)};
-#define CVK_ABLH(A) case A: hipLaunchKernelGGL((k_conv3x3_wino4f<false, A, false, true>), dim3(grid), dim3(512), 0, s, x, (const float*)Uh, bias, y, nullptr, nullptr, Mt, H, W, Wt, Cin, Cout, ldy, tilesN, ntiles, Mpix, tilesM, FBnRed{nullptr, nullptr, nullptr, nullptr, nullptr}, sp, FVpl{nullptr, 0, 0}); break;
+#define CVK_ABLH(A) case A: hipLaunchKernelGGL((k_conv3x3_wino4f<false, A, false, true>), dim3(grid), dim3(512), 0, s, x, (const float*)Uh, bias, y, nullptr, nullptr, Mt, H, W, Wt, Cin, Cout, ldy, tilesN, ntiles, Mpix, tilesM, FBnRed{nullptr, nullptr, nullptr, nullptr, nullptr}, sp, FVpl{nullptr, 0, 0}, FTail{nullptr, nullptr}); break;
     switch (abl) {
         CVK_ABLH(0) CVK_ABLH(1) CVK_ABLH(2) CVK_ABLH(4) CVK_ABLH(8) CVK_ABLH(9) CVK_ABLH(11) CVK_ABLH(15) CVK_ABLH(16) CVK_ABLH(31) CVK_ABLH(32) CVK_ABLH(33) CVK_ABLH(64) CVK_ABLH(65)
         default: return -1;
diff --git a/pytorch-camvid_amd/engine.py b/pytorch-camvid_amd/engine.py
--- a/pytorch-camvid_amd/engine.py
+++ b/pytorch-camvid_amd/engine.py
@@ -102,6 +102,7 @@
 WINO4F_DEFAULT = os.environ.get("CVK_WINO4F", "1") != "0"
 WGRADP_DEFAULT = {"0": False, "1": True, "always": "always"}[os.environ.get("CVK_WGRADP", "1")]
 VPLANES_DEFAULT = os.environ.get("CVK_VPLANES", "1") != "0"
+W4F_TAIL_DEFAULT = os.environ.get("CVK_W4F_TAIL", "1") != "0"
 
 
 def amax_blocks(lib, n, dev):
@@ -504,6 +505,7 @@
         self.wino4f = WINO4F_DEFAULT
         self.wgradp = WGRADP_DEFAULT
         self.vplanes = VPLANES_DEFAULT
+        self.w4f_tail = W4F_TAIL_DEFAULT
         self.thin = os.environ.get("CVK_THIN", "1") != "0"
         self.pool_bnred = os.environ.get("CVK_POOL_BNRED", "1") != "0"
         self.wino2d = WINO2D_DEFAULT
@@ -704,7 +706,7 @@
 
     def kernel_config(self):
         return (self.wino, self.wino4, self.wino4f, self.wino2d, self.wgradp, self.vplanes, self.thin, self.pool_bnred, self.w2d_split,
-                self.w2tile_cfg)
+                self.w2tile_cfg, self.w4f_tail)
 
     def routes(self, plan, training, need_grad):
         key = (self.kernel_config(), training, need_grad)
```

Result: no change. 248.3 images/s (median of 6 runs) (+0.2%).
